# dcmlr/groundgrid

Measured on AMD Instinct MI355X. Metric: point clouds/s (Velodyne-64, ~120k pts, 120m/0.33m grid), higher is better.
Workload: dtype f32+f64 (the reference's mixed float/double arithmetic, bit-exact)

## Files before the change

groundgrid_amd/csrc/gg_context.hip:

```cpp
#include <float.h>
#include <math.h>
#include <stdio.h>
#include <string.h>

#include <algorithm>
#include <atomic>
#include <condition_variable>
#include <cstdlib>
#include <cstdio>
#include <functional>
#include <mutex>
#include <string>
#include <thread>
#include <vector>
#include <chrono>

#include <dlfcn.h>
#include <sched.h>
#include <unistd.h>

#include "gg_internal.h"
#include "host_helper.h"
#include "scroll_core.h"
#include "sweep_core.h"
// ... 816 lines not shown
    a.slot_cfg_launch = own_half[0] ? 1 : 0;
    if (split) {
        if (!ctx->probe_no_fork) {
            HIPCHK(ctx, hipEventRecord(ctx->half_fork, s));
            HIPCHK(ctx, hipStreamWaitEvent(ctx->half_stream, ctx->half_fork, 0));
        }
        Arena a2 = a;
        a2.front_sync = a.front_sync2;
        a2.sweep_sync = a.sweep_sync2;
        a2.sweep_rec_clouds = 0;
        a2.scan_sync = a.scan_sync2;
        a2.slot_cfg_launch = own_half[1] ? 1 : 0;
        a.fresh_launch = fresh_half[0] ? 1 : 0;
        a2.fresh_launch = fresh_half[1] ? 1 : 0;
        if (const int rc = fill_fresh(0, n_first, s)) return rc;
        if (const int rc = fill_fresh(n_first, nb, ctx->half_stream)) return rc;
        HIPCHK(ctx, hipMemcpyAsync(dp, hp, sizeof(CloudParams) * n_first, hipMemcpyHostToDevice, s));
        HIPCHK(ctx, hipMemcpyAsync(dp + n_first, hp + n_first, sizeof(CloudParams) * (nb - n_first), hipMemcpyHostToDevice, ctx->half_stream));
        launch_sequence(ctx, a, dp, score_half[0] ? io_score : io, n_first, max_n[0], s, nullptr, hp[0].slot, false, score_half[0]);
        launch_sequence(ctx, a2, dp + n_first, score_half[1] ? io_score : io, nb - n_first, max_n[1], ctx->half_stream, nullptr, hp[n_first].slot, false, score_half[1]);
        HIPCHK(ctx, hipGetLastError());
        HIPCHK(ctx, ctx->ring.recorded2(g, ctx->half_stream));
        HIPCHK(ctx, hipEventRecord(ctx->half_done, ctx->half_stream));
        ctx->have_half_event = true;
    } else {
        a.fresh_launch = fresh_half[0] ? 1 : 0;
        if (const int rc = fill_fresh(0, nb, s)) return rc;
        if (const int rc = launch_or_replay(ctx, a, hp, dp, score_half[0] ? io_score : io, nb, max_n[0], s, plan, score_half[0])) return rc;
        HIPCHK(ctx, hipGetLastError());
    }
    HIPCHK(ctx, ctx->ring.recorded(g, s));
    HIPCHK(ctx, hipEventRecord(ctx->batch_event, s));
    ctx->last_batch_stream = s;
    ctx->have_batch_event = true;
    if (s != ctx->stream) ctx->map_event_pending = false;
    return GG_OK;
}

void free_call_scratch(CallScratch &m)
{
    if (m.dev) hipFree(m.dev);
    if (m.pinned) hipHostFree(m.pinned);
    m = CallScratch{};
}
void free_call_scratch(CallScratch &m, ParamRing &r)
{
    free_call_scratch(m);
    r.destroy();
}

struct TableUpload {
    size_t offset;
    const void *src;
    size_t bytes;
};
int alloc_call_scratch(gg_context *ctx, const char *who, hipStream_t st, size_t dev_bytes, size_t pinned_bytes, std::initializer_list<TableUpload> tables, CallScratch *mem,
                       ParamRing *ring)
{
    hipStreamCaptureStatus cs = hipStreamCaptureStatusNone;
    if (hipStreamIsCapturing(st, &cs) == hipSuccess && cs != hipStreamCaptureStatusNone)
        return fail(ctx, GG_ERR_INVALID, who, "the first call allocates its scratch and cannot be captured into a graph");
    (void)hipGetLastError();
    CallScratch m;
    ParamRing r;
    int code = GG_ERR_NOMEM;
    const char *what = "device scratch";
    hipError_t e = hipMalloc(&m.dev, dev_bytes);
    if (e != hipSuccess) m.dev = nullptr;
    if (e == hipSuccess) {
        what = "pinned parameter ring";
        e = hipHostMalloc(&m.pinned, pinned_bytes, hipHostMallocDefault);
        if (e != hipSuccess) m.pinned = nullptr;
    }
    if (e == hipSuccess) code = GG_ERR_HIP;
    if (e == hipSuccess && ring) {
        what = "events";
        e = r.create();
    }
    for (const TableUpload &t : tables)
        if (e == hipSuccess) {
            what = "table upload";
            e = hipMemcpy((char *)m.dev + t.offset, t.src, t.bytes, hipMemcpyHostToDevice);
        }
    if (e != hipSuccess) {
        free_call_scratch(m, r);
        (void)hipGetLastError();
        return fail(ctx, code, (std::string(who) + ": " + what).c_str(), e);
    }
    *mem = m;
    if (ring) *ring = r;
    return GG_OK;
}

void map_shift(double res, double pos_x, double pos_y, double odom_x, double odom_y, int s[2], double moved[2])
{
    const double odom[2] = {odom_x, odom_y};
    const double pos[2] = {pos_x, pos_y};
    for (int i = 0; i < 2; ++i) {
        const double tmp = (odom[i] - pos[i]) / res;
        s[i] = -(int)(tmp + 0.5 * (tmp > 0 ? 1 : -1));
        moved[i] = pos[i] + (double)(-s[i]) * res;
    }
}

}

static int rebuild_patch_table(gg_context *ctx, const DevConfig &cfg);

extern "C" {

int gg_abi_version(void) { return GG_ABI_VERSION; }

const char *gg_kernel_name(int k)
{
    static const char *names[GG_NUM_KERNELS] = {"k_classify", "k_scan", "k_scatter", "k_reduce", "k_patch", "k_sweep", "k_label"};
    return (k >= 0 && k < GG_NUM_KERNELS) ? names[k] : "?";
}

void gg_default_config(gg_config *c)
{
    if (!c) return;
    c->point_count_cell_variance_threshold = 10;
    c->max_ring = 1024;
    c->groundpatch_detection_minimum_threshold = 0.01;
    c->distance_factor = 0.0001;
    c->minimum_distance_factor = 0.0005;
    c->miminum_point_height_threshold = 0.3;
    c->minimum_point_height_obstacle_threshold = 0.1;
    c->outlier_tolerance = 0.1;
    c->ground_patch_detection_minimum_point_count_threshold = 0.25;
    c->patch_size_change_distance = 20;
    c->occupied_cells_decrease_factor = 5.0;
    c->occupied_cells_point_count_factor = 20;
    c->min_outlier_detection_ground_confidence = 1.25;
    c->thread_count = 8;
}

void gg_default_geometry(gg_geometry *g)
{
    if (!g) return;
    g->length = 120.0f;
    g->resolution = .33f;
    g->vertical_point_ang_dist = (float)(0.00174532925 * 2);
    g->min_dist_squared = 12.0f;
}

int gg_create(const gg_geometry *geom_in, int n_slots, size_t max_points, int device, gg_context **out)
{
    if (!out) return GG_ERR_INVALID;
    *out = nullptr;
    if (n_slots <= 0 || max_points == 0 || max_points > (size_t)1 << 30) return GG_ERR_INVALID;
    gg_geometry geom;
    gg_default_geometry(&geom);
    if (geom_in) {
        if (geom_in->length > 0.f) geom.length = geom_in->length;
        if (geom_in->resolution > 0.f) geom.resolution = geom_in->resolution;
        const float sensor[2] = {geom_in->vertical_point_ang_dist, geom_in->min_dist_squared};
        for (const float v : sensor)
            if (!(v >= 0.f) || isinf(v)) return GG_ERR_GEOMETRY;
        if (geom_in->vertical_point_ang_dist > 0.f) geom.vertical_point_ang_dist = geom_in->vertical_point_ang_dist;
        if (geom_in->min_dist_squared > 0.f) geom.min_dist_squared = geom_in->min_dist_squared;
    }

    const double res = (double)geom.resolution;
    const int n = (int)round((double)geom.length / res);
    const size_t dimension = (size_t)geom.length;
    const size_t cellCount = (size_t)roundf((float)dimension / geom.resolution);
    if (n < 8 || (size_t)n != cellCount) return GG_ERR_GEOMETRY;

    int ndev = 0;
    if (hipGetDeviceCount(&ndev) != hipSuccess || ndev <= 0 || device < 0 || device >= ndev) return GG_ERR_NO_DEVICE;
    hipDeviceProp_t prop;
    if (hipGetDeviceProperties(&prop, device) != hipSuccess) return GG_ERR_NO_DEVICE;
    if (strncmp(prop.gcnArchName, "gfx950", 6) != 0) return GG_ERR_NO_DEVICE;

    gg_context *ctx = new (std::nothrow) gg_context();
    if (!ctx) return GG_ERR_NOMEM;
    ctx->device = device;
    ctx->geom = geom;
    ctx->n_slots = n_slots;
    ctx->max_points = max_points;
    gg_default_config(&ctx->cfg);
    ctx->pos_x.assign(n_slots, 0.0);
    ctx->no_confidence.assign(n_slots, 0);
    ctx->fresh.assign(n_slots, 0);
    ctx->fresh_z.assign(n_slots, 0.0f);
    ctx->fresh_enabled = !(getenv("GG_FRESH_MAPS") && atoi(getenv("GG_FRESH_MAPS")) == 0);
    ctx->lazy_pending.assign(n_slots, 0);
    ctx->lazy_params.assign(n_slots, CloudParams{});
    ctx->slot_own.assign(n_slots, 0);
    ctx->score_on.assign(n_slots, 0);
    ctx->slot_cfg.assign(n_slots, gg_config{});
    ctx->slot_dev.assign(n_slots, DevConfig{});
    ctx->pos_y.assign(n_slots, 0.0);

#define CREATE_CHK(call)                                             \
    do {                                                             \
        hipError_t e__ = (call);                                     \
        if (e__ != hipSuccess) {                                     \
            fprintf(stderr, "groundgrid_hip: %s failed: %s\n", #call, hipGetErrorString(e__)); \
            gg_destroy(ctx);                                         \
            return e__ == hipErrorOutOfMemory ? GG_ERR_NOMEM : GG_ERR_HIP; \
        }                                                            \
    } while (0)

    CREATE_CHK(hipSetDevice(device));
    CREATE_CHK(hipStreamCreateWithFlags(&ctx->stream, hipStreamNonBlocking));
    CREATE_CHK(hipStreamCreateWithFlags(&ctx->h2d_stream, hipStreamNonBlocking));
    CREATE_CHK(hipStreamCreateWithFlags(&ctx->d2h_stream, hipStreamNonBlocking));
    CREATE_CHK(hipStreamCreateWithFlags(&ctx->half_stream, hipStreamNonBlocking));
    CREATE_CHK(hipEventCreateWithFlags(&ctx->half_fork, hipEventDisableTiming));
    CREATE_CHK(hipEventCreateWithFlags(&ctx->half_done, hipEventDisableTiming));
    CREATE_CHK(hipEventCreateWithFlags(&ctx->map_event, hipEventDisableTiming));
    CREATE_CHK(hipEventCreateWithFlags(&ctx->batch_event, hipEventDisableTiming));
    CREATE_CHK(hipEventCreateWithFlags(&ctx->gather_event, hipEventDisableTiming));
    CREATE_CHK(hipEventCreateWithFlags(&ctx->fork_event, hipEventDisableTiming));
    CREATE_CHK(hipEventCreateWithFlags(&ctx->join_event, hipEventDisableTiming));
    CREATE_CHK(hipEventCreateWithFlags(&ctx->layers_event, hipEventDisableTiming));
    if (const char *e = getenv("GG_GRAPH")) ctx->graphs_enabled = atoi(e) != 0;

    Arena &a = ctx->arena;
    Geometry &g = a.g;
    g.rows = g.cols = n;
    g.C = n * n;
    g.tiles_r = (n + TILE - 1) / TILE;
    g.tiles_c = (n + TILE - 1) / TILE;
    g.T = g.tiles_r * g.tiles_c;
    g.resolution = res;
    g.inv_resolution = 1.0 / res;
    g.length0 = g.length1 = (double)n * res;
    g.half0 = 0.5 * g.length0;
    g.half1 = 0.5 * g.length1;
    g.resolution_f = (float)res;
    g.min_dist_squared = geom.min_dist_squared;
    g.center = n / 2 - 1;
    a.hist_pitch = (g.T + 3) & ~3;
    a.n_slots = n_slots;
    if (g.T > 65535 || (size_t)4 * a.hist_pitch * sizeof(uint32_t) > 150 * 1024) {
        gg_destroy(ctx);
        return GG_ERR_GEOMETRY;
    }
    a.PW = g.T <= 1024 ? (n_slots >= PW_BIG_CONTEXT_SLOTS ? 2048 : 1024) : 8192;
    if (getenv("GG_PW")) a.PW = atoi(getenv("GG_PW"));
    if (a.PW < 64 || a.PW % 64 != 0) {
        gg_destroy(ctx);
        return GG_ERR_INVALID;
    }
    a.tune_sweep_waves = getenv("GG_SWEEP_WAVES") ? atoi(getenv("GG_SWEEP_WAVES")) : 0;
    a.tune_sweep_gpw = getenv("GG_SWEEP_GPW") ? atoi(getenv("GG_SWEEP_GPW")) : 0;
    a.tune_sweep_split = getenv("GG_SWEEP_SPLIT") ? atoi(getenv("GG_SWEEP_SPLIT")) : 0;
    a.tune_sweep_pair = getenv("GG_SWEEP_PAIR") ? atoi(getenv("GG_SWEEP_PAIR")) : 0;
    a.tune_sweep_pair_wgs = getenv("GG_SWEEP_PAIR_WGS") ? atoi(getenv("GG_SWEEP_PAIR_WGS")) : 0;
    a.tune_sweep_pair_waves = getenv("GG_SWEEP_PAIR_WAVES") ? atoi(getenv("GG_SWEEP_PAIR_WAVES")) : 0;
    a.tune_front = getenv("GG_FRONT") ? atoi(getenv("GG_FRONT")) : 0;
    a.tune_k2_per_cloud = getenv("GG_K2_PER_CLOUD") ? atoi(getenv("GG_K2_PER_CLOUD")) : 0;
    a.tune_k2_dense_share = getenv("GG_K2_DENSE_SHARE") ? atoi(getenv("GG_K2_DENSE_SHARE")) : 0;
    a.k2_skip = getenv("GG_K2_SKIP") ? atoi(getenv("GG_K2_SKIP")) : 0;
    a.NCH = (int)((max_points + a.PW - 1) / a.PW);
    make_dev_config(ctx->cfg, a.cfg);

    ctx->h_expected.resize((size_t)g.C);
    for (size_t i = 0; i < cellCount; ++i)
        for (size_t j = 0; j < cellCount; ++j) {
            const float dist = (float)hypot((double)i - (double)cellCount / 2.0, (double)j - (double)cellCount / 2.0);
            ctx->h_expected[i + j * cellCount] = atanf(1 / dist) / geom.vertical_point_ang_dist;
        }

    ctx->sweep_params = gg::sweep::make_params(n, res, geom.min_dist_squared, ctx->cfg.occupied_cells_decrease_factor);
    if (gg::sweep_lds_bytes(ctx->sweep_params) > 158 * 1024) {
        gg_destroy(ctx);
        return GG_ERR_GEOMETRY;
    }
    std::vector<uint16_t> tile_rank(g.T), rank_tile(g.T);
    {
        std::vector<std::pair<uint32_t, int>> order(g.T);
        for (int tc = 0; tc < g.tiles_c; ++tc)
            for (int tr = 0; tr < g.tiles_r; ++tr) order[tr + tc * g.tiles_r] = {morton2((uint32_t)tr, (uint32_t)tc), tr + tc * g.tiles_r};
        std::sort(order.begin(), order.end());
        for (int r = 0; r < g.T; ++r) {
            rank_tile[r] = (uint16_t)order[r].second;
            tile_rank[order[r].second] = (uint16_t)r;
        }
    }

    const size_t A = 256;
    size_t off = 0;
    auto carve = [&](size_t bytes) {
        const size_t o = off;
        off = align_up(off + bytes, A);
        return o;
    };
    const size_t C = (size_t)g.C;
    const size_t Cpad = align_up(C * 4, A) / 4;
    const size_t Npad = align_up(max_points * 8, A) / 8;
    const size_t o_expected = carve(C * 4);
    const size_t o_ptable = carve(C * 16);
    const size_t o_trank = carve((size_t)g.T * 2);
    const size_t o_rtile = carve((size_t)g.T * 2);
    const size_t o_rcell0 = carve((size_t)g.T * 4);
    const size_t percall_slot_floats = align_up((size_t)g.T * PERCALL_BLOCK * 4, A) / 4;
    const size_t o_layers = carve((size_t)n_slots * percall_slot_floats * 4);
    a.gpl = make_gp_layout(n);
    a.gp_bits_off = (int)align_up((size_t)a.gpl.elems, 16);
    a.gp_bits_words = (a.gpl.elems / 64 + 2 + 1) & ~1;
    a.gp2_stride = align_up(((size_t)a.gp_bits_off + (size_t)a.gp_bits_words) * 8, A) / 8;
    a.gp_bits_stride = a.gp2_stride;
    const size_t o_gp2 = carve((size_t)n_slots * a.gp2_stride * 8);
    const size_t o_rec = carve((size_t)n_slots * Npad * 8);
    const size_t o_sorted = carve((size_t)n_slots * Npad * 8);
    a.zcell_stride = align_up((Npad + (size_t)32 * g.T + 64) * 4, A) / 4;
    const size_t o_zcell = carve((size_t)n_slots * a.zcell_stride * 4);
    a.hist_stride = align_up((size_t)a.NCH * a.hist_pitch * 4, A) / 4;
    const size_t o_hist = carve((size_t)n_slots * a.hist_stride * 4);
    a.emit_stride = align_up((size_t)a.NCH * 4 * 4, A) / 4;
    const size_t o_emit = carve((size_t)n_slots * a.emit_stride * 4);
    const size_t o_totals = carve((size_t)n_slots * 4 * 4);
    a.tile_start_stride = align_up((size_t)(g.T + 1) * 4, A) / 4;
    const size_t o_tstart = carve((size_t)n_slots * a.tile_start_stride * 4);
    a.tile_live_stride = align_up((size_t)g.T, A);
    const size_t o_tlive = carve((size_t)n_slots * a.tile_live_stride * 4);
    a.tile_list_stride = align_up((size_t)g.T * 16, A) / 16;
    const size_t o_tlist = carve((size_t)n_slots * a.tile_list_stride * 16);
    const size_t o_tlcnt = carve((size_t)n_slots * 2 * 4);
    const size_t o_fsync = carve(((size_t)2 * n_slots + 16) * 4);
    const size_t o_ssync = carve(64);
    const size_t o_fsync2 = carve(((size_t)2 * n_slots + 16) * 4);
    const size_t o_ssync2 = carve(64);
    const size_t o_scansync = carve((size_t)n_slots * SCAN_SYNC_WORDS * 8);
    const size_t o_scansync2 = carve((size_t)n_slots * SCAN_SYNC_WORDS * 8);
    a.sweep_xchg_stride = align_up(std::max<size_t>(gg::sweep_xchg_entries(ctx->sweep_params), 1) * 16, A) / 8;
    const size_t o_xchg = carve((size_t)n_slots * a.sweep_xchg_stride * 8);
    a.sweep_rec_stride = gg::sweep_pair_rec_floats(ctx->sweep_params);
    a.sweep_rec_clouds = a.sweep_rec_stride ? std::min(n_slots, SWEEP_PAIR_MAX_CLOUDS) : 0;
    const size_t o_srec = carve(std::max<size_t>((size_t)a.sweep_rec_clouds * a.sweep_rec_stride * 4, 64));
    const size_t o_params = carve((size_t)PARAM_RING * n_slots * sizeof(CloudParams));
    const size_t o_gparams = carve(sizeof(CloudParams));
    const size_t o_spts = carve(max_points * sizeof(gg_point16));
    const size_t o_slab = carve(max_points);
    const size_t o_sidx = carve(max_points * 4);
    const size_t o_scnt = carve(64);
    const size_t o_scls = carve(max_points);
    const size_t o_scell = carve(max_points * 4);
    size_t o_apts[GG_ASYNC_DEPTH], o_alab[GG_ASYNC_DEPTH], o_aidx[GG_ASYNC_DEPTH], o_acnt[GG_ASYNC_DEPTH];
    for (int k = 0; k < GG_ASYNC_DEPTH; ++k) {
        o_apts[k] = carve(max_points * sizeof(gg_point16));
        o_acnt[k] = carve(64 + max_points * 5 + 64);
        o_aidx[k] = o_alab[k] = 0;
    }
    const size_t o_scroll = carve(a.gp2_stride * 8);
    const size_t o_image = carve(3 * Cpad * 4);
    const size_t o_bounds = carve(64);
    const size_t gp_valid_words = ((size_t)a.gpl.elems + 31) / 32;
    const size_t o_gpvalid = carve(gp_valid_words * 4);
    std::vector<int> gp_border;
    for (int col = 0; col < n; ++col)
        for (int row = 0; row < n; ++row)
            if (std::max(std::abs(row - a.gpl.c), std::abs(col - a.gpl.c)) >= a.gpl.c) gp_border.push_back(gp_index(a.gpl, row, col));
    a.gp_border_n = (int)gp_border.size();
    const size_t o_gpborder = carve(std::max<size_t>(gp_border.size() * 4, 64));
    a.gp_fresh_cell = 1 + (a.gpl.VS - 1) * 64;
    const size_t o_dbg = carve(64 * 8);
    const size_t o_pdbg = carve(2048 * 8);
    const bool k2_timing = getenv("GG_K2_DEBUG") && (atoi(getenv("GG_K2_DEBUG")) == 9 || atoi(getenv("GG_K2_DEBUG")) == 5 || atoi(getenv("GG_K2_DEBUG")) == 6);
    const size_t o_k2dbg = carve(k2_timing ? (size_t)K2_DBG_WGS * 32 * 8 : 64);
    const size_t o_slotmaps = carve((size_t)n_slots * sizeof(ExportMap));
    ctx->arena_bytes = off;
    CREATE_CHK(hipMalloc(&ctx->d_arena, ctx->arena_bytes));
    char *base = (char *)ctx->d_arena;
    CREATE_CHK(hipMemsetAsync(base, 0, ctx->arena_bytes, ctx->stream));

    a.expected = (const float *)(base + o_expected);
    a.patch_table = (const float4 *)(base + o_ptable);
    a.tile_rank = (const uint16_t *)(base + o_trank);
    a.rank_tile = (const uint16_t *)(base + o_rtile);
    a.rank_cell0 = (const uint32_t *)(base + o_rcell0);
    a.layers = (float *)(base + o_layers);
    a.gp2 = (float2 *)(base + o_gp2);
    a.gp_bits = (unsigned long long *)(base + o_gp2) + a.gp_bits_off;
    a.slot_layer_stride = percall_slot_floats;
    a.rec = (uint2 *)(base + o_rec);
    a.sorted = (uint2 *)(base + o_sorted);
    a.zcell = (float *)(base + o_zcell);
    a.point_stride = Npad;
    a.hist = (uint32_t *)(base + o_hist);
    a.chunk_emit = (uint32_t *)(base + o_emit);
    a.totals = (uint32_t *)(base + o_totals);
    a.tile_start = (uint32_t *)(base + o_tstart);
    a.tile_live = (uint32_t *)(base + o_tlive);
    a.tile_list = (uint4 *)(base + o_tlist);
    a.tile_list_cnt = (uint32_t *)(base + o_tlcnt);
    a.front_sync = (uint32_t *)(base + o_fsync);
    a.sweep_sync = (uint32_t *)(base + o_ssync);
    a.front_sync2 = (uint32_t *)(base + o_fsync2);
    a.sweep_sync2 = (uint32_t *)(base + o_ssync2);
    a.scan_sync = (unsigned long long *)(base + o_scansync);
    a.scan_sync2 = (unsigned long long *)(base + o_scansync2);
    {
        const uint32_t first_epoch[4] = {0u, 0u, 1u, 0u};
        CREATE_CHK(hipMemcpyAsync(a.sweep_sync, first_epoch, sizeof first_epoch, hipMemcpyHostToDevice, ctx->stream));
        const uint32_t first_epoch2[4] = {0u, 0u, 0x80000001u, 0u};
        CREATE_CHK(hipMemcpyAsync(a.sweep_sync2, first_epoch2, sizeof first_epoch2, hipMemcpyHostToDevice, ctx->stream));
        CREATE_CHK(hipStreamSynchronize(ctx->stream));
    }
    {
        CREATE_CHK(hipHostMalloc((void **)&ctx->h_dev_error, 64, hipHostMallocMapped));
        *ctx->h_dev_error = 0u;
        void *dptr = nullptr;
        CREATE_CHK(hipHostGetDevicePointer(&dptr, (void *)ctx->h_dev_error, 0));
        a.dev_error = (uint32_t *)dptr;
    }
    a.sweep_xchg = (unsigned long long *)(base + o_xchg);
    a.sweep_rec = a.sweep_rec_clouds ? (float *)(base + o_srec) : nullptr;
    a.pair_dbg = getenv("GG_PAIR_TIMING") ? (unsigned long long *)(base + o_pdbg) : nullptr;
    a.flags = 0;
    a.k2_debug = getenv("GG_K2_DEBUG") ? atoi(getenv("GG_K2_DEBUG")) : 0;
    a.k2_dbg = (unsigned long long *)(base + o_k2dbg);
    a.k3_debug = getenv("GG_K3_DEBUG") ? atoi(getenv("GG_K3_DEBUG")) : 0;
    a.k5_debug = getenv("GG_K5_DEBUG") ? atoi(getenv("GG_K5_DEBUG")) : 0;
    ctx->d_params = (CloudParams *)(base + o_params);
    ctx->d_gparams = (CloudParams *)(base + o_gparams);
    ctx->d_stage_pts = (gg_point16 *)(base + o_spts);
    ctx->d_stage_labels = (uint8_t *)(base + o_slab);
    ctx->d_stage_index = (int32_t *)(base + o_sidx);
    ctx->d_stage_counts = (int32_t *)(base + o_scnt);
    ctx->d_stage_class = (uint8_t *)(base + o_scls);
    ctx->d_stage_cell = (int32_t *)(base + o_scell);
    for (int k = 0; k < GG_ASYNC_DEPTH; ++k) {
        gg_context::AsyncSlot &as = ctx->async_slot[k];
        as.d_pts = (gg_point16 *)(base + o_apts[k]);
        as.d_counts = (int32_t *)(base + o_acnt[k]);
        as.d_index = (int32_t *)(base + o_acnt[k] + 64);
        as.d_labels = nullptr;
    }
    ctx->d_scroll_scratch = (float *)(base + o_scroll);
    ctx->d_image = (float *)(base + o_image);
    ctx->d_bounds = (float *)(base + o_bounds);
    a.gp_valid = (const uint32_t *)(base + o_gpvalid);
    a.gp_border = (const int *)(base + o_gpborder);
    {
        int row, col;
        if (gp_cell_of(a.gpl, a.gp_fresh_cell, row, col)) {
            gg_destroy(ctx);
            return GG_ERR_INVALID;
        }
        CREATE_CHK(hipMemcpyAsync(base + o_gpborder, gp_border.data(), gp_border.size() * 4, hipMemcpyHostToDevice, ctx->stream));
        CREATE_CHK(hipStreamSynchronize(ctx->stream));
    }
    if (getenv("GG_SWEEP_TIMING")) {
        ctx->d_sweep_dbg = (unsigned long long *)(base + o_dbg);
        const unsigned long long mode = getenv("GG_SWEEP_DEBUG") ? strtoull(getenv("GG_SWEEP_DEBUG"), nullptr, 0) : 0ull;
        hipStreamSynchronize(ctx->stream);
        hipMemcpy(ctx->d_sweep_dbg + 63, &mode, 8, hipMemcpyHostToDevice);
    }

    std::vector<uint32_t> gp_valid(gp_valid_words, 0u);
    for (int col = 0; col < n; ++col)
        for (int row = 0; row < n; ++row) {
            const int e = gp_index(a.gpl, row, col);
            gp_valid[(size_t)e >> 5] |= 1u << (e & 31);
        }
    {
        const int group = getenv("GG_FILL_GROUP") ? atoi(getenv("GG_FILL_GROUP")) : 16;
        if (group == 8 || group == 16 || group == 32)
            for (size_t w = 0; w < gp_valid_words; ++w) {
                uint32_t v = gp_valid[w], o = 0u;
                for (int b = 0; b < 32; b += group) {
                    const uint32_t gm = (group == 32 ? 0xFFFFFFFFu : ((1u << group) - 1u)) << b;
                    if (v & gm) o |= gm;
                }
                gp_valid[w] = o;
            }
    }
    CREATE_CHK(hipMemcpyAsync(base + o_gpvalid, gp_valid.data(), gp_valid_words * 4, hipMemcpyHostToDevice, ctx->stream));
    CREATE_CHK(hipMemcpyAsync(base + o_expected, ctx->h_expected.data(), C * 4, hipMemcpyHostToDevice, ctx->stream));
    CREATE_CHK(hipMemcpyAsync(base + o_trank, tile_rank.data(), (size_t)g.T * 2, hipMemcpyHostToDevice, ctx->stream));
    CREATE_CHK(hipMemcpyAsync(base + o_rtile, rank_tile.data(), (size_t)g.T * 2, hipMemcpyHostToDevice, ctx->stream));
    std::vector<uint32_t> rank_cell0(g.T);
    for (int r = 0; r < g.T; ++r) {
        const int tile = rank_tile[r];
        rank_cell0[r] = (uint32_t)((tile % g.tiles_r) * TILE) | ((uint32_t)((tile / g.tiles_r) * TILE) << 16);
    }
    CREATE_CHK(hipMemcpyAsync(base + o_rcell0, rank_cell0.data(), (size_t)g.T * 4, hipMemcpyHostToDevice, ctx->stream));
    std::vector<ExportMap> slot_maps((size_t)n_slots);
    for (int s = 0; s < n_slots; ++s) slot_maps[(size_t)s] = ExportMap{s, 0, 0.0f, 0};
    CREATE_CHK(hipMemcpyAsync(base + o_slotmaps, slot_maps.data(), slot_maps.size() * sizeof(ExportMap), hipMemcpyHostToDevice, ctx->stream));
    ctx->d_slot_maps = (const ExportMap *)(base + o_slotmaps);
    CREATE_CHK(hipStreamSynchronize(ctx->stream));

    CREATE_CHK(hipHostMalloc((void **)&ctx->h_params, sizeof(CloudParams) * PARAM_RING * n_slots, hipHostMallocDefault));
    CREATE_CHK(hipHostMalloc((void **)&ctx->h_stage_pts, max_points * sizeof(gg_point16), hipHostMallocDefault));
    CREATE_CHK(hipHostMalloc((void **)&ctx->h_stage_labels, max_points, hipHostMallocDefault));
    CREATE_CHK(hipHostMalloc((void **)&ctx->h_stage_index, max_points * 4, hipHostMallocDefault));
    CREATE_CHK(hipHostMalloc((void **)&ctx->h_stage_counts, 64, hipHostMallocDefault));
    CREATE_CHK(ctx->ring.create());
    for (int k = 0; k < GG_ASYNC_DEPTH; ++k) {
        gg_context::AsyncSlot &as = ctx->async_slot[k];
        CREATE_CHK(hipHostMalloc((void **)&as.h_pts, max_points * sizeof(gg_point16), hipHostMallocDefault));
        CREATE_CHK(hipHostMalloc((void **)&as.h_counts, 64 + max_points * 5 + 64, hipHostMallocDefault));
        as.h_index = as.h_counts + 16;
        as.h_labels = nullptr;
        if (hipHostGetDevicePointer((void **)&as.hd_counts, as.h_counts, 0) != hipSuccess) {
            as.hd_counts = nullptr;
            (void)hipGetLastError();
        }
        CREATE_CHK(hipEventCreateWithFlags(&as.uploaded, hipEventDisableTiming));
        CREATE_CHK(hipEventCreateWithFlags(&as.computed, hipEventDisableTiming));
        CREATE_CHK(hipEventCreateWithFlags(&as.downloaded, hipEventDisableTiming));
    }

    ctx->helper.configure((getenv("GG_HOST_THREADS") ? std::max(1, std::min(atoi(getenv("GG_HOST_THREADS")), 16)) : 8) - 1);
    {
        const int rc = rebuild_patch_table(ctx, a.cfg);
        if (rc != GG_OK) {
            gg_destroy(ctx);
            return rc;
        }
    }
    {
        const int rc = gg_reset_maps(ctx, 0, n_slots, 0.0, 0.0, 0.0f, 0, nullptr);
        if (rc != GG_OK) {
            gg_destroy(ctx);
            return rc;
        }
    }
    CREATE_CHK(hipStreamSynchronize(ctx->stream));
#undef CREATE_CHK
    *out = ctx;
    return GG_OK;
}

void gg_destroy(gg_context *ctx)
{
    if (!ctx) return;
    ctx->helper.stop();
    hipSetDevice(ctx->device);
    if (ctx->have_batch_event) hipEventSynchronize(ctx->batch_event);
    if (ctx->half_stream) hipStreamSynchronize(ctx->half_stream);
    if (ctx->h2d_stream) hipStreamSynchronize(ctx->h2d_stream);
    if (ctx->stream) hipStreamSynchronize(ctx->stream);
    if (ctx->d2h_stream) hipStreamSynchronize(ctx->d2h_stream);
    for (auto &p : ctx->pending) {
        if (p.owns_start) hipEventDestroy(p.start);
        hipEventDestroy(p.stop);
    }
    for (hipEvent_t e : ctx->free_single_events) hipEventDestroy(e);
    ctx->ring.destroy();
    if (ctx->half_fork) hipEventDestroy(ctx->half_fork);
    if (ctx->half_done) hipEventDestroy(ctx->half_done);
    if (ctx->half_stream) hipStreamDestroy(ctx->half_stream);
    for (int k = 0; k < GG_ASYNC_DEPTH; ++k) {
        gg_context::AsyncSlot &as = ctx->async_slot[k];
        if (as.h_pts) hipHostFree(as.h_pts);
        if (as.h_counts) hipHostFree(as.h_counts);
        if (as.uploaded) hipEventDestroy(as.uploaded);
        if (as.computed) hipEventDestroy(as.computed);
        if (as.downloaded) hipEventDestroy(as.downloaded);
    }
    if (ctx->map_event) hipEventDestroy(ctx->map_event);
    if (ctx->batch_event) hipEventDestroy(ctx->batch_event);
    if (ctx->gather_event) hipEventDestroy(ctx->gather_event);
    drop_graphs(ctx);
    if (ctx->fork_event) hipEventDestroy(ctx->fork_event);
    if (ctx->join_event) hipEventDestroy(ctx->join_event);
    if (ctx->layers_event) hipEventDestroy(ctx->layers_event);
    for (auto &r : ctx->registered) hipHostUnregister(r.first);
    ctx->registered.clear();
    if (ctx->h2d_stream) hipStreamDestroy(ctx->h2d_stream);
    if (ctx->d2h_stream) hipStreamDestroy(ctx->d2h_stream);
    if (ctx->h_dev_error) hipHostFree((void *)ctx->h_dev_error);
    if (ctx->h_params) hipHostFree(ctx->h_params);
    if (ctx->h_stage_pts) hipHostFree(ctx->h_stage_pts);
    if (ctx->h_stage_labels) hipHostFree(ctx->h_stage_labels);
    if (ctx->h_stage_index) hipHostFree(ctx->h_stage_index);
    if (ctx->h_stage_counts) hipHostFree(ctx->h_stage_counts);
    if (ctx->d_planes) hipFree(ctx->d_planes);
    free_call_scratch(ctx->move_mem, ctx->move_ring);
    free_call_scratch(ctx->export_mem, ctx->export_ring);
    free_call_scratch(ctx->split_mem);
    if (ctx->d_pc2) hipFree(ctx->d_pc2);
    if (ctx->h_pc2) hipHostFree(ctx->h_pc2);
    if (ctx->h_planes) hipHostFree(ctx->h_planes);
    if (ctx->d_arena) hipFree(ctx->d_arena);
    if (ctx->d_slot_cfg) hipFree(ctx->d_slot_cfg);
    if (ctx->d_score_block) hipFree(ctx->d_score_block);
    if (ctx->stream) hipStreamDestroy(ctx->stream);
    delete ctx;
}

static int wait_for_batches_in_flight(gg_context *ctx)
{
    HIPCHK(ctx, hipSetDevice(ctx->device));
    if (ctx->have_batch_event) HIPCHK(ctx, hipEventSynchronize(ctx->batch_event));
    if (ctx->have_half_event) HIPCHK(ctx, hipEventSynchronize(ctx->half_done));
    HIPCHK(ctx, hipStreamSynchronize(ctx->stream));
    return GG_OK;
}

static int rebuild_patch_table(gg_context *ctx, const DevConfig &cfg)
{
    const Geometry &g = ctx->arena.g;
    const int rows = g.rows, cols = g.cols;
    std::vector<float> t((size_t)g.C * 4);
    const double res2 = (double)g.resolution_f * (double)g.resolution_f;
    for (int j = 0; j < cols; ++j)
        for (int i = 0; i < rows; ++i) {
            float *e = &t[((size_t)i + (size_t)j * rows) * 4];
            const float expected = ctx->h_expected[(size_t)i + (size_t)j * rows];
// ... 1224 lines not shown
    unsigned mask = 0u;
    if (layers)
        for (int l = 0; l < GG_NUM_LAYERS; ++l)
            if (layers[l]) mask |= 1u << l;
    if (!mask || (ctx->flags & GG_FLAG_MINIMAL_LAYERS)) {
        const int rc = filter_cloud_impl(ctx, slot, cloud, n, map_from_cloud, origin, base_z, out_cloud, out_n, out_label, out_index);
        if (rc != GG_OK || !mask) return rc;
        void *d[GG_NUM_LAYERS];
        for (int l = 0; l < GG_NUM_LAYERS; ++l) d[l] = layers[l];
        return get_layers_impl(ctx, slot, d);
    }
    HIPCHK(ctx, hipSetDevice(ctx->device));
    const size_t C = (size_t)ctx->arena.g.C, plane = align_up(C * 4, 256) / 4;
    if (!ctx->d_planes) HIPCHK(ctx, hipMalloc((void **)&ctx->d_planes, (size_t)GG_NUM_LAYERS * plane * sizeof(float)));
    if (!ctx->h_planes) HIPCHK(ctx, hipHostMalloc((void **)&ctx->h_planes, (size_t)GG_NUM_LAYERS * plane * sizeof(float), hipHostMallocDefault));
    LayerPlan plan;
    plan.mask = mask;
    bool staged[GG_NUM_LAYERS] = {};
    for (int l = 0; l < GG_NUM_LAYERS; ++l) {
        if (!((mask >> l) & 1u)) continue;
        staged[l] = !host_range_registered(ctx, layers[l], C * sizeof(float));
        plan.dst[l] = staged[l] ? (void *)(ctx->h_planes + (size_t)l * plane) : (void *)layers[l];
    }
    int ticket = -1;
    const int rc = enqueue_ticket(ctx, slot, cloud, n, map_from_cloud, origin, base_z, &ticket, false, &plan);
    if (rc != GG_OK) {
        (void)hipStreamSynchronize(ctx->d2h_stream);
        (void)hipStreamSynchronize(ctx->stream);
        return rc;
    }
    auto copy_staged = [&](unsigned group) {
        int want[GG_NUM_LAYERS], n_want = 0;
        for (int l = 0; l < GG_NUM_LAYERS; ++l)
            if (staged[l] && ((group >> l) & 1u)) want[n_want++] = l;
        if (n_want)
            ctx->helper.split((size_t)n_want * C, [&](size_t lo, size_t hi) {
                for (size_t k = lo / C; k < (size_t)n_want && k * C < hi; ++k) {
                    const size_t a0 = std::max(lo, k * C) - k * C, a1 = std::min(hi, (k + 1) * C) - k * C;
                    memcpy(layers[want[k]] + a0, ctx->h_planes + (size_t)want[k] * plane + a0, (a1 - a0) * sizeof(float));
                }
            });
    };
    if (mask & EARLY_LAYERS) {
        HIPCHK(ctx, hipEventSynchronize(ctx->join_event));
        copy_staged(EARLY_LAYERS);
    }
    const int rc_wait = gg_filter_cloud_wait(ctx, ticket, out_cloud, out_n, out_label, out_index);
    SYNCCHK(ctx, hipEventSynchronize(ctx->layers_event));
    if (rc_wait != GG_OK) return rc_wait;
    if (ctx->layer_copy_failed) {
        ctx->layer_copy_failed = false;
        ctx->last_error = "gg_filter_cloud_layers: a layer download could not be enqueued";
        return GG_ERR_HIP;
    }
    copy_staged(~EARLY_LAYERS);
    return GG_OK;
}

extern "C++" {
namespace {
struct Rccl {
    struct UniqueId {
        char internal[128];
    };
    int (*GetUniqueId)(UniqueId *) = nullptr;
    int (*CommInitRank)(void **, int, UniqueId, int) = nullptr;
    int (*CommDestroy)(void *) = nullptr;
    int (*AllGather)(const void *, void *, size_t, int, void *, hipStream_t) = nullptr;
    const char *(*GetErrorString)(int) = nullptr;
    bool ok = false;
    Rccl()
    {
        void *h = dlopen("librccl.so.1", RTLD_NOW | RTLD_GLOBAL);
        if (!h) h = dlopen("librccl.so", RTLD_NOW | RTLD_GLOBAL);
        if (!h) h = dlopen("/opt/rocm/lib/librccl.so.1", RTLD_NOW | RTLD_GLOBAL);
        if (!h) return;
        GetUniqueId = reinterpret_cast<decltype(GetUniqueId)>(dlsym(h, "ncclGetUniqueId"));
        CommInitRank = reinterpret_cast<decltype(CommInitRank)>(dlsym(h, "ncclCommInitRank"));
        CommDestroy = reinterpret_cast<decltype(CommDestroy)>(dlsym(h, "ncclCommDestroy"));
        AllGather = reinterpret_cast<decltype(AllGather)>(dlsym(h, "ncclAllGather"));
        GetErrorString = reinterpret_cast<decltype(GetErrorString)>(dlsym(h, "ncclGetErrorString"));
        ok = GetUniqueId && CommInitRank && CommDestroy && AllGather;
    }
};
Rccl &rccl()
{
    static Rccl r;
    return r;
}
}
}

int gg_collective_available(void) { return rccl().ok ? 1 : 0; }

int gg_comm_unique_id(uint8_t id_out[128])
{
    if (!id_out) return GG_ERR_INVALID;
    if (!rccl().ok) return GG_ERR_NO_DEVICE;
    Rccl::UniqueId id;
    if (rccl().GetUniqueId(&id) != 0) return GG_ERR_HIP;
    memcpy(id_out, id.internal, 128);
    return GG_OK;
}

int gg_comm_init_rank(const uint8_t id_in[128], int n_ranks, int rank, void **comm_out)
{
    if (!id_in || !comm_out || n_ranks <= 0 || rank < 0 || rank >= n_ranks) return GG_ERR_INVALID;
    *comm_out = nullptr;
    if (!rccl().ok) return GG_ERR_NO_DEVICE;
    Rccl::UniqueId id;
    memcpy(id.internal, id_in, 128);
    if (rccl().CommInitRank(comm_out, n_ranks, id, rank) != 0) return GG_ERR_HIP;
    return GG_OK;
}

int gg_comm_init_rank_for(gg_context *ctx, const uint8_t id_in[128], int n_ranks, int rank, void **comm_out)
{
    if (!ctx) return GG_ERR_INVALID;
    HIPCHK(ctx, hipSetDevice(ctx->device));
    const int rc = gg_comm_init_rank(id_in, n_ranks, rank, comm_out);
    if (rc != GG_OK) fail(ctx, rc, rc == GG_ERR_NO_DEVICE ? "librccl.so could not be loaded" : "ncclCommInitRank failed");
    return rc;
}

int gg_comm_destroy(void *comm)
{
    if (!comm) return GG_ERR_INVALID;
    if (!rccl().ok) return GG_ERR_NO_DEVICE;
    return rccl().CommDestroy(comm) == 0 ? GG_OK : GG_ERR_HIP;
}

int gg_allgather_label_masks(gg_context *ctx, void *comm, const uint8_t *d_send, uint8_t *d_recv, size_t bytes_per_rank, void *stream)
{
    if (!ctx) return GG_ERR_INVALID;
    if (!comm) return fail(ctx, GG_ERR_INVALID, "gg_allgather_label_masks: null communicator");
    if (!d_send || !d_recv || bytes_per_rank == 0) return fail(ctx, GG_ERR_INVALID, "gg_allgather_label_masks: null buffer / zero size");
    if (!rccl().ok) return fail(ctx, GG_ERR_NO_DEVICE, "librccl.so could not be loaded");
    HIPCHK(ctx, hipSetDevice(ctx->device));
    const hipStream_t s = pick_stream(ctx, stream);
    if (ctx->have_batch_event && ctx->last_batch_stream != s) HIPCHK(ctx, hipStreamWaitEvent(s, ctx->batch_event, 0));
    if (const int rc_half = stream_waits_for_second_half(ctx, s)) return rc_half;
    const int rc = rccl().AllGather(d_send, d_recv, bytes_per_rank,  1, comm, s);
    if (rc != 0) {
        char buf[256];
        snprintf(buf, sizeof buf, "ncclAllGather: %s", rccl().GetErrorString ? rccl().GetErrorString(rc) : "error");
        ctx->last_error = buf;
        return GG_ERR_HIP;
    }
    HIPCHK(ctx, hipEventRecord(ctx->gather_event, s));
    ctx->gather_stream = s;
    ctx->gather_lo = d_send;
    ctx->gather_hi = d_send + bytes_per_rank;
    return GG_OK;
}

int gg_get_point_classes(gg_context *ctx, int slot, size_t n, uint8_t *out_class, int32_t *out_cell)
{
    if (!slot_ok(ctx, slot)) return GG_ERR_CAPACITY;
    if (n > ctx->max_points) return GG_ERR_CAPACITY;
    if (n == 0) return GG_OK;
    HIPCHK(ctx, hipSetDevice(ctx->device));
    if (const int rc = own_stream_waits_for_batches(ctx)) return rc;
    launch_decode_classes(ctx->arena, slot, n, ctx->d_stage_class, ctx->d_stage_cell, ctx->stream);
    HIPCHK(ctx, hipGetLastError());
    if (out_class) HIPCHK(ctx, hipMemcpyAsync(out_class, ctx->d_stage_class, n, hipMemcpyDeviceToHost, ctx->stream));
    if (out_cell) HIPCHK(ctx, hipMemcpyAsync(out_cell, ctx->d_stage_cell, n * 4, hipMemcpyDeviceToHost, ctx->stream));
    SYNCCHK(ctx, hipStreamSynchronize(ctx->stream));
    return GG_OK;
}

int gg_run_stage(gg_context *ctx, int slot, int stage, const gg_stage_args *args)
{
    if (!slot_ok(ctx, slot)) return GG_ERR_CAPACITY;
    if (!args) return fail(ctx, GG_ERR_INVALID, "gg_run_stage: null arguments");
    const Geometry &g = ctx->arena.g;
    switch (stage) {
    case GG_STAGE_DETECT_GROUND_PATCHES:
        if (args->section < -1 || args->section > 3) return fail(ctx, GG_ERR_INVALID, "gg_run_stage: section must be 0..3 or -1");
        break;
    case GG_STAGE_SPIRAL_GROUND_INTERPOLATION: break;
    case GG_STAGE_DETECT_GROUND_PATCH_3:
    case GG_STAGE_DETECT_GROUND_PATCH_5: {
        const int h = stage == GG_STAGE_DETECT_GROUND_PATCH_3 ? 1 : 2;
        if (args->i < h || args->j < h || args->i >= g.rows - h || args->j >= g.cols - h) return fail(ctx, GG_ERR_INVALID, "gg_run_stage: the cell's block leaves the map");
        break;
    }
    case GG_STAGE_INTERPOLATE_CELL:
        if (args->i < 1 || args->j < 1 || args->i >= g.rows - 1 || args->j >= g.cols - 1) return fail(ctx, GG_ERR_INVALID, "gg_run_stage: the cell's block leaves the map");
        break;
    default: return fail(ctx, GG_ERR_INVALID, "gg_run_stage: unknown stage");
    }
    HIPCHK(ctx, hipSetDevice(ctx->device));
    if (const int rc = own_stream_waits_for_batches(ctx)) return rc;
    const hipStream_t s = ctx->stream;
    Arena a = ctx->arena;
    a.flags = ctx->flags;
    a.eigen_reduction = ctx->conv.eigen_reduction;
    const bool own = ctx->slot_own[slot] != 0;
    if (own) a.cfg = ctx->slot_dev[slot];
    if (stage == GG_STAGE_DETECT_GROUND_PATCHES || stage == GG_STAGE_SPIRAL_GROUND_INTERPOLATION) {
        int r;
        HIPCHK(ctx, ctx->ring.acquire(&r));
        CloudParams *hp = ctx->h_params + (size_t)r * ctx->n_slots, *dp = ctx->d_params + (size_t)r * ctx->n_slots;
        hp[0] = CloudParams{};
        hp[0].slot = slot;
        hp[0].base_z = (float)args->base_z;
        hp[0].pos_x = ctx->pos_x[slot];
        hp[0].pos_y = ctx->pos_y[slot];
        hp[0].cfg_index = own ? slot : -1;
        HIPCHK(ctx, hipMemcpyAsync(dp, hp, sizeof(CloudParams), hipMemcpyHostToDevice, s));
        if (stage == GG_STAGE_DETECT_GROUND_PATCHES) {
            a.slot_cfg_launch = own ? 1 : 0;
            launch_patch_stage(a, dp, slot, args->section, s);
        } else {
            sweep::Params sp = ctx->sweep_params;
            sp.decrease = own ? ctx->slot_cfg[slot].occupied_cells_decrease_factor : ctx->cfg.occupied_cells_decrease_factor;
            sp.inv_decrease = 1.0 / sp.decrease;
            sp.decay_fast = sp.decrease >= 1.25 && sp.decrease < 1e300;
            sp.keep_points = 1;
            launch_sweep(a, sp, dp, 1, s, nullptr);
        }
        HIPCHK(ctx, hipGetLastError());
        HIPCHK(ctx, ctx->ring.recorded(r, s));
    } else {
        launch_stage_cell(a, slot, stage, args->i, args->j, s);
        HIPCHK(ctx, hipGetLastError());
    }
    ctx->no_confidence[slot] = 0;
    if (const int rc = own_stream_mutated_map(ctx)) return rc;
    SYNCCHK(ctx, hipStreamSynchronize(s));
    return GG_OK;
}

int gg_insert_cloud(gg_context *ctx, int slot, const gg_point32 *cloud, size_t start, size_t end, const float origin[3], uint8_t *out_class, int32_t *out_cell)
{
    if (!slot_ok(ctx, slot)) return GG_ERR_CAPACITY;
    if (!origin || end < start || (end > start && !cloud)) return fail(ctx, GG_ERR_INVALID, "gg_insert_cloud: null cloud / origin or end < start");
    const size_t n = end - start;
    if (n > ctx->max_points) return fail(ctx, GG_ERR_CAPACITY, "gg_insert_cloud: range larger than max_points");
    if (n == 0) return GG_OK;
    HIPCHK(ctx, hipSetDevice(ctx->device));
    if (const int rc = own_stream_waits_for_batches(ctx)) return rc;
    const hipStream_t s = ctx->stream;
    if (const int rc = ensure_lazy_layers(ctx, slot, true)) return rc;
    Arena a = ctx->arena;
    a.flags = ctx->flags & ~(unsigned)GG_FLAG_MINIMAL_LAYERS;
    a.eigen_reduction = ctx->conv.eigen_reduction;
    if (ctx->slot_own[slot]) a.cfg = ctx->slot_dev[slot];
    launch_materialise_maps(a, ctx->d_slot_maps + slot, 1, s);
    HIPCHK(ctx, hipGetLastError());
    for (size_t i = 0; i < n; ++i) {
        const gg_point32 &p = cloud[start + i];
        gg_point16 &d = ctx->h_stage_pts[i];
        d.x = p.x, d.y = p.y, d.z = p.z, d.ring = p.ring, d.pad = 0;
    }
    HIPCHK(ctx, hipMemcpyAsync(ctx->d_stage_pts, ctx->h_stage_pts, n * sizeof(gg_point16), hipMemcpyHostToDevice, s));
    int r;
    HIPCHK(ctx, ctx->ring.acquire(&r));
    CloudParams *hp = ctx->h_params + (size_t)r * ctx->n_slots, *dp = ctx->d_params + (size_t)r * ctx->n_slots;
    hp[0] = CloudParams{};
    hp[0].slot = slot;
    hp[0].n_points = (int)n;
    hp[0].ox = origin[0], hp[0].oy = origin[1], hp[0].oz = origin[2];
    hp[0].pos_x = ctx->pos_x[slot];
    hp[0].pos_y = ctx->pos_y[slot];
    hp[0].no_confidence = ctx->no_confidence[slot] ? 1 : 0;
    hp[0].fresh = 0;
    HIPCHK(ctx, hipMemcpyAsync(dp, hp, sizeof(CloudParams), hipMemcpyHostToDevice, s));
    BatchIO io{};
    io.d_points = ctx->d_stage_pts;
    io.cloud_stride = ctx->max_points;
    io.point_format = GG_POINT16;
    const int front = launch_classify(a, dp, io, 1, (int)n, s);
    if (front == FRONT_THREE_LAUNCHES) launch_scan(a, dp, 1, s);
    if (front != FRONT_ONE_LAUNCH) launch_scatter(a, dp, 1, (int)n, s);
    launch_stage_insert(a, dp, s);
    launch_fill_bytes((uint8_t *)(a.tile_live + (size_t)slot * a.tile_live_stride), (size_t)a.g.T * 4, 0xFF, s);
    launch_decode_classes(a, slot, n, ctx->d_stage_class, ctx->d_stage_cell, s);
    HIPCHK(ctx, hipGetLastError());
    if (out_class) HIPCHK(ctx, hipMemcpyAsync(out_class, ctx->d_stage_class, n, hipMemcpyDeviceToHost, s));
    if (out_cell) HIPCHK(ctx, hipMemcpyAsync(out_cell, ctx->d_stage_cell, n * 4, hipMemcpyDeviceToHost, s));
    HIPCHK(ctx, ctx->ring.recorded(r, s));
    ctx->lazy_pending[slot] = 0;
    if (const int rc = own_stream_mutated_map(ctx)) return rc;
    SYNCCHK(ctx, hipStreamSynchronize(s));
    return GG_OK;
}

extern "C" int gg_debug_set_tuning(gg_context *ctx, const char *key, int value)
{
    if (!ctx || !key || value < 0) return GG_ERR_INVALID;
    if (!strcmp(key, "pw")) return ctx->arena.PW;
    if (!strcmp(key, "graph_replays")) return (int)std::min<long>(ctx->graph_replays, 1 << 30);
    if (!strcmp(key, "fresh_count")) {
        int c = 0;
        for (int k = 0; k < ctx->n_slots; ++k) c += ctx->fresh[k] ? 1 : 0;
        return c;
    }
    if (!strcmp(key, "lazy_count")) {
        int c = 0;
        for (int k = 0; k < ctx->n_slots; ++k) c += ctx->lazy_pending[k] ? 1 : 0;
        return c;
    }
    if (!strcmp(key, "export_variant_default")) return EXPORT_VARIANT_DEFAULT;
    if (!strcmp(key, "import_variant_default")) return IMPORT_VARIANT_DEFAULT;
    if (!strcmp(key, "images_variant_default")) return IMAGES_VARIANT_DEFAULT;
    if (!strcmp(key, "graphs")) {
        ctx->graphs_enabled = value != 0;
        drop_graphs(ctx);
        return GG_OK;
    }
    drop_graphs(ctx);
    if (!strcmp(key, "sweep_waves")) ctx->arena.tune_sweep_waves = value;
    else if (!strcmp(key, "sweep_gpw")) ctx->arena.tune_sweep_gpw = value;
    else if (!strcmp(key, "sweep_split")) ctx->arena.tune_sweep_split = value;
    else if (!strcmp(key, "sweep_pair")) ctx->arena.tune_sweep_pair = value;
    else if (!strcmp(key, "sweep_pair_wgs")) ctx->arena.tune_sweep_pair_wgs = value;
    else if (!strcmp(key, "sweep_pair_waves")) ctx->arena.tune_sweep_pair_waves = value;
    else if (!strcmp(key, "fresh_maps")) ctx->fresh_enabled = value != 0;
    else if (!strcmp(key, "front")) ctx->arena.tune_front = std::min(value, 3);
    else if (!strcmp(key, "sweep_poll_cap")) ctx->arena.tune_sweep_poll_cap = value;
    else if (!strcmp(key, "scan_parts")) ctx->arena.tune_scan_parts = value;
    else if (!strcmp(key, "scan_poll_cap")) ctx->arena.tune_scan_poll_cap = value;
    else if (!strcmp(key, "upload_pieces")) ctx->upload_pieces = value;
    else if (!strcmp(key, "results_direct")) ctx->results_direct = value;
    else if (!strcmp(key, "halves_min_clouds")) ctx->halves_min_clouds = std::max(2, value);
    else if (!strcmp(key, "move_chunk")) ctx->move_chunk_tune = value;
    else if (!strcmp(key, "export_variant")) ctx->export_variant = value ? 1 : 0;
    else if (!strcmp(key, "import_variant")) ctx->import_variant = value ? 1 : 0;
    else if (!strcmp(key, "images_variant")) ctx->images_variant = value ? 1 : 0;
    else if (!strcmp(key, "halves_no_fork")) ctx->probe_no_fork = value != 0;
    else if (!strcmp(key, "scan_fault")) ctx->arena.tune_scan_fault = value;
    else if (!strcmp(key, "sweep_fault")) ctx->arena.tune_sweep_fault = value;
    else if (!strcmp(key, "probe_unordered_streams")) ctx->probe_unordered_streams = value != 0;
    else if (!strcmp(key, "clear_device_error")) *ctx->h_dev_error = 0u;
    else if (!strcmp(key, "k2_per_cloud")) ctx->arena.tune_k2_per_cloud = value;
    else if (!strcmp(key, "k2_dense_share")) ctx->arena.tune_k2_dense_share = std::min(value, 15);
    else return GG_ERR_INVALID;
    return GG_OK;
}

extern "C" int gg_debug_sweep_timing(gg_context *ctx, unsigned long long out[64])
{
    if (!ctx || !out || !ctx->d_sweep_dbg) return GG_ERR_INVALID;
    if (hipMemcpy(out, ctx->d_sweep_dbg, 64 * 8, hipMemcpyDeviceToHost) != hipSuccess) return GG_ERR_HIP;
    return GG_OK;
}

extern "C" int gg_debug_pair_timing(gg_context *ctx, unsigned long long out[2048])
{
    if (!ctx || !out || !ctx->arena.pair_dbg) return GG_ERR_INVALID;
    if (hipDeviceSynchronize() != hipSuccess) return GG_ERR_HIP;
    if (hipMemcpy(out, ctx->arena.pair_dbg, 2048 * 8, hipMemcpyDeviceToHost) != hipSuccess) return GG_ERR_HIP;
    return GG_OK;
}

extern "C" int gg_debug_k2_census(gg_context *ctx, unsigned long long *out, int reset)
{
    if (!ctx || !out || ctx->arena.k2_debug != 5) return GG_ERR_INVALID;
    if (hipDeviceSynchronize() != hipSuccess) return GG_ERR_HIP;
    if (hipMemcpy(out, ctx->arena.k2_dbg, 1024 * 8 * 8, hipMemcpyDeviceToHost) != hipSuccess) return GG_ERR_HIP;
    if (reset) {
        std::vector<unsigned long long> z(1024 * 8, 0ull);
        for (int k = 0; k < 1024; ++k) z[(size_t)k * 8 + 4] = ~0ull;
        if (hipMemcpy(ctx->arena.k2_dbg, z.data(), z.size() * 8, hipMemcpyHostToDevice) != hipSuccess) return GG_ERR_HIP;
    }
    return GG_OK;
}

extern "C" int gg_debug_k2_trace(gg_context *ctx, unsigned long long *out, int n)
{
    if (!ctx || !out || ctx->arena.k2_debug != 6 || n < 1 || n > 65536) return GG_ERR_INVALID;
    if (hipDeviceSynchronize() != hipSuccess) return GG_ERR_HIP;
    if (hipMemcpy(out, ctx->arena.k2_dbg, (size_t)n * 4 * 8, hipMemcpyDeviceToHost) != hipSuccess) return GG_ERR_HIP;
    return GG_OK;
}

extern "C" int gg_debug_k2_phases(gg_context *ctx, unsigned long long out[64], int reset)
{
    if (!ctx || !out || ctx->arena.k2_debug != 9) return GG_ERR_INVALID;
    if (hipDeviceSynchronize() != hipSuccess) return GG_ERR_HIP;
    std::vector<unsigned long long> all((size_t)32768 * 32);
    if (hipMemcpy(all.data(), ctx->arena.k2_dbg, all.size() * 8, hipMemcpyDeviceToHost) != hipSuccess) return GG_ERR_HIP;
    for (int k = 0; k < 64; ++k) out[k] = 0;
    for (size_t wg = 0; wg < 32768; ++wg)
        for (int k = 0; k < 32; ++k) out[k] += all[wg * 32 + k];
    if (reset && hipMemset(ctx->arena.k2_dbg, 0, all.size() * 8) != hipSuccess) return GG_ERR_HIP;
    return GG_OK;
}

int gg_get_kernel_times(gg_context *ctx, double ms[GG_NUM_KERNELS], int64_t launches[GG_NUM_KERNELS], int reset)
{
    if (!ctx) return GG_ERR_INVALID;
    HIPCHK(ctx, hipSetDevice(ctx->device));
    const int rc = drain_profile(ctx);
    if (rc != GG_OK) return rc;
    for (int k = 0; k < GG_NUM_KERNELS; ++k) {
        if (ms) ms[k] = ctx->k_ms[k];
        if (launches) launches[k] = ctx->k_launches[k];
        if (reset) {
            ctx->k_ms[k] = 0.0;
            ctx->k_launches[k] = 0;
        }
    }
    return GG_OK;
}

}
```

groundgrid_amd/csrc/gg_internal.h:

```cpp
#pragma once

#include <hip/hip_runtime.h>
#include <stdint.h>

#include <atomic>
#include <mutex>

#include "groundgrid_hip.h"
#include "gp_layout.h"

namespace gg {

constexpr int TILE = 16;
constexpr int TILE_CELLS = TILE * TILE;
constexpr uint32_t KEY_OUTSIDE = 0xFFFFFFFFu;
constexpr int K2_DBG_WGS = 32768;
constexpr int PW_BIG_CONTEXT_SLOTS = 128;
constexpr int SWEEP_LATENCY_MAX_CLOUDS = 256;
constexpr int K2_MIN_GROUPS_PER_CLOUD = 64;
constexpr int PACKED_TILE_COUNTERS_MIN_T = 1024;
constexpr int K2_LIGHT_MAX = 512;
constexpr int KEY_TILE_SHIFT = 12;
constexpr int SCAN_MAX_PARTS = 16, SCAN_SYNC_WORDS = 1 + SCAN_MAX_PARTS;
constexpr uint32_t KEY_EMIT_BIT = 1u << 10;
constexpr int KEY_CLASS_SHIFT = 8;

struct DevConfig {
    int point_count_cell_variance_threshold;
    int max_ring;
    double outlier_tolerance;
    double gpd_min_point_count_threshold;
    double patch_size_change_distance_sq;
    double occupied_cells_decrease_factor;
    double occupied_cells_point_count_factor;
    double occupied_cells_point_count_factor_x2;
    double min_outlier_detection_ground_confidence;
    double distance_factor_sq;
    double minimum_distance_factor_sq;
    double minimum_distance_factor_x10_sq;
    double min_dist_fac;
    double min_point_height_thres;
    double min_point_height_obs_thres;
    double inv_decrease;
    int decay_fast;
};

struct Geometry {
    int rows, cols;
    int C;
    int tiles_r, tiles_c, T;
    double resolution;
    double inv_resolution;
    double length0, length1;
    double half0, half1;
    float resolution_f;
    float min_dist_squared;
    int center;
};

struct CloudParams {
    int slot;
    int n_points;
    float ox, oy, oz;
    float base_z;
    double pos_x, pos_y;
    int has_tf;
    int fresh;
    int no_confidence;
    double tf[12];
    int label_shift;
    int io_index;
    int cfg_index = -1;
};

struct Arena {
    Geometry g;
    DevConfig cfg;
    const float *expected;
    const float4 *patch_table;
    const uint16_t *tile_rank;
    const uint16_t *rank_tile;
    const uint32_t *rank_cell0;
    float *layers;  size_t slot_layer_stride;
    const uint32_t *gp_valid;
    float2 *gp2;    size_t gp2_stride;    GpLayout gpl;
    unsigned long long *gp_bits;  size_t gp_bits_stride;  int gp_fresh_cell;
    int gp_bits_off, gp_bits_words;
    const int *gp_border;  int gp_border_n;
    int fresh_launch;
    uint2 *rec;     uint2 *sorted;  size_t point_stride;
    float *zcell;   size_t zcell_stride;
    uint32_t *hist;        size_t hist_stride;
    int hist_pitch;
    uint32_t *front_sync;
    uint32_t *dev_error;
    uint32_t *chunk_emit;  size_t emit_stride;
    uint32_t *totals;
    uint32_t *tile_start;  size_t tile_start_stride;
    uint32_t *tile_live;   size_t tile_live_stride;
    uint4 *tile_list;      size_t tile_list_stride;
    uint32_t *tile_list_cnt;
    unsigned long long *scan_sync;
    uint32_t *front_sync2, *sweep_sync2;
    unsigned long long *scan_sync2;
    uint32_t *sweep_sync;
    unsigned long long *sweep_xchg; size_t sweep_xchg_stride;
    float *sweep_rec; size_t sweep_rec_stride; int sweep_rec_clouds;
    unsigned long long *pair_dbg;
    int n_slots;
    int PW;
    int NCH;
    int tune_sweep_waves;
    int tune_sweep_gpw;
    int tune_sweep_split;
    int tune_sweep_pair;
    int tune_sweep_pair_wgs;
    int tune_sweep_pair_waves;
    int tune_sweep_poll_cap;
    int tune_sweep_fault;
    int tune_scan_fault;
    int tune_scan_poll_cap;
    int tune_scan_parts;
    int tune_front;
    int tune_k2_per_cloud;
    int tune_k2_dense_share;
    int k2_skip;
    unsigned flags;
    int k2_debug;
    unsigned long long *k2_dbg;
    int k5_debug;
    int k3_debug;
    int eigen_reduction;
    const DevConfig *slot_cfg;
    int slot_cfg_launch;
};

constexpr int PERCALL_LAYERS = 9;
constexpr int PERCALL_BLOCK = PERCALL_LAYERS * TILE * TILE;
enum : int { PL_POINTS = 0, PL_VARIANCE = 1, PL_MINGROUNDHEIGHT = 2, PL_M2 = 3, PL_POINTSRAW = 4, PL_MEANVARIANCE = 5, PL_MAXGROUNDHEIGHT = 6,
             PL_GROUNDCANDIDATES = 7, PL_PLANEDIST = 8 };
__host__ __device__ inline int percall_position(int layer)
{
    switch (layer) {
    case GG_LAYER_POINTS: return PL_POINTS;
    case GG_LAYER_VARIANCE: return PL_VARIANCE;
    case GG_LAYER_MINGROUNDHEIGHT: return PL_MINGROUNDHEIGHT;
    case GG_LAYER_M2: return PL_M2;
    case GG_LAYER_POINTSRAW: return PL_POINTSRAW;
    case GG_LAYER_MEANVARIANCE: return PL_MEANVARIANCE;
    case GG_LAYER_MAXGROUNDHEIGHT: return PL_MAXGROUNDHEIGHT;
    case GG_LAYER_GROUNDCANDIDATES: return PL_GROUNDCANDIDATES;
    case GG_LAYER_PLANEDIST: return PL_PLANEDIST;
    default: return -1;
    }
}
__host__ __device__ inline float *percall_ptr(const Arena &a, int slot) { return a.layers + (size_t)slot * a.slot_layer_stride; }
__host__ __device__ inline size_t percall_index(int rank, int position, int cell) { return (size_t)rank * PERCALL_BLOCK + (size_t)position * (TILE * TILE) + (size_t)cell; }
__device__ inline size_t percall_index_of(const Arena &a, int position, int row, int col)
{
    return percall_index(a.tile_rank[(row / TILE) + (col / TILE) * a.g.tiles_r], position, (row % TILE) + (col % TILE) * TILE);
}

__host__ __device__ inline float layer_reset_value(int layer)
{
    return layer == GG_LAYER_MINGROUNDHEIGHT ? 3.402823466e+38f  : layer == GG_LAYER_MAXGROUNDHEIGHT ? 1.175494351e-38f  : 0.0f;
}
__host__ __device__ inline int live_bit(int cell) { return cell >> 3; }
__device__ inline bool cell_is_live(const Arena &a, int slot, int row, int col)
{
    const int rank = a.tile_rank[(row / TILE) + (col / TILE) * a.g.tiles_r];
    return ((a.tile_live[(size_t)slot * a.tile_live_stride + rank] >> live_bit((row % TILE) + (col % TILE) * TILE)) & 1u) != 0u;
}

__host__ __device__ inline float2 *gp2_ptr(const Arena &a, int slot) { return a.gp2 + (size_t)slot * a.gp2_stride; }
__host__ __device__ inline int gp_idx(const Arena &a, int row, int col) { return gp_index(a.gpl, row, col); }

struct BatchIO {
    const void *d_points;
    size_t cloud_stride;
    int point_format;
    uint8_t *d_labels;
    int32_t *d_out_index;
    gg_point32 *d_out_clouds;
    int32_t *d_out_counts;
    uint8_t *d_label_masks;
    uint8_t *d_out_pc2;
};

constexpr int SCORE_BINS = GG_SCORE_MAX_LABELS + 1;
constexpr int SCORE_WORDS = 1 + SCORE_BINS * 2;
struct ScoreArgs {
    const uint8_t *ring_bin;
    const uint8_t *slot_on;
    unsigned long long *scores;
};

constexpr int EXPORT_TILE = 64;
struct ExportMap {
    int slot;
    int fresh;
    float fresh_z;
    int reserved;
};
struct PlaneArgs {
    const ExportMap *maps;
    const uint32_t *block_off, *elem;
    const uint16_t *cell;
    int blocks_r, blocks_c;
    unsigned mask;
    int n_planes;
    int order;
    float *planes;
    size_t plane_stride;
};

constexpr int IMAGE_GATHER_PARTS = 64;
struct ImageArgs {
    const ExportMap *maps;
    const uint32_t *block_off, *elem;
    const uint16_t *cell;
    int blocks_r, blocks_c;
    unsigned mask;
    int n_planes;
    uint8_t *images;
    size_t image_stride;
    float *partials;
    int n_parts;
    float *bounds;
    float *terrain;
    size_t terrain_stride;
    int terrain_layout;
};
inline int image_parts(const Geometry &g, int variant)
{
    const int blocks = ((g.rows + EXPORT_TILE - 1) / EXPORT_TILE) * ((g.cols + EXPORT_TILE - 1) / EXPORT_TILE);
    const int gather = (g.C + 255) / 256 < IMAGE_GATHER_PARTS ? (g.C + 255) / 256 : IMAGE_GATHER_PARTS;
    return variant == 1 ? gather : blocks;
}

struct SplitCloud {
    int slot;
    int n_points;
    int fresh;
    float fresh_z;
    int has_tf;
    int io_index;
    double pos_x, pos_y;
    double tf[12];
};
struct SplitSet {
    gg_point16 *points;
    float *height;
    int32_t *source;
};
struct SplitArgs {
    const SplitCloud *clouds;
    int point_format;
    const void *points;
    size_t cloud_stride;
    const uint8_t *labels, *masks;
    SplitSet set[2];
    int32_t *counts;
    uint2 *chunk_counts;
    int nch;
};

struct PerDeviceOnce {
    std::atomic<uint64_t> done{0};
    std::mutex lock;
    template <class F> void run(F opt_in)
    {
        int dev = 0;
        (void)hipGetDevice(&dev);
        const bool tracked = dev >= 0 && dev < 64;
        const uint64_t bit = tracked ? 1ull << dev : 0ull;
        if (tracked && (done.load(std::memory_order_acquire) & bit)) return;
        std::lock_guard<std::mutex> g(lock);
        if (tracked && (done.load(std::memory_order_relaxed) & bit)) return;
        opt_in();
        if (tracked) done.fetch_or(bit, std::memory_order_release);
    }
};

enum : uint32_t { GG_DEVERR_NONE = 0, GG_DEVERR_FRONT_WAIT = 1 , GG_DEVERR_SWEEP_WAIT = 2 ,
                  GG_DEVERR_SCAN_WAIT = 3  };
enum : int { FRONT_AUTO = 0, FRONT_THREE_LAUNCHES = 1, FRONT_SCAN_IN_CLASSIFY = 2, FRONT_ONE_LAUNCH = 3 };
constexpr int FRONT_DEFAULT_SHAPE = FRONT_THREE_LAUNCHES;

int launch_classify(const Arena &a, const CloudParams *d_params, const BatchIO &io, int n_clouds, int max_n, hipStream_t s);
void launch_scan(const Arena &a, const CloudParams *d_params, int n_clouds, hipStream_t s);
void launch_scatter(const Arena &a, const CloudParams *d_params, int n_clouds, int max_n, hipStream_t s);
void launch_reduce(const Arena &a, const CloudParams *d_params, int n_clouds, hipStream_t s);
void launch_stage_insert(const Arena &a, const CloudParams *d_params, hipStream_t s);
void launch_reduce_lazy(const Arena &a, const CloudParams &cp, hipStream_t s);
void launch_reduce_lazy_batch(const Arena &a, const CloudParams *d_params, int n_clouds, hipStream_t s);
void launch_export(const Arena &a, const PlaneArgs &x, int n_maps, int variant, hipStream_t s);
void launch_import(const Arena &a, const PlaneArgs &x, int n_maps, int variant, hipStream_t s);
void launch_images(const Arena &a, const ImageArgs &x, int n_maps, int variant, hipStream_t s);
void launch_split(const Arena &a, const SplitArgs &x, int n_clouds, hipStream_t s);
void launch_planes_gather(const Arena &a, const PlaneArgs &x, int n_maps, hipStream_t s);
void launch_planes_scatter(const Arena &a, const PlaneArgs &x, int n_maps, hipStream_t s);
void launch_materialise_maps(const Arena &a, const ExportMap *maps, int n_maps, hipStream_t s);
void launch_patch(const Arena &a, const CloudParams *d_params, int n_clouds, hipStream_t s);
void launch_patch_stage(const Arena &a, const CloudParams *d_params, int slot, int section, hipStream_t s);
void launch_stage_cell(const Arena &a, int slot, int stage, int i, int j, hipStream_t s);
namespace sweep {
struct Params;
Params make_params(int n, double resolution, float min_dist_squared, double decrease);
}
void launch_sweep(const Arena &a, const sweep::Params &P, const CloudParams *d_params, int n_clouds, hipStream_t s,
                  unsigned long long *dbg = nullptr);
bool launch_sweep_pair(const Arena &a, const sweep::Params &P, const CloudParams *d_params, int n_clouds, hipStream_t s);
bool sweep_takes_fresh(const Arena &a, const sweep::Params &P, int n_clouds);
bool launch_sweep_pair_batch(const Arena &a, const sweep::Params &P, const CloudParams *d_params, int n_clouds, hipStream_t s);
size_t sweep_pair_rec_floats(const sweep::Params &P);
constexpr int SWEEP_PAIR_MAX_CLOUDS = 16;
size_t sweep_lds_bytes(const sweep::Params &P);
size_t sweep_xchg_entries(const sweep::Params &P);
void launch_label(const Arena &a, const CloudParams *d_params, const BatchIO &io, int n_clouds, int max_n, hipStream_t s);
void launch_score(const Arena &a, const CloudParams *d_params, const BatchIO &io, const ScoreArgs &sc, int n_clouds, int max_n, hipStream_t s);
void launch_fill(float *dst, size_t n, float v, hipStream_t s);
void launch_fill_bytes(uint8_t *dst, size_t n, uint8_t v, hipStream_t s);
void launch_fill_strided(float *dst, size_t n, size_t stride, int count, float v, hipStream_t s);
void launch_fill_percall(const Arena &a, int first_slot, int n_slots, const float init[GG_NUM_LAYERS], hipStream_t s);
void launch_fill2_strided(float2 *dst, size_t n, size_t stride, int count, float x, float y, const uint32_t *valid, hipStream_t s);
void launch_fill2(float2 *dst, size_t n, float x, float y, hipStream_t s);
void launch_reset_fresh(const Arena &a, int first_slot, int count, float x, float y, hipStream_t s, int all_ones = 0);
void launch_layer_to_u8(const float *layer, int rows, int cols, float *d_bounds, uint8_t *d_img, hipStream_t s);
void launch_terrain_image(const Arena &a, int slot, float *d_img, hipStream_t s);
void launch_scroll(const Arena &a, int slot, float2 *scratch, int s0, int s1, double pos_x, double pos_y, const double plane[4], hipStream_t s);
struct MoveParams;
void launch_scroll_batch(const Arena &a, const int2 *cells, const MoveParams *d_params, int n_maps, float2 *scratch, hipStream_t s);
void launch_pack16(const gg_point32 *src, gg_point16 *dst, size_t n, hipStream_t s);
void launch_decode_classes(const Arena &a, int slot, size_t n, uint8_t *d_class, int32_t *d_cell, hipStream_t s);

}
```

groundgrid_amd/csrc/gp_layout.h:

```cpp
#pragma once

#include <stddef.h>

#if defined(__HIPCC__)
#include <hip/hip_runtime.h>
#define GPL_HD __host__ __device__ __forceinline__
#else
#define GPL_HD inline
#endif

#ifndef GG_SWEEP_SKEW
#define GG_SWEEP_SKEW 1
#endif

namespace gg {

constexpr int GP_SHEAR = GG_SWEEP_SKEW + 1;

struct GpLayout {
    int n, c;
    int G;
    int VS;
    int elems;
};

GPL_HD GpLayout make_gp_layout(int n)
{
    GpLayout L;
    L.n = n;
    L.c = n / 2 - 1;
    const int rmax = n - 1 - L.c;
    L.G = (rmax - 1) / 64 + 1;
    L.VS = n + GP_SHEAR * 63;
    L.elems = 1 + 4 * L.G * L.VS * 64;
    return L;
}

GPL_HD int gp_index(const GpLayout &L, int row, int col)
{
    const int dx = row - L.c, dy = col - L.c;
    const int ax = dx < 0 ? -dx : dx, ay = dy < 0 ? -dy : dy;
    const int r = ax > ay ? ax : ay;
    if (r == 0) return 0;
    const int g = (r - 1) >> 6, l = (r - 1) & 63;
    int side, v;
    if (dx == -r && dy < r) {
        side = 0;
        v = col;
    } else if (dx == r) {
        side = 2;
        v = L.n - 1 - col;
    } else if (dy == -r) {
        side = 1;
        v = row;
    } else {
        side = 3;
        v = L.n - 1 - row;
    }
    return 1 + ((side * L.G + g) * L.VS + v + GP_SHEAR * l) * 64 + l;
}

GPL_HD bool gp_cell_of(const GpLayout &L, int e, int &row, int &col)
{
    if (e == 0) {
        row = col = L.c;
        return true;
    }
    if (e < 0 || e >= L.elems) return false;
    const int q = e - 1, l = q & 63, rest = q >> 6;
    const int vs = rest % L.VS, sg = rest / L.VS, g = sg % L.G, side = sg / L.G;
    const int r = 64 * g + l + 1, v = vs - GP_SHEAR * l;
    if (side > 3 || v < 0 || v >= L.n) return false;
    if (side == 0) {
        row = L.c - r;
        col = v;
    } else if (side == 2) {
        row = L.c + r;
        col = L.n - 1 - v;
    } else if (side == 1) {
        col = L.c - r;
        row = v;
    } else {
        col = L.c + r;
        row = L.n - 1 - v;
    }
    if (row < 0 || row >= L.n || col < 0 || col >= L.n) return false;
    return gp_index(L, row, col) == e;
}

}
```

groundgrid_amd/csrc/k4_sweep.hip:

```cpp
#include "gg_device.h"
#include "sweep_core.h"

#include <algorithm>
#include <cstdlib>

#include <stdlib.h>

namespace gg {

using namespace sweep;

typedef uint32_t u32x2 __attribute__((ext_vector_type(2)));

typedef __attribute__((address_space(3))) int lds_int;
typedef __attribute__((address_space(3))) uint64_t lds_u64;

__shared__ __attribute__((aligned(16))) uint32_t sweep_static[4];
#define sweep_wait_failed sweep_static[2]

template <bool DBG> struct DevMemT {
    __amdgpu_buffer_rsrc_t rsrc;
    lds_int *lds;
    int dbg_mode_rt = 0;
    unsigned long long *marks = nullptr, last_mark = 0, acc[6] = {0, 0, 0, 0, 0, 0};
    GG_DEV int dbg_mode() const { return DBG ? dbg_mode_rt : 0; }
    GG_DEV void mark(int k)
    {
        if (!(dbg_mode() & 4)) return;
        const unsigned long long now = __builtin_readcyclecounter();
        if (k > 0) acc[k] += now - last_mark;
        last_mark = now;
    }
    GG_DEV void flush_marks()
    {
        if (dbg_mode() & 4)
            for (int k = 0; k < 6; ++k) marks[k] = acc[k];
    }
    GG_DEV bool give_up(int polls, const Params &P) const
    {
        if (polls < P.poll_cap) return false;
        __hip_atomic_store(&sweep_wait_failed, 1u, __ATOMIC_RELAXED, __HIP_MEMORY_SCOPE_WORKGROUP);
        return true;
    }
    static constexpr uint32_t OOR = 0x80000000u;
    unsigned long long *xchg = nullptr;
    uint32_t seq = 0;
    GG_DEV void export_wp_if(bool c, int entry, WP v) const
    {
        if (c) {
            const unsigned long long tag = (unsigned long long)seq << 32;
            __hip_atomic_store(xchg + 2 * (size_t)entry, tag | __float_as_uint(v.w), __ATOMIC_RELAXED, __HIP_MEMORY_SCOPE_AGENT);
            __hip_atomic_store(xchg + 2 * (size_t)entry + 1, tag | __float_as_uint(v.p), __ATOMIC_RELAXED, __HIP_MEMORY_SCOPE_AGENT);
        }
    }
    GG_DEV bool import_wp(int entry, WP &v) const
    {
        const unsigned long long a = __hip_atomic_load(xchg + 2 * (size_t)entry, __ATOMIC_RELAXED, __HIP_MEMORY_SCOPE_AGENT);
        const unsigned long long b = __hip_atomic_load(xchg + 2 * (size_t)entry + 1, __ATOMIC_RELAXED, __HIP_MEMORY_SCOPE_AGENT);
        v = WP{__uint_as_float((uint32_t)a), __uint_as_float((uint32_t)b)};
        return (uint32_t)(a >> 32) == seq && (uint32_t)(b >> 32) == seq;
    }
    GG_DEV void ring_put(int word, const PrepRec &r) const
    {
        lds_u64 *p = (lds_u64 *)(lds + word);
        __hip_atomic_store(p + 0, (uint64_t)__float_as_uint(r.w_new) | ((uint64_t)__float_as_uint(r.own_g) << 32), __ATOMIC_RELAXED, __HIP_MEMORY_SCOPE_WORKGROUP);
        __hip_atomic_store(p + 1, (uint64_t)__float_as_uint(r.own_w) | ((uint64_t)__float_as_uint(r.own_p) << 32), __ATOMIC_RELAXED, __HIP_MEMORY_SCOPE_WORKGROUP);
        __hip_atomic_store(p + 2, (uint64_t)__float_as_uint(r.out_w) | ((uint64_t)__float_as_uint(r.out_p) << 32), __ATOMIC_RELAXED, __HIP_MEMORY_SCOPE_WORKGROUP);
    }
    GG_DEV PrepRec ring_get(int word) const
    {
        lds_u64 *p = (lds_u64 *)(lds + word);
        const uint64_t a = __hip_atomic_load(p + 0, __ATOMIC_RELAXED, __HIP_MEMORY_SCOPE_WORKGROUP);
        const uint64_t b = __hip_atomic_load(p + 1, __ATOMIC_RELAXED, __HIP_MEMORY_SCOPE_WORKGROUP);
        const uint64_t c = __hip_atomic_load(p + 2, __ATOMIC_RELAXED, __HIP_MEMORY_SCOPE_WORKGROUP);
        PrepRec r;
        r.w_new = __uint_as_float((uint32_t)a), r.own_g = __uint_as_float((uint32_t)(a >> 32));
        r.own_w = __uint_as_float((uint32_t)b), r.own_p = __uint_as_float((uint32_t)(b >> 32));
        r.out_w = __uint_as_float((uint32_t)c), r.out_p = __uint_as_float((uint32_t)(c >> 32));
        return r;
    }
    GG_DEV void set_counter(int word, int value) const
    {
        __hip_atomic_store(lds + word, value, __ATOMIC_RELAXED, __HIP_MEMORY_SCOPE_WORKGROUP);
    }

    GG_DEV Cell load_issue(bool valid, int cell) const
    {
        const u32x2 v = __builtin_amdgcn_raw_buffer_load_b64(rsrc, (valid && !(dbg_mode() & 2)) ? (uint32_t)cell * 8u : OOR, 0, 0);
        return Cell{__uint_as_float(v.x), __uint_as_float(v.y)};
    }
    GG_DEV Cell load_value(const Cell &queued, bool, int) const { return queued; }
    uint32_t bits_byte0 = 0u;
    GG_DEV uint32_t bits_dword(uint32_t voffset, uint32_t soffset) const { return __builtin_amdgcn_raw_buffer_load_b32(rsrc, voffset, soffset, 0); }
    GG_DEV bool bit_of(int cell) const
    {
        const unsigned e = (unsigned)cell - 1u;
        const uint32_t w = bits_dword(bits_byte0 + (e >> 5) * 4u, 0u);
        return cell <= 0 || ((w >> (e & 31u)) & 1u) != 0u;
    }
    GG_DEV Cell fresh(const Cell &v) const
    {
        Cell o;
        asm volatile("v_mov_b32 %0, %2\n\tv_mov_b32 %1, %3" : "=&v"(o.g), "=&v"(o.w) : "v"(v.g), "v"(v.w));
        return o;
    }
    GG_DEV void store(bool valid, int cell, Cell v) const
    {
        u32x2 d;
        d.x = __float_as_uint(v.g);
        d.y = __float_as_uint(v.w);
        __builtin_amdgcn_raw_buffer_store_b64(d, rsrc, (valid && !(dbg_mode() & 1)) ? (uint32_t)cell * 8u : OOR, 0, 0);
    }
    GG_DEV WP get(int word) const
    {
        const uint64_t u = __hip_atomic_load((lds_u64 *)(lds + word), __ATOMIC_RELAXED, __HIP_MEMORY_SCOPE_WORKGROUP);
        return WP{__uint_as_float((uint32_t)u), __uint_as_float((uint32_t)(u >> 32))};
    }
    GG_DEV void put(int word, WP v) const
    {
        const uint64_t u = (uint64_t)__float_as_uint(v.w) | ((uint64_t)__float_as_uint(v.p) << 32);
        __hip_atomic_store((lds_u64 *)(lds + word), u, __ATOMIC_RELAXED, __HIP_MEMORY_SCOPE_WORKGROUP);
    }
    GG_DEV void publish(int data_word, WP v, int counter_word, int value) const
    {
        const uint32_t da = (uint32_t)(data_word * 4) + lds_base(), ca = (uint32_t)(counter_word * 4) + lds_base();
        u32x2 d;
        d.x = __float_as_uint(v.w);
        d.y = __float_as_uint(v.p);
        asm volatile("ds_write_b64 %0, %1\n\tds_write_b32 %2, %3" ::"v"(da), "v"(d), "v"(ca), "v"(value) : "memory");
    }
    GG_DEV void publish_if(bool c, int lane, const LdsMap &L, int data_word, WP v, int counter_word, int value) const
    {
        const int sw = (L.scratch + 1 + 3 * lane) & ~1;
        publish(c ? data_word : sw, v, c ? counter_word : sw + 2, value);
    }
    GG_DEV void put_if(bool c, int lane, const LdsMap &L, int word, WP v) const { put(c ? word : (L.scratch + 1 + 3 * lane) & ~1, v); }
    GG_DEV WP bcast(WP v, int lane) const
    {
        return WP{__int_as_float(__builtin_amdgcn_readlane(__float_as_int(v.w), lane)), __int_as_float(__builtin_amdgcn_readlane(__float_as_int(v.p), lane))};
    }
    GG_DEV int counter(int word) const
    {
        int v;
        const uint32_t ca = (uint32_t)(word * 4) + lds_base();
        asm volatile("ds_read_b32 %0, %1\n\ts_waitcnt lgkmcnt(0)" : "=v"(v) : "v"(ca) : "memory");
        return __builtin_amdgcn_readfirstlane(v);
    }
    GG_DEV int counter_and_get(int counter_word, int data_word, WP &v) const
    {
        int c;
        u32x2 d;
        const uint32_t ca = (uint32_t)(counter_word * 4) + lds_base(), da = (uint32_t)(data_word * 4) + lds_base();
        asm volatile("ds_read_b32 %0, %2\n\tds_read_b64 %1, %3\n\ts_waitcnt lgkmcnt(0)" : "=&v"(c), "=&v"(d) : "v"(ca), "v"(da) : "memory");
        v = WP{__uint_as_float(d.x), __uint_as_float(d.y)};
        return __builtin_amdgcn_readfirstlane(c);
    }
    GG_DEV void counters3(int w0, int w1, int w2, int &v0, int &v1, int &v2) const
    {
        int a, b, c;
        const uint32_t a0 = (uint32_t)(w0 * 4) + lds_base(), a1 = (uint32_t)(w1 * 4) + lds_base(), a2 = (uint32_t)(w2 * 4) + lds_base();
        asm volatile("ds_read_b32 %0, %3\n\tds_read_b32 %1, %4\n\tds_read_b32 %2, %5\n\ts_waitcnt lgkmcnt(0)"
                     : "=&v"(a), "=&v"(b), "=&v"(c)
                     : "v"(a0), "v"(a1), "v"(a2)
                     : "memory");
        v0 = __builtin_amdgcn_readfirstlane(a);
        v1 = __builtin_amdgcn_readfirstlane(b);
        v2 = __builtin_amdgcn_readfirstlane(c);
    }
    GG_DEV uint32_t lds_base() const { return (uint32_t)(uintptr_t)lds; }
};

GG_DEV int scalar_here(int v)
{
    v = __builtin_amdgcn_readfirstlane(v);
    asm volatile("" : "+s"(v));
    return v;
}

GG_DEV float wave_shr1(float v)
{
    return __int_as_float(__builtin_amdgcn_update_dpp(__float_as_int(v), __float_as_int(v), 0x138, 0xF, 0xF, false));
}

template <bool DBG> struct WaveClockT {
    unsigned long long *out_rt;
    GG_DEV unsigned long long *out_ptr() const { return DBG ? out_rt : nullptr; }
    unsigned long long t0 = 0, polling = 0, waits = 0;
    GG_DEV void begin() { t0 = out_ptr() ? __builtin_readcyclecounter() : 0ull; }
    GG_DEV void end(int wave, int lane)
    {
        unsigned long long *out = out_ptr();
        if (out && lane == 0) {
            out[wave * 4 + 0] = t0;
            out[wave * 4 + 1] = __builtin_readcyclecounter();
            out[wave * 4 + 2] = polling;
            out[wave * 4 + 3] = waits;
        }
    }
};

#ifndef GG_SWEEP_SLEEP_LONG
#define GG_SWEEP_SLEEP_LONG 6
#endif
constexpr int SLEEP_LONG = GG_SWEEP_SLEEP_LONG;

#ifndef GG_SWEEP_REC_AHEAD
#define GG_SWEEP_REC_AHEAD 1
#endif
#ifndef GG_SWEEP_BATCH_RANGES
#define GG_SWEEP_BATCH_RANGES 3
#endif
#ifndef GG_SWEEP_BATCH_KINDS
#define GG_SWEEP_BATCH_KINDS 2
#endif
template <bool S, int B, int J> struct TripKind {
    static constexpr bool starts = S;
    static constexpr int bnd = B, join = J;
};

template <int SIDE, bool DBG, bool SPLIT, bool FRESH = false>
GG_DEV void run_chain(const Params &P, const LdsMap &L, DevMemT<DBG> &mem, int wave_of_side, int lane, WaveClockT<DBG> &clk, int g0, int g1)
{
    static_assert(!(FRESH && SPLIT), "fresh maps: the plain chain only");
    ChainLane<SIDE> st;
    int have_prep = 0;
    const int w_take = lane == 0 ? L.take_done + SIDE : ((L.scratch + 1 + 3 * lane) & ~1) + 2;
    for (int group = g0 + wave_of_side; group < g1; group += P.waves_per_side) {
        const int r0 = LANES * group + 1;
        const int nl = min(P.rings - (r0 - 1), (int)LANES);
        st.init(lane, r0, nl, group, P, L);
        const int t_first = group_first_step(), t_last = group_last_step<SIDE>(r0, nl);
        const int has_next = __builtin_amdgcn_readfirstlane(group + 1 < P.groups ? 1 : 0);
        uint32_t fo_own = 0u, fo_out = 0u, sh_own = 0u, sh_out = 0u, mq_own[2] = {0u, 0u}, mq_out[2] = {0u, 0u};
        if constexpr (FRESH) {
            const unsigned eo = (unsigned)st.ownA - 1u, eu = (unsigned)st.outA - 1u;
            fo_own = mem.bits_byte0 + 8u * (unsigned)((int)(eo >> 6) + t_first + 1 + (int)PF) + 4u * ((eo & 63u) >> 5);
            fo_out = mem.bits_byte0 + 8u * (unsigned)((int)(eu >> 6) + t_first + 1 + (int)PF) + 4u * ((eu & 63u) >> 5);
            sh_own = eo & 31u;
            sh_out = eu & 31u;
            st.xold_bit = mem.bit_of(st.xold_cell);
            st.end_bit = mem.bit_of(st.own_end);
#pragma unroll
            for (int k = 0; k < 2; ++k) {
                mq_own[k] = mem.bits_dword(fo_own, 8u * (unsigned)k);
                mq_out[k] = mem.bits_dword(fo_out, 8u * (unsigned)k);
            }
        }
        ChainSync<SIDE> sync;
        sync.init(r0, nl, group, P, L);
        const int turn = __builtin_amdgcn_readfirstlane((((join_turn_residue<SIDE>(r0) - t_first) % 3) + 3) % 3);
        auto trip = [&](const int tb, auto kind) __attribute__((always_inline)) {
            using K = decltype(kind);
            constexpr bool STARTS = K::starts;
            const bool trip_bnd = K::bnd == 3 && group > 0 && tb + (int)TRIP - 1 >= 0 && tb < st.u_len0;
            const bool trip_join = K::join == 3 && tb + (int)TRIP - 1 >= st.u_join_first && tb <= st.u_join_last;
            const bool trip_pub = K::join == 3 && has_next != 0 && tb + (int)TRIP - 1 >= st.u_l3_last && tb < st.u_lend_last;
            PrepRec rec_ahead{};
#pragma unroll
            for (int u = 0; u < TRIP; ++u) {
                const int t = tb + u;
                sync.advance(t);
                auto wait_a = [&]() {
                    const unsigned long long w0 = clk.out_ptr() ? __builtin_readcyclecounter() : 0ull;
                    sync.poll(mem);
                    int spins = 0;
#pragma nounroll
                    for (; spins < 4 && !sync.slow_ok_a(); ++spins) {
                        __builtin_amdgcn_s_sleep(1);
                        sync.poll(mem);
                    }
#pragma nounroll
                    while (!sync.slow_ok_a()) {
                        __builtin_amdgcn_s_sleep(SLEEP_LONG);
                        sync.poll(mem);
                        ++spins;
                    }
                    sync.cover();
                    if (clk.out_ptr()) {
                        clk.polling += __builtin_readcyclecounter() - w0;
                        clk.waits += spins ? 1 : 0;
                    }
                };
                auto wait_b = [&](WP &join_read) {
                    const unsigned long long w0 = clk.out_ptr() ? __builtin_readcyclecounter() : 0ull;
                    const int need = sync.need_join_at(t);
                    sync.have_join = K::join == 2 ? mem.counter_and_get(sync.w_join, st.a_join, join_read) : mem.counter(sync.w_join);
                    int spins = 0;
#pragma nounroll
                    for (; spins < 4 && sync.have_join < need; ++spins) {
                        __builtin_amdgcn_s_sleep(1);
                        sync.have_join = K::join == 2 ? mem.counter_and_get(sync.w_join, st.a_join, join_read) : mem.counter(sync.w_join);
                    }
#pragma nounroll
                    while (sync.have_join < need) {
                        __builtin_amdgcn_s_sleep(SLEEP_LONG);
                        sync.have_join = K::join == 2 ? mem.counter_and_get(sync.w_join, st.a_join, join_read) : mem.counter(sync.w_join);
                        ++spins;
                    }
                    sync.cover_b();
                    if (clk.out_ptr()) {
                        clk.polling += __builtin_readcyclecounter() - w0;
                        clk.waits += spins ? 1 : 0;
                    }
                };
                if (__builtin_expect(!sync.ok_a(), 0)) wait_a();
                const WP ho = st.handed_over();
                const WP x_in{wave_shr1(ho.w), wave_shr1(ho.p)};
                WP join_read{0.f, 0.f};
                if (K::join == 2) join_read = mem.get(st.a_join);
                constexpr int t_first_mod = ((-2 - (int)PF) % (int)SKEW + (int)SKEW) % (int)SKEW;
                const int tmod = (t_first_mod + u) % (int)SKEW;
                if (SPLIT) {
                    const int step_no = t - t_first;
                    const int AHEAD = (GG_SWEEP_REC_AHEAD && u + 1 < (int)TRIP) ? 1 : 0;
                    if (__builtin_expect(have_prep <= step_no + AHEAD, 0)) {
                        have_prep = mem.counter(L.prep_done + SIDE);
                        while (have_prep <= step_no + AHEAD) {
                            __builtin_amdgcn_s_sleep(1);
                            have_prep = mem.counter(L.prep_done + SIDE);
                        }
                    }
                    const int rec_word = L.prep + (SIDE * (int)PREP_DEPTH * (int)LANES + lane) * (int)PREP_WORDS;
                    PrepRec rec;
                    if (GG_SWEEP_REC_AHEAD && u > 0) rec = rec_ahead;
                    else rec = mem.ring_get(rec_word + u * (int)LANES * (int)PREP_WORDS);
                    if (AHEAD) rec_ahead = mem.ring_get(rec_word + (u + 1) * (int)LANES * (int)PREP_WORDS);
                    st.template take<STARTS, K::bnd>(t, tmod, rec, x_in, group > 0, mem);
                    mem.set_counter(w_take, step_no + 1 + AHEAD);
                } else if constexpr (FRESH) {
                    static_assert((int)TRIP % 2 == 0, "the bit queue's slot is a constant of the unrolled trip");
                    const uint32_t w_own = mq_own[u & 1], w_out = mq_out[u & 1];
                    const uint32_t ahead = 8u * (unsigned)(t + 2 - t_first);
                    mq_own[u & 1] = mem.bits_dword(fo_own, ahead);
                    mq_out[u & 1] = mem.bits_dword(fo_out, ahead);
                    const bool own_bit = ((w_own >> sh_own) & 1u) != 0u, out_bit = ((w_out >> sh_out) & 1u) != 0u;
                    st.template step_a<STARTS, K::bnd, true>(t, u % (int)PF, tmod, x_in, P, L, K::bnd == 3 ? trip_bnd : group > 0, mem, own_bit, out_bit);
                } else {
                    st.template step_a<STARTS, K::bnd>(t, u % (int)PF, tmod, x_in, P, L, K::bnd == 3 ? trip_bnd : group > 0, mem);
                }
                if (__builtin_expect(!sync.ok_b(), 0)) wait_b(join_read);
                st.template step_b<STARTS, K::join>(t, tmod, P, L, K::join == 3 ? trip_pub : (SPLIT ? scalar_here(has_next) : has_next) != 0, group, mem,
                                                    SKEW != 1 || (SPLIT ? scalar_here(turn) : turn) == (u % 3), join_read, trip_join);
            }
        };
        if (SPLIT || GG_SWEEP_BATCH_KINDS >= 3) {
            const int bnd_until = min(st.u_len0, st.u_join_first);
            for (int tb = t_first; tb <= t_last;) {
                if (tb > st.u_start_last && tb >= st.u_join_first && (group == 0 || tb >= st.u_len0)) {
                    for (; tb <= t_last; tb += TRIP) trip(tb, TripKind<false, 0, 2>{});
                } else if (group > 0 && tb > st.u_start_last && tb + (int)TRIP - 1 < bnd_until) {
                    for (; tb <= t_last && tb + (int)TRIP - 1 < bnd_until; tb += TRIP) trip(tb, TripKind<false, 2, 0>{});
                } else {
                    trip(tb, TripKind<true, 1, 1>{});
                    tb += TRIP;
                }
            }
        } else {
            int tb = t_first;
#if GG_SWEEP_BATCH_KINDS >= 2
            for (; tb <= t_last && tb <= st.u_start_last; tb += TRIP) trip(tb, TripKind<true, GG_SWEEP_BATCH_RANGES, GG_SWEEP_BATCH_RANGES>{});
            for (; tb <= t_last; tb += TRIP) trip(tb, TripKind<false, GG_SWEEP_BATCH_RANGES, GG_SWEEP_BATCH_RANGES>{});
#else
            for (; tb <= t_last; tb += TRIP) trip(tb, TripKind<true, GG_SWEEP_BATCH_RANGES, GG_SWEEP_BATCH_RANGES>{});
#endif
        }
    }
}

template <int SIDE, bool DBG> GG_DEV void run_prep(const Params &P, const LdsMap &L, DevMemT<DBG> &mem, int lane, int group)
{
    PrepLane<SIDE> st;
    const int r0 = LANES * group + 1;
    const int nl = min(P.rings - (r0 - 1), (int)LANES);
    st.init(lane, r0, nl, P);
    static_assert((int)PREP_DEPTH == (int)TRIP, "a step's ring slot is its position in the trip");
    const int t_first = group_first_step(), t_last = group_last_step<SIDE>(r0, nl);
    int have_taken = 0;
    const int w_prep = lane == 0 ? L.prep_done + SIDE : ((L.scratch + 1 + 3 * lane) & ~1) + 2;
    for (int tb = t_first; tb <= t_last; tb += TRIP) {
#pragma unroll
        for (int u = 0; u < TRIP; ++u) {
            const int t = tb + u, step_no = t - t_first;
            if (step_no - have_taken >= (int)PREP_DEPTH) {
                have_taken = mem.counter(L.take_done + SIDE);
                while (step_no - have_taken >= (int)PREP_DEPTH) {
                    __builtin_amdgcn_s_sleep(2);
                    have_taken = mem.counter(L.take_done + SIDE);
                }
            }
            const PrepRec rec = st.step(t, u % (int)PF, P, mem);
            mem.ring_put(L.prep + ((SIDE * (int)PREP_DEPTH + u) * (int)LANES + lane) * (int)PREP_WORDS, rec);
            mem.set_counter(w_prep, step_no + 1);
        }
    }
}

template <int CD, bool DBG, bool FRESH = false> GG_DEV void run_corner(const Params &P, const LdsMap &L, DevMemT<DBG> &mem, int lane, WaveClockT<DBG> &clk, int g0, int g1)
{
    (void)clk;
    CornerRing<CD> st;
    for (int group = g0; group < g1; ++group) {
        const int r0 = LANES * group + 1;
        const int nl = min(P.rings - (r0 - 1), (int)LANES);
        st.template issue<FRESH>(r0 + lane, P, mem);
        st.finish(P, mem);
        if (group == g0 && g0 > 0)
            while (mem.counter(L.corner_done + CD) < r0 - 1) __builtin_amdgcn_s_sleep(SLEEP_LONG);
        const int prev = L.corner + 2 * ((CD * P.c + r0 - 1) * 2);
        WP in_corner = mem.get(prev + 2);
        WP in_x1 = r0 > 1 ? mem.get(prev) : WP{0.f, 0.f};
        for (int l = 0; l < nl; ++l) {
            if (CD && r0 + l == 1) {
                while (!CornerRing<CD>::ready(1, L, mem)) __builtin_amdgcn_s_sleep(1);
                in_x1 = mem.get(L.join + 2 * (SIDE_B * P.c + 1));
            }
            WP x1, y0;
            st.recur(lane == l, lane, in_corner, in_x1, P, L, mem, x1, y0);
            in_corner = mem.bcast(y0, l);
            in_x1 = mem.bcast(x1, l);
        }
    }
    mem.flush_marks();
}

template <bool DBG> GG_DEV void run_import(const Params &P, const LdsMap &L, DevMemT<DBG> &mem, int lane, int g0)
{
    const int gb = g0, rb = LANES * g0;
    {
        WP v{0.f, 0.f};
        bool ok = lane >= 4;
        for (int polls = 0;; ++polls) {
            if (!ok) ok = mem.import_wp(xchg_misc(gb, lane), v);
            if (__all(ok) || mem.give_up(polls, P)) break;
            __builtin_amdgcn_s_sleep(SLEEP_LONG);
        }
        if (lane < 4) mem.put(L.corner + 2 * (((lane >> 1) * P.c + rb) * 2) + 2 * (lane & 1), v);
        if (lane == 0) {
            mem.set_counter(L.corner_done + 0, rb);
            mem.set_counter(L.corner_done + 1, rb);
        }
    }
    bool joins = false;
    int done[4] = {0, 0, 0, 0};
    const int len[4] = {chain_len<SIDE_A>(rb), chain_len<SIDE_B>(rb), chain_len<SIDE_C>(rb), chain_len<SIDE_D>(rb)};
    for (int idle = 0;;) {
        bool all_done = joins, progress = false;
        if (!joins) {
            WP v{0.f, 0.f};
            const bool ok = lane >= 2 || mem.import_wp(xchg_misc(gb, X_JOIN_C + lane), v);
            if (__all(ok)) {
                if (lane < 2) mem.put(L.join + 2 * ((lane == 0 ? (int)SIDE_C : (int)SIDE_D) * P.c + rb), v);
                if (lane == 0) {
                    mem.set_counter(L.join_done + SIDE_C, rb);
                    mem.set_counter(L.join_done + SIDE_D, rb);
                }
                joins = true;
                progress = true;
            }
        }
#pragma unroll
        for (int side = 0; side < 4; ++side) {
            if (done[side] >= len[side]) continue;
            all_done = false;
            const int e = done[side] + lane;
            WP v{0.f, 0.f};
            const bool ok = e < len[side] && mem.import_wp(xchg_chain(gb, side, e), v);
            const unsigned long long m = __ballot(ok);
            const int nv = (~m == 0ull) ? 64 : __builtin_ctzll(~m);
            if (nv == 0) continue;
            if (lane < nv) mem.put(L.bnd + 2 * (side * L.bnd_stride + bnd_offset(g0 - 1) - L.bnd_base + e), v);
            done[side] += nv;
            if (lane == 0) mem.set_counter(L.bnd_done + side * P.groups + (g0 - 1), done[side]);
            progress = true;
        }
        if (all_done) break;
        idle = progress ? 0 : idle + 1;
        if (!progress) {
            if (mem.give_up(idle, P)) {
                if (lane == 0) {
                    mem.set_counter(L.join_done + SIDE_C, rb);
                    mem.set_counter(L.join_done + SIDE_D, rb);
                    for (int side = 0; side < 4; ++side) mem.set_counter(L.bnd_done + side * P.groups + (g0 - 1), len[side]);
                }
                break;
            }
            __builtin_amdgcn_s_sleep(SLEEP_LONG);
        }
    }
}

template <bool DBG> GG_DEV void run_export(const Params &P, const LdsMap &L, DevMemT<DBG> &mem, int lane, int g1)
{
    const int gb = g1, rb = LANES * g1;
    int sent[4] = {0, 0, 0, 0};
    const int len[4] = {chain_len<SIDE_A>(rb), chain_len<SIDE_B>(rb), chain_len<SIDE_C>(rb), chain_len<SIDE_D>(rb)};
    bool head = false, corners = false;
    for (;;) {
        bool all_done = head && corners, progress = false;
#pragma unroll
        for (int side = 0; side < 4; ++side) {
            if (sent[side] >= len[side]) continue;
            all_done = false;
            const int avail = mem.counter(L.bnd_done + side * P.groups + (g1 - 1));
            while (sent[side] < avail) {
                const int e = sent[side] + lane;
                if (e < avail) mem.export_wp_if(true, xchg_chain(gb, side, e), mem.get(L.bnd + 2 * (side * L.bnd_stride + bnd_offset(g1 - 1) - L.bnd_base + e)));
                sent[side] = min(sent[side] + (int)LANES, avail);
                progress = true;
            }
        }
        if (!corners) {
            int c0, c1, unused;
            mem.counters3(L.corner_done + 0, L.corner_done + 1, L.join_done + SIDE_C, c0, c1, unused);
            if (c0 >= rb && c1 >= rb) {
                if (lane < 4) mem.export_wp_if(true, xchg_misc(gb, lane), mem.get(L.corner + 2 * (((lane >> 1) * P.c + rb) * 2) + 2 * (lane & 1)));
                corners = true;
                progress = true;
            }
        }
        if (!head) {
            const int jc = mem.counter(L.join_done + SIDE_C), jd = mem.counter(L.join_done + SIDE_D);
            if (jc >= rb && jd >= rb) {
                if (lane < 2 && P.debug_fault != 2) mem.export_wp_if(true, xchg_misc(gb, X_JOIN_C + lane), mem.get(L.join + 2 * ((lane == 0 ? (int)SIDE_C : (int)SIDE_D) * P.c + rb)));
                head = true;
                progress = true;
            }
        }
        if (all_done) break;
        if (!progress) __builtin_amdgcn_s_sleep(SLEEP_LONG);
    }
}

template <bool DBG, bool PARTS, bool FRESH = false, bool SC = false>
__global__ __launch_bounds__(1024, 5) void k_sweep(const Arena a, const Params P_arg, const CloudParams *__restrict__ params, int n_clouds, int n_parts_rt,
                                                   unsigned long long *dbg)
{
    const int n_parts = PARTS ? n_parts_rt : 1;
    extern __shared__ __attribute__((aligned(16))) int lds[];
    uint32_t *s_sync = sweep_static;
    uint32_t *sync_words = a.sweep_sync;
    uint32_t id = blockIdx.x, epoch = 0u;
    if (PARTS) {
        if (threadIdx.x == 0) {
            s_sync[0] = __hip_atomic_fetch_add(sync_words + 0, 1u, __ATOMIC_RELAXED, __HIP_MEMORY_SCOPE_AGENT);
            s_sync[1] = __hip_atomic_load(sync_words + 2, __ATOMIC_RELAXED, __HIP_MEMORY_SCOPE_AGENT);
        }
        __syncthreads();
        id = s_sync[0];
        epoch = s_sync[1];
        if (P_arg.debug_fault == 1) id = gridDim.x - 1u - id;
    }
    int cloud, part;
    {
        const int full = n_clouds & ~7, tail = n_clouds - full;
        if ((int)id < full * n_parts) {
            const int rem = (int)id % (8 * n_parts);
            part = rem >> 3;
            cloud = ((int)id / (8 * n_parts)) * 8 + (rem & 7);
        } else {
            const int rem = (int)id - full * n_parts;
            part = rem / tail;
            cloud = full + rem % tail;
        }
    }
    const int g0 = part * P_arg.gpw, g1 = min(g0 + P_arg.gpw, P_arg.groups);
    const LdsMap L = lds_layout(P_arg.c, P_arg.groups, g0, g1, P_arg.split_steps != 0);
    const CloudParams &cp = params[cloud];
    Params P_own;
    if (SC) {
        P_own = P_arg;
        DevConfig c;
        load_cloud_config(a, cp.cfg_index, c);
        P_own.decrease = c.occupied_cells_decrease_factor;
        P_own.inv_decrease = c.inv_decrease;
        P_own.decay_fast = c.decay_fast;
    }
    const Params &P = SC ? P_own : P_arg;
    float2 *gp2 = gp2_ptr(a, cp.slot);
    float *percall = percall_ptr(a, cp.slot);
    const int nthreads = blockDim.x;

    for (int k = threadIdx.x; k < L.corner; k += nthreads) lds[k] = 0;
    if (PARTS && threadIdx.x == 0) sweep_wait_failed = 0u;
    const WP centre{1.0f, 1.0f * cp.base_z};
    if (threadIdx.x == 0) {
        if (part == 0) gp2[gp_index(P.gl, P.c, P.c)] = make_float2(cp.base_z, 1.0f);
        float *f = reinterpret_cast<float *>(lds);
        for (int side = 0; side < 2; ++side) {
            f[L.corner + 2 * ((side * P.c + 0) * 2) + 2] = centre.w;
            f[L.corner + 2 * ((side * P.c + 0) * 2) + 3] = centre.p;
        }
        for (int side = SIDE_C; side <= SIDE_D; ++side) {
            f[L.join + 2 * (side * P.c + 0)] = centre.w;
            f[L.join + 2 * (side * P.c + 0) + 1] = centre.p;
        }
    }
    if (FRESH) {
        const float2 init = gp2[a.gp_fresh_cell];
        const unsigned long long *bw = a.gp_bits + (size_t)cp.slot * a.gp_bits_stride;
        for (int k = (int)threadIdx.x + part * nthreads; k < a.gp_border_n; k += nthreads * n_parts) {
            const int e = a.gp_border[k];
            const unsigned q = (unsigned)e - 1u;
            if (((bw[q >> 6] >> (q & 63u)) & 1ull) == 0ull) gp2[e] = init;
        }
    }
    if (!P.keep_points) {
        const uint32_t *tile_live = a.tile_live + (size_t)cp.slot * a.tile_live_stride;
        const int lane_ = threadIdx.x & 63, wave_ = (int)(threadIdx.x >> 6) + part * (nthreads >> 6), nwaves = (nthreads >> 6) * n_parts;
        for (int rank = wave_; rank < a.g.T; rank += nwaves) {
            const uint32_t cols_live = tile_live[rank];
            if (!cols_live) continue;
            float *points = percall + percall_index(rank, PL_POINTS, 0);
#pragma unroll
            for (int k = 0; k < 4; ++k) {
                const int cell = lane_ + 64 * k;
                if ((cols_live >> live_bit(cell)) & 1u) points[cell] = 0.0f;
            }
        }
    }
    __syncthreads();

    DevMemT<DBG> mem;
    mem.rsrc = __builtin_amdgcn_make_buffer_rsrc(gp2, 0, FRESH ? (a.gp_bits_off + a.gp_bits_words) * 8 : P.gl.elems * 8, 0x00020000);
    mem.lds = (lds_int *)lds;
    mem.xchg = a.sweep_xchg + (size_t)cp.slot * a.sweep_xchg_stride;
    mem.seq = epoch;
    if (FRESH) mem.bits_byte0 = (uint32_t)a.gp_bits_off * 8u;
    const int wave = __builtin_amdgcn_readfirstlane((int)(threadIdx.x >> 6)), lane = (int)(threadIdx.x & 63u);
    const int W = P.waves_per_side;
    WaveClockT<DBG> clk;
    clk.out_rt = (DBG && dbg && blockIdx.x == 0) ? dbg : nullptr;
    mem.dbg_mode_rt = (DBG && dbg) ? (int)dbg[63] : 0;
    mem.marks = (DBG && dbg) ? dbg + 48 + ((threadIdx.x >> 6) & 1) * 6 : nullptr;
    clk.begin();
    const int side = wave & 3, w_of_side = wave >> 2;
    if (!FRESH && P.split_steps) {
        if (wave < 4) {
            if (side == SIDE_A) run_chain<SIDE_A, DBG, true>(P, L, mem, 0, lane, clk, g0, g1);
            else if (side == SIDE_B) run_chain<SIDE_B, DBG, true>(P, L, mem, 0, lane, clk, g0, g1);
            else if (side == SIDE_C) run_chain<SIDE_C, DBG, true>(P, L, mem, 0, lane, clk, g0, g1);
            else run_chain<SIDE_D, DBG, true>(P, L, mem, 0, lane, clk, g0, g1);
        } else if (wave < 8) {
            if (side == SIDE_A) run_prep<SIDE_A, DBG>(P, L, mem, lane, g0);
            else if (side == SIDE_B) run_prep<SIDE_B, DBG>(P, L, mem, lane, g0);
            else if (side == SIDE_C) run_prep<SIDE_C, DBG>(P, L, mem, lane, g0);
            else run_prep<SIDE_D, DBG>(P, L, mem, lane, g0);
        } else if (wave == 8)
            run_corner<0, DBG>(P, L, mem, lane, clk, g0, g1);
        else if (wave == 9)
            run_corner<1, DBG>(P, L, mem, lane, clk, g0, g1);
        else if (PARTS && wave == 10) {
            if (part > 0) run_import<DBG>(P, L, mem, lane, g0);
        } else if (PARTS && g1 < P.groups)
            run_export<DBG>(P, L, mem, lane, g1);
    } else if (wave < 4 * W && side == SIDE_A)
        run_chain<SIDE_A, DBG, false, FRESH>(P, L, mem, w_of_side, lane, clk, g0, g1);
    else if (wave < 4 * W && side == SIDE_B)
        run_chain<SIDE_B, DBG, false, FRESH>(P, L, mem, w_of_side, lane, clk, g0, g1);
    else if (wave < 4 * W && side == SIDE_C)
        run_chain<SIDE_C, DBG, false, FRESH>(P, L, mem, w_of_side, lane, clk, g0, g1);
    else if (wave < 4 * W)
        run_chain<SIDE_D, DBG, false, FRESH>(P, L, mem, w_of_side, lane, clk, g0, g1);
    else if (wave == 4 * W)
        run_corner<0, DBG, FRESH>(P, L, mem, lane, clk, g0, g1);
    else if (wave == 4 * W + 1)
        run_corner<1, DBG, FRESH>(P, L, mem, lane, clk, g0, g1);
    else if (PARTS && wave == 4 * W + 2) {
        if (part > 0) run_import<DBG>(P, L, mem, lane, g0);
    } else if (PARTS && g1 < P.groups)
        run_export<DBG>(P, L, mem, lane, g1);
    clk.end(wave, lane);
    if (PARTS) {
        __syncthreads();
        if (threadIdx.x == 0 && sweep_wait_failed) __hip_atomic_store(a.dev_error, (uint32_t)GG_DEVERR_SWEEP_WAIT, __ATOMIC_RELAXED, __HIP_MEMORY_SCOPE_SYSTEM);
        if (threadIdx.x == 0 && __hip_atomic_fetch_add(sync_words + 1, 1u, __ATOMIC_RELAXED, __HIP_MEMORY_SCOPE_AGENT) == gridDim.x - 1u) {
            __hip_atomic_store(sync_words + 0, 0u, __ATOMIC_RELAXED, __HIP_MEMORY_SCOPE_AGENT);
            __hip_atomic_store(sync_words + 1, 0u, __ATOMIC_RELAXED, __HIP_MEMORY_SCOPE_AGENT);
            uint32_t next = ((epoch + 1u) & 0x7FFFFFFFu) | (epoch & 0x80000000u);
            if ((next & 0x7FFFFFFFu) == 0u) next |= 1u;
            __hip_atomic_store(sync_words + 2, next, __ATOMIC_RELAXED, __HIP_MEMORY_SCOPE_AGENT);
        }
    }
}

static size_t parts_lds_bytes(const Params &P, int gpw, bool split = false)
{
    size_t words = 0;
    for (int g0 = 0; g0 < std::max(P.groups, 1); g0 += gpw)
        words = std::max(words, (size_t)lds_layout(P.c, P.groups, g0, std::min(g0 + gpw, P.groups), split).words);
    return words * 4;
}
size_t sweep_lds_bytes(const Params &P) { return parts_lds_bytes(P, 1); }
size_t sweep_xchg_entries(const Params &P) { return (size_t)xchg_entries(P.groups); }

bool sweep_takes_fresh(const Arena &a, const Params &P_in, int n_clouds)
{
    if (P_in.rings <= 0 || n_clouds <= SWEEP_PAIR_MAX_CLOUDS || a.tune_sweep_gpw || a.tune_sweep_split == 1 || a.tune_sweep_fault || a.tune_sweep_pair == 4) return false;
    Params P = P_in;
    const int n_groups = std::max(P.groups, 1);
    int n_parts = std::max(1, std::min(n_groups, SWEEP_LATENCY_MAX_CLOUDS / std::max(n_clouds, 1)));
    P.gpw = (n_groups + n_parts - 1) / n_parts;
    while (P.gpw > 1 && parts_lds_bytes(P, P.gpw) > 158 * 1024) --P.gpw;
    n_parts = (n_groups + P.gpw - 1) / P.gpw;
    const bool split = P.gpw == 1 && a.tune_sweep_split != 2 && n_clouds * n_parts <= SWEEP_LATENCY_MAX_CLOUDS && parts_lds_bytes(P, 1, true) <= 158 * 1024;
    return !split;
}

void launch_sweep(const Arena &a, const Params &P_in, const CloudParams *d_params, int n_clouds, hipStream_t s, unsigned long long *dbg)
{
    if (n_clouds == 0 || P_in.rings <= 0) return;
    const bool k_sweep_forced = a.tune_sweep_waves || a.tune_sweep_gpw || a.tune_sweep_split || a.tune_sweep_fault;
    if (!dbg && a.tune_sweep_pair != 2 && !k_sweep_forced) {
        if (a.tune_sweep_pair == 4 && !a.slot_cfg_launch && launch_sweep_pair_batch(a, P_in, d_params, n_clouds, s)) return;
        if (a.tune_sweep_pair != 4 && launch_sweep_pair(a, P_in, d_params, n_clouds, s)) return;
    }
    Params P = P_in;
    const int n_groups = std::max(P.groups, 1);
    int n_parts = std::max(1, std::min(n_groups, SWEEP_LATENCY_MAX_CLOUDS / std::max(n_clouds, 1)));
    P.gpw = (n_groups + n_parts - 1) / n_parts;
    if (a.tune_sweep_gpw > 0) P.gpw = std::min(a.tune_sweep_gpw, n_groups);
    while (P.gpw > 1 && parts_lds_bytes(P, P.gpw) > 158 * 1024) --P.gpw;
    n_parts = (n_groups + P.gpw - 1) / P.gpw;
    const int groups_per_part = std::min(P.gpw, n_groups);
    if (a.tune_sweep_waves > 0)
        P.waves_per_side = std::max(1, std::min(std::min(groups_per_part, 3), a.tune_sweep_waves));
    else if (n_clouds * n_parts <= SWEEP_LATENCY_MAX_CLOUDS)
        P.waves_per_side = std::max(1, std::min(groups_per_part, 3));
    else
        P.waves_per_side = std::min(P.waves_per_side, std::max(1, std::min(groups_per_part, 3)));
    P.split_steps = (P.gpw == 1 && a.tune_sweep_split != 2 && (a.tune_sweep_split == 1 || n_clouds * n_parts <= SWEEP_LATENCY_MAX_CLOUDS) &&
                     parts_lds_bytes(P, 1, true) <= 158 * 1024)
                        ? 1
                        : 0;
    if (P.split_steps) P.waves_per_side = 1;
    const size_t lds = parts_lds_bytes(P, P.gpw, P.split_steps != 0);
    static PerDeviceOnce big_lds;
    if (lds > 64 * 1024)
        big_lds.run([] {
            hipFuncSetAttribute(reinterpret_cast<const void *>(k_sweep<false, false>), hipFuncAttributeMaxDynamicSharedMemorySize, 160 * 1024 - 256);
            hipFuncSetAttribute(reinterpret_cast<const void *>(k_sweep<false, true>), hipFuncAttributeMaxDynamicSharedMemorySize, 160 * 1024 - 256);
            hipFuncSetAttribute(reinterpret_cast<const void *>(k_sweep<true, true>), hipFuncAttributeMaxDynamicSharedMemorySize, 160 * 1024 - 256);
            hipFuncSetAttribute(reinterpret_cast<const void *>(k_sweep<false, false, true>), hipFuncAttributeMaxDynamicSharedMemorySize, 160 * 1024 - 256);
            hipFuncSetAttribute(reinterpret_cast<const void *>(k_sweep<false, true, true>), hipFuncAttributeMaxDynamicSharedMemorySize, 160 * 1024 - 256);
            hipFuncSetAttribute(reinterpret_cast<const void *>(k_sweep<false, false, false, true>), hipFuncAttributeMaxDynamicSharedMemorySize, 160 * 1024 - 256);
            hipFuncSetAttribute(reinterpret_cast<const void *>(k_sweep<false, true, false, true>), hipFuncAttributeMaxDynamicSharedMemorySize, 160 * 1024 - 256);
            hipFuncSetAttribute(reinterpret_cast<const void *>(k_sweep<false, false, true, true>), hipFuncAttributeMaxDynamicSharedMemorySize, 160 * 1024 - 256);
            hipFuncSetAttribute(reinterpret_cast<const void *>(k_sweep<false, true, true, true>), hipFuncAttributeMaxDynamicSharedMemorySize, 160 * 1024 - 256);
        });
    P.fresh_cell = a.gp_fresh_cell;
    P.poll_cap = a.tune_sweep_poll_cap > 0 ? a.tune_sweep_poll_cap : 1 << 22;
    P.debug_fault = a.tune_sweep_fault;
    const int threads = P.split_steps ? 12 * 64 : (4 * P.waves_per_side + 2 + (n_parts > 1 ? 2 : 0)) * 64;
    if (dbg)
        hipLaunchKernelGGL((k_sweep<true, true>), dim3(n_clouds * n_parts), dim3(threads), lds, s, a, P, d_params, n_clouds, n_parts, dbg);
    else if (a.slot_cfg_launch) {
        if (a.fresh_launch && !P.split_steps && n_parts == 1)
            hipLaunchKernelGGL((k_sweep<false, false, true, true>), dim3(n_clouds), dim3(threads), lds, s, a, P, d_params, n_clouds, n_parts, dbg);
        else if (a.fresh_launch && !P.split_steps)
            hipLaunchKernelGGL((k_sweep<false, true, true, true>), dim3(n_clouds * n_parts), dim3(threads), lds, s, a, P, d_params, n_clouds, n_parts, dbg);
        else if (n_parts > 1)
            hipLaunchKernelGGL((k_sweep<false, true, false, true>), dim3(n_clouds * n_parts), dim3(threads), lds, s, a, P, d_params, n_clouds, n_parts, dbg);
        else
            hipLaunchKernelGGL((k_sweep<false, false, false, true>), dim3(n_clouds * n_parts), dim3(threads), lds, s, a, P, d_params, n_clouds, n_parts, dbg);
    } else if (a.fresh_launch && !P.split_steps && n_parts == 1)
        hipLaunchKernelGGL((k_sweep<false, false, true>), dim3(n_clouds), dim3(threads), lds, s, a, P, d_params, n_clouds, n_parts, dbg);
    else if (a.fresh_launch && !P.split_steps)
        hipLaunchKernelGGL((k_sweep<false, true, true>), dim3(n_clouds * n_parts), dim3(threads), lds, s, a, P, d_params, n_clouds, n_parts, dbg);
    else if (n_parts > 1)
        hipLaunchKernelGGL((k_sweep<false, true>), dim3(n_clouds * n_parts), dim3(threads), lds, s, a, P, d_params, n_clouds, n_parts, dbg);
    else
        hipLaunchKernelGGL((k_sweep<false, false>), dim3(n_clouds * n_parts), dim3(threads), lds, s, a, P, d_params, n_clouds, n_parts, dbg);
}

}
```

groundgrid_amd/csrc/sweep_core.h:

```cpp
#pragma once

#include <float.h>
#include <stdint.h>
#include <string.h>

#include "gp_layout.h"

#if defined(__HIPCC__)
#include <hip/hip_runtime.h>
#define SW_HD __host__ __device__ __forceinline__
#else
#define SW_HD inline
#endif

namespace gg {
namespace sweep {

enum { SIDE_A = 0, SIDE_B = 1, SIDE_C = 2, SIDE_D = 3 };
enum { LANES = 64, SKEW = GG_SWEEP_SKEW, PF = 3, TRIP = 6 };
static_assert(SKEW >= 1 && SKEW <= 3 && TRIP % SKEW == 0 && TRIP % PF == 0 && TRIP % 2 == 0, "the step code names t mod SKEW residues");

struct WP {
    float w, p;
};
struct Cell {
    float g, w;
};
struct PrepRec {
    float w_new;
    float own_g, own_w, own_p;
    float out_w, out_p;
};

struct Params {
    int n;
    int c;
    int rings;
    int groups;
    int waves_per_side;
    int gpw;
    int split_steps;
    int fresh_cell;
    int r2min;
    double decrease, inv_decrease;
    int decay_fast;
    int poll_cap;
    int debug_fault;
    int keep_points;
    GpLayout gl;
};

template <int SIDE> SW_HD int chain_len(int r) { return SIDE == SIDE_A ? 2 * r - 2 : SIDE == SIDE_D ? 2 * r : 2 * r - 1; }
template <int SIDE> SW_HD int chain_k0() { return (SIDE == SIDE_A || SIDE == SIDE_C) ? 2 : 1; }

template <int SIDE> SW_HD int side_cell(const Params &P, int r, int line, int j)
{
    const int rp = P.c - r, R = P.c + r;
    int x, y;
    if (SIDE == SIDE_A) {
        x = rp - line;
        y = rp + j;
    } else if (SIDE == SIDE_B) {
        x = rp + j;
        y = rp - line;
    } else if (SIDE == SIDE_C) {
        x = R + line;
        y = R - j;
    } else {
        x = R - j;
        y = R + line;
    }
    return gp_index(P.gl, x, y);
}

template <int SIDE> SW_HD int side_r2(int r, int j)
{
    const int a = (SIDE == SIDE_A || SIDE == SIDE_B) ? j - r : r - j;
    return r * r + a * a;
}

template <int SIDE> SW_HD constexpr int tree_pos(int line, int pos)
{
    return SIDE == SIDE_A   ? (2 - line) + 3 * pos
           : SIDE == SIDE_B ? pos + 3 * (2 - line)
           : SIDE == SIDE_C ? line + 3 * (2 - pos)
                            : (2 - pos) + 3 * line;
}

SW_HD float sw_tree9(const float *e) { return ((e[0] + e[1]) + (e[2] + e[3])) + ((e[4] + e[5]) + (e[6] + (e[7] + e[8]))); }
SW_HD double sw_max(double a, double b) { return (a < b) ? b : a; }

SW_HD float sw_maxf(float a, float b) { return (a < b) ? b : a; }
#if defined(__HIP_DEVICE_COMPILE__)
SW_HD bool sw_any(bool b) { return __any(b) != 0; }
#define SW_KEEP_BRANCH() __asm__ volatile("; rare path" ::: "memory")
#else
SW_HD bool sw_any(bool b) { return b; }
#define SW_KEEP_BRANCH() ((void)0)
#endif

SW_HD float decayed_confidence(float occupied, bool decay, const Params &P)
{
    const float floor_f = (float)0.001;
    const double x = (double)occupied;
    const double t = x - x * P.inv_decrease;
    uint64_t bits;
#if defined(__HIP_DEVICE_COMPILE__)
    bits = (uint64_t)__double_as_longlong(t);
#else
    memcpy(&bits, &t, 8);
#endif
    const uint32_t low = (uint32_t)bits & 0x1FFFFFFFu;
    const bool near_boundary = (low - (0x10000000u - 64u)) <= 128u;
    float d = sw_maxf((float)t, floor_f);
    const bool exact = (!P.decay_fast || near_boundary) && decay;
    if (sw_any(exact)) {
        SW_KEEP_BRANCH();
        const float de = (float)sw_max(x - x / P.decrease, 0.001);
        d = exact ? de : d;
    }
    return decay ? d : occupied;
}

SW_HD float interpolated_height(const float (&w)[9], const float (&p)[9], float height, float occupied)
{
    const float gvlSum = sw_tree9(w) + FLT_MIN;
    const float avg = sw_tree9(p) / gvlSum;
    return (1.0f - occupied) * avg + occupied * height;
}

#if defined(__HIP_DEVICE_COMPILE__)
typedef float sw_f2 __attribute__((ext_vector_type(2)));
SW_HD float interpolated_height2(const WP (&e)[9], float height, float occupied)
{
    sw_f2 v[9];
#pragma unroll
    for (int k = 0; k < 9; ++k) v[k] = sw_f2{e[k].w, e[k].p};
    const sw_f2 sum = ((v[0] + v[1]) + (v[2] + v[3])) + ((v[4] + v[5]) + (v[6] + (v[7] + v[8])));
    const float gvlSum = sum.x + FLT_MIN;
    const float avg = sum.y / gvlSum;
    return (1.0f - occupied) * avg + occupied * height;
}
#else
SW_HD float interpolated_height2(const WP (&e)[9], float height, float occupied)
{
    float w[9], p[9];
    for (int k = 0; k < 9; ++k) {
        w[k] = e[k].w;
        p[k] = e[k].p;
    }
    return interpolated_height(w, p, height, occupied);
}
#endif

SW_HD Cell visit(const float (&w)[9], const float (&p)[9], float height, float occupied, bool decay, const Params &P)
{
    Cell out;
    out.w = decayed_confidence(occupied, decay, P);
    out.g = interpolated_height(w, p, height, occupied);
    return out;
}

struct LdsMap {
    int corner_done;
    int join_done;
    int bnd_done;
    int prep_done;
    int take_done;
    int corner;
    int join;
    int bnd;
    int bnd_stride;
    int bnd_base;
    int scratch;
    int prep;
    int words;
};

SW_HD int bnd_offset(int b) { return 64 * b * (b + 1) + 2 * b; }

SW_HD int xchg_len(int gb) { return 2 * LANES * gb + 2; }
SW_HD int xchg_base(int gb)
{
    int o = 0;
    for (int g = 1; g < gb; ++g) o += 4 * xchg_len(g) + 6;
    return o;
}
SW_HD int xchg_entries(int groups) { return xchg_base(groups > 1 ? groups : 1); }
enum { X_CORNER = 0, X_JOIN_C = 4, X_JOIN_D = 5 };
SW_HD int xchg_chain(int gb, int side, int e) { return xchg_base(gb) + side * xchg_len(gb) + e; }
SW_HD int xchg_misc(int gb, int k) { return xchg_base(gb) + 4 * xchg_len(gb) + k; }

enum { PREP_DEPTH = TRIP, PREP_WORDS = 6 };
SW_HD LdsMap lds_layout(int c, int groups, int g0 = 0, int g1 = -1, bool split_steps = false)
{
    if (g1 < 0) g1 = groups;
    LdsMap m;
    int o = 0;
    m.corner_done = o;
    o += 2;
    m.join_done = o;
    o += 4;
    m.bnd_done = o;
    o += 4 * groups;
    m.prep_done = o;
    o += 4;
    m.take_done = o;
    o += 4;
    o = (o + 1) & ~1;
    m.corner = o;
    o += 2 * c * 2 * 2;
    m.join = o;
    o += 4 * c * 2;
    const int b_first = g0 > 0 ? g0 - 1 : 0, b_end = g1 < groups ? g1 : (g1 > 0 ? g1 - 1 : 0);
    m.bnd_base = bnd_offset(b_first);
    m.bnd_stride = bnd_offset(b_end > b_first ? b_end : b_first) - m.bnd_base;
    m.bnd = o;
    o += 4 * m.bnd_stride * 2;
    m.scratch = o;
    o += LANES * 3 + 1;
    o = (o + 1) & ~1;
    m.prep = o;
    if (split_steps) o += 4 * PREP_DEPTH * LANES * PREP_WORDS;
    m.words = o;
    return m;
}


template <int SIDE> struct ChainSync {
    enum { NEVER = 0x7fffffff, ALWAYS = 0x3fffffff };
    int t_;
    int safe_a, safe_b;
    int have_corner, have_join, have_bnd;
    int start_t0, start_r0, n_start;
    int join_t0, join_r0;
    int bnd_end;
    int w_corner, w_join, w_bnd;

    SW_HD void init(int r0, int nl, int group, const Params &P, const LdsMap &L)
    {
        const int b = SIDE == SIDE_A ? -2 : SIDE == SIDE_D ? 0 : -1;
        const int side_from = SIDE == SIDE_A ? SIDE_D : SIDE == SIDE_B ? SIDE_C : SIDE == SIDE_C ? SIDE_B : SIDE_A;
        w_corner = L.corner_done + ((SIDE == SIDE_A || SIDE == SIDE_B) ? 0 : 1);
        w_join = L.join_done + side_from;
        w_bnd = L.bnd_done + SIDE * P.groups + (group > 0 ? group - 1 : 0);
        have_corner = have_join = have_bnd = 0;
        int l1 = (1 - b + 1) / 2 - r0;
        if (l1 < 0) l1 = 0;
        n_start = l1 < nl ? nl - l1 : 0;
        start_t0 = l1 < nl ? SKEW * l1 : (int)NEVER;
        start_r0 = r0 + l1;
        join_t0 = l1 < nl ? (SKEW + 2) * l1 + 2 * r0 + b - 2 : (int)NEVER;
        join_r0 = (SIDE == SIDE_A || SIDE == SIDE_B) ? r0 + l1 - 1 : r0 + l1;
        bnd_end = group > 0 ? chain_len<SIDE>(r0) - 2 : 0;
        t_ = -2 - (int)PF;
        cover();
    }
    SW_HD int need_corner_at(int t) const
    {
        const int ds = t - start_t0;
        const int ks = (int)((unsigned)ds / (unsigned)SKEW), last = n_start - 1;
        return ds < 0 ? 0 : start_r0 + (ks < last ? ks : last);
    }
    SW_HD int need_join_at(int t) const
    {
        const int dj = t - join_t0;
        const int kj = (int)((unsigned)dj / ((unsigned)SKEW + 2u)), last = n_start - 1;
        return dj < 0 ? 0 : join_r0 + (kj < last ? kj : last);
    }
    SW_HD int need_bnd_at(int t) const
    {
        const int tb = t + 1 < bnd_end ? t + 1 : bnd_end;
        return tb > 0 ? tb : 0;
    }
    SW_HD void cover()
    {
        const int last = n_start - 1;
        int sc, kc = have_corner - start_r0;
        if (start_t0 == (int)NEVER || kc >= last) sc = ALWAYS;
        else if (kc < 0) sc = start_t0 - 1;
        else sc = start_t0 + (int)SKEW * kc + (int)SKEW - 1;
        const int sb = have_bnd >= bnd_end ? (int)ALWAYS : have_bnd - 1;
        safe_a = sc < sb ? sc : sb;
        cover_b();
    }
    SW_HD void cover_b()
    {
        const int kj = have_join - join_r0;
        if (join_t0 == (int)NEVER || kj >= n_start - 1) safe_b = ALWAYS;
        else if (kj < 0) safe_b = join_t0 - 1;
        else safe_b = join_t0 + ((int)SKEW + 2) * kj + (int)SKEW + 1;
    }
    SW_HD void advance(int t) { t_ = t; }
    SW_HD bool ok_a() const { return t_ <= safe_a; }
    SW_HD bool ok_b() const { return t_ <= safe_b; }
    SW_HD bool slow_ok_a() const { return have_corner >= need_corner_at(t_) && have_bnd >= need_bnd_at(t_); }
    SW_HD bool slow_ok_b() const { return have_join >= need_join_at(t_); }
    template <class Mem> SW_HD void poll(Mem &mem) { mem.counters3(w_corner, w_join, w_bnd, have_corner, have_join, have_bnd); }
    template <class Mem> SW_HD void refresh(Mem &mem)
    {
        poll(mem);
        cover();
    }
};

template <int SIDE> struct ChainLane {
    int l, r, len;
    int l3, lend;
    int lim;
    int ownA, outA;
    int xold_cell, own_end;
    int a_s0, a_s1, a_pred, a_join, a_bnd, a_pub;
    int r2c, r2r;
    int pb_word, pb_step, pb_cnt, pb_idle;
    int u_start_last;
    int u_join_first, u_join_last;
    int u_len0;
    int u_l3_last, u_lend_last;
    WP I[3], U[3], OP;
    float Sg, Sw, Sp, Ng, Nw, Np;
    WP xold;
    WP h1, h2, h3;
    Cell q_own[PF], q_out[PF];
    WP xa, cs0, cs1, cpred;
    float w_new_;
    bool xold_bit = true, end_bit = true;

    SW_HD void init(int lane, int r0, int nl, int group, const Params &P, const LdsMap &L)
    {
        l = lane;
        const bool live = lane < nl;
        r = live ? r0 + lane : r0;
        len = live ? chain_len<SIDE>(r) : 0;
        const int k0 = chain_k0<SIDE>();
        l3 = SKEW * l;
        lend = l3 + len;
        lim = len > 0 ? len + 2 : 0;
        const int own1 = side_cell<SIDE>(P, r, 0, 1), out1 = side_cell<SIDE>(P, r, 1, 1);
        ownA = own1 + 64 * (k0 - 1 - l3);
        outA = out1 + 64 * (k0 - 1 - l3);
        xold_cell = side_cell<SIDE>(P, r, -1, k0 + len);
        own_end = side_cell<SIDE>(P, r, 0, k0 + len);
        const int side = (SIDE == SIDE_A || SIDE == SIDE_B) ? 0 : 1;
        const int own_first = L.corner + 2 * ((side * P.c + r) * 2), own_second = own_first + 2;
        const int in_first = L.corner + 2 * ((side * P.c + r - 1) * 2), in_second = in_first + 2;
        const int side_from = SIDE == SIDE_A ? SIDE_D : SIDE == SIDE_B ? SIDE_C : SIDE == SIDE_C ? SIDE_B : SIDE_A;
        a_join = L.join + 2 * (side_from * P.c + ((SIDE == SIDE_A || SIDE == SIDE_B) ? r - 1 : r));
        a_pub = L.join + 2 * (SIDE * P.c + r);
        if (SIDE == SIDE_A) {
            a_s0 = in_second;
            a_s1 = in_first;
            a_pred = own_first;
        } else if (SIDE == SIDE_B) {
            a_s0 = own_first;
            a_s1 = in_second;
            a_pred = own_second;
        } else if (SIDE == SIDE_C) {
            a_s0 = in_second;
            a_s1 = r == 1 ? a_join : in_first;
            a_pred = own_first;
        } else {
            a_s0 = own_first;
            a_s1 = in_second;
            a_pred = own_second;
        }
        a_bnd = group > 0 ? L.bnd + 2 * (SIDE * L.bnd_stride + bnd_offset(group - 1) - L.bnd_base) : L.bnd;
        r2c = k0 - r - l3;
        r2r = r * r;
        pb_idle = (L.scratch + 1 + 3 * l) & ~1;
        pb_word = l == LANES - 1 ? L.bnd + 2 * ((SIDE * L.bnd_stride) + bnd_offset(group) - L.bnd_base - l3) : pb_idle;
        pb_step = l == LANES - 1 ? 2 : 0;
        pb_cnt = l == LANES - 1 ? L.bnd_done + SIDE * P.groups + group : pb_idle + 2;
        u_start_last = SKEW * (nl - 1);
        u_len0 = chain_len<SIDE>(r0);
        u_join_first = u_len0 - 2;
        u_l3_last = SKEW * (LANES - 1);
        u_lend_last = SKEW * (nl - 1) + chain_len<SIDE>(r0 + nl - 1);
        u_join_last = u_lend_last - 2;
        I[0] = I[1] = I[2] = U[0] = U[1] = U[2] = OP = xold = h1 = h2 = h3 = WP{0.f, 0.f};
        Sg = Sw = Sp = Ng = Nw = Np = 0.f;
        for (int k = 0; k < PF; ++k) q_own[k] = q_out[k] = Cell{0.f, 0.f};
    }

    SW_HD WP handed_over() const { return SKEW == 1 ? h1 : SKEW == 2 ? h2 : h3; }

    template <bool STARTS = true, int BND = 1, bool FRESH = false, class Mem>
    SW_HD void step_a(int t, int slot, int tmod, WP x_in, const Params &P, const LdsMap &L, bool has_prev_group, Mem &mem, bool own_bit = true, bool out_bit = true)
    {
        (void)L;
        const int ao = t + r2c;
        w_new_ = decayed_confidence(Nw, r2r + ao * ao >= P.r2min, P);
        WP c_bnd{0.f, 0.f};
        if (BND == 2 || (BND == 3 && has_prev_group) || (BND == 1 && has_prev_group && t >= 0 && t < u_len0)) c_bnd = mem.get(a_bnd + (l == 0 ? 2 * t : 0));
        if (STARTS && tmod == 0 && t >= 0 && t <= u_start_last) {
            cs0 = mem.get(a_s0);
            cs1 = mem.get(a_s1);
            cpred = mem.get(a_pred);
        }
        const unsigned ua = (unsigned)(t + 2 - l3);
        const bool col = ua < (unsigned)lim;
        const int own_col = ownA + 64 * (t + 1);
        int own_now = (int)ua == len + 1 ? own_end : own_col;
        own_now = ua == 0u ? xold_cell : own_now;
        const Cell own = mem.fresh(mem.load_value(q_own[slot], col, own_now));
        const Cell out = mem.fresh(mem.load_value(q_out[slot], col, outA + 64 * (t + 1)));
        const unsigned uq = ua + (unsigned)PF;
        const bool colq = uq < (unsigned)lim;
        const int own_colq = ownA + 64 * (t + 1 + PF);
        int own_req = (int)uq == len + 1 ? own_end : own_colq;
        own_req = uq == 0u ? xold_cell : own_req;
        int out_req = outA + 64 * (t + 1 + PF);
        if (FRESH) {
            bool ob = (int)uq == len + 1 ? end_bit : own_bit;
            ob = uq == 0u ? xold_bit : ob;
            own_req = ob ? own_req : P.fresh_cell;
            out_req = out_bit ? out_req : P.fresh_cell;
        }
        q_own[slot] = mem.load_issue(colq, own_req);
        q_out[slot] = mem.load_issue(colq, out_req);
        Sg = Ng;
        Sw = Nw;
        Sp = Np;
        Ng = own.g;
        Nw = own.w;
        Np = own.w * own.g;
        xold = (tmod == (2 * SKEW - 2) % SKEW && ua == 0u) ? WP{own.w, Np} : xold;
        U[0] = U[1];
        U[1] = U[2];
        U[2] = WP{out.w, out.w * out.g};
        xa = (BND != 0 && l == 0) ? c_bnd : x_in;
        xa = t + 1 == lend ? xold : xa;
    }

    template <bool STARTS = true, int BND = 1, class Mem>
    SW_HD void take(int t, int tmod, const PrepRec &rec, WP x_in, bool has_prev_group, Mem &mem)
    {
        w_new_ = rec.w_new;
        WP c_bnd{0.f, 0.f};
        if (BND == 2 || (BND == 3 && has_prev_group) || (BND == 1 && has_prev_group && t >= 0 && t < u_len0)) c_bnd = mem.get(a_bnd + (l == 0 ? 2 * t : 0));
        if (STARTS && tmod == 0 && t >= 0 && t <= u_start_last) {
            cs0 = mem.get(a_s0);
            cs1 = mem.get(a_s1);
            cpred = mem.get(a_pred);
        }
        const unsigned ua = (unsigned)(t + 2 - l3);
        Sg = Ng;
        Sw = Nw;
        Sp = Np;
        Ng = rec.own_g;
        Nw = rec.own_w;
        Np = rec.own_p;
        xold = (tmod == (2 * SKEW - 2) % SKEW && ua == 0u) ? WP{rec.own_w, rec.own_p} : xold;
        U[0] = U[1];
        U[1] = U[2];
        U[2] = WP{rec.out_w, rec.out_p};
        xa = (BND != 0 && l == 0) ? c_bnd : x_in;
        xa = t + 1 == lend ? xold : xa;
    }

    template <bool STARTS = true, int JOIN = 1, class Mem>
    SW_HD void step_b(int t, int tmod, const Params &P, const LdsMap &L, bool has_next_group, int group, Mem &mem, bool join_turn = true, WP join_read = WP{0.f, 0.f},
                      bool trip_join = true)
    {
        WP x = xa;
        if (JOIN == 2 || (JOIN == 3 && trip_join) || (JOIN == 1 && t >= u_join_first && t <= u_join_last)) {
            const WP c_join = JOIN == 2 ? join_read : mem.get(a_join);
            x = t + 2 == lend ? c_join : x;
        }
        I[0] = I[1];
        I[1] = I[2];
        I[2] = x;
        if (STARTS && tmod == 0 && t >= 0 && t <= u_start_last) {
            const bool first = t == l3;
            I[0] = first ? cs0 : I[0];
            I[1] = first ? cs1 : I[1];
            OP = first ? cpred : OP;
        }
        const bool active = (unsigned)(t - l3) < (unsigned)len;
        WP win[9];
        win[tree_pos<SIDE>(0, 0)] = I[0];
        win[tree_pos<SIDE>(0, 1)] = I[1];
        win[tree_pos<SIDE>(0, 2)] = I[2];
        win[tree_pos<SIDE>(1, 0)] = OP;
        win[tree_pos<SIDE>(1, 1)] = WP{Sw, Sp};
        win[tree_pos<SIDE>(1, 2)] = WP{Nw, Np};
        win[tree_pos<SIDE>(2, 0)] = U[0];
        win[tree_pos<SIDE>(2, 1)] = U[1];
        win[tree_pos<SIDE>(2, 2)] = U[2];
        Cell v;
        v.w = w_new_;
        v.g = interpolated_height2(win, Sg, Sw);
        mem.store(active, ownA + 64 * t, v);
        const WP res = WP{v.w, v.w * v.g};
        OP = active ? res : OP;
        h3 = h2;
        h2 = h1;
        h1 = res;
        if (join_turn) mem.publish_if(t + 1 == lend && len > 0, l, L, a_pub, res, L.join_done + SIDE, r);
        if (has_next_group && (!STARTS || JOIN == 3 || (t >= u_l3_last && t < u_lend_last)))
            mem.publish(active ? pb_word + pb_step * t : pb_idle, res, active ? pb_cnt : pb_idle + 2, t - l3 + 1);
    }
};

template <int SIDE> struct PrepLane {
    int l3, len, lim, ownA, outA, xold_cell, own_end, r2c, r2r;
    float Nw;
    Cell q_own[PF], q_out[PF];
    SW_HD void init(int lane, int r0, int nl, const Params &P)
    {
        const bool live = lane < nl;
        const int r = live ? r0 + lane : r0;
        len = live ? chain_len<SIDE>(r) : 0;
        const int k0 = chain_k0<SIDE>();
        l3 = SKEW * lane;
        lim = len > 0 ? len + 2 : 0;
        ownA = side_cell<SIDE>(P, r, 0, 1) + 64 * (k0 - 1 - l3);
        outA = side_cell<SIDE>(P, r, 1, 1) + 64 * (k0 - 1 - l3);
        xold_cell = side_cell<SIDE>(P, r, -1, k0 + len);
        own_end = side_cell<SIDE>(P, r, 0, k0 + len);
        r2c = k0 - r - l3;
        r2r = r * r;
        Nw = 0.f;
        for (int k = 0; k < PF; ++k) q_own[k] = q_out[k] = Cell{0.f, 0.f};
    }
    template <class Mem> SW_HD PrepRec step(int t, int slot, const Params &P, Mem &mem)
    {
        PrepRec rec;
        const int ao = t + r2c;
        rec.w_new = decayed_confidence(Nw, r2r + ao * ao >= P.r2min, P);
        const unsigned ua = (unsigned)(t + 2 - l3);
        const bool col = ua < (unsigned)lim;
        int own_now = (int)ua == len + 1 ? own_end : ownA + 64 * (t + 1);
        own_now = ua == 0u ? xold_cell : own_now;
        const Cell own = mem.fresh(mem.load_value(q_own[slot], col, own_now));
        const Cell out = mem.fresh(mem.load_value(q_out[slot], col, outA + 64 * (t + 1)));
        const unsigned uq = ua + (unsigned)PF;
        const bool colq = uq < (unsigned)lim;
        int own_req = (int)uq == len + 1 ? own_end : ownA + 64 * (t + 1 + PF);
        own_req = uq == 0u ? xold_cell : own_req;
        q_own[slot] = mem.load_issue(colq, own_req);
        q_out[slot] = mem.load_issue(colq, outA + 64 * (t + 1 + PF));
        Nw = own.w;
        rec.own_g = own.g;
        rec.own_w = own.w;
        rec.own_p = own.w * own.g;
        rec.out_w = out.w;
        rec.out_p = out.w * out.g;
        return rec;
    }
};

template <int SIDE> SW_HD int join_turn_residue(int r0) { return (((chain_len<SIDE>(r0) - 1) % 3) + 3) % 3; }
SW_HD bool join_turn_of(int t, int residue) { return SKEW != 1 || ((t % 3) + 3) % 3 == residue; }

SW_HD int group_first_step() { return -2 - PF; }
template <int SIDE> SW_HD int group_last_step(int r0, int nl) { return SKEW * (nl - 1) + chain_len<SIDE>(r0 + nl - 1) - 1; }

template <int CD> struct CornerRing {
    int r;
    bool live;
    Cell q[3][4];
    int e00, e0m1;
    float g00, g0m1;
    float ow[3][4], op[3][4];
    float x0w, x1w, y0w;

    SW_HD static int cell_at(const Params &P, int r, int a, int b)
    {
        const int o = CD ? 1 : -1, z = P.c + o * r;
        if (r < 3) return gp_index(P.gl, z + o * a, z + o * b);
        const int ring = r + (a >= b ? a : b);
        const int g = (ring - 1) >> 6, l = (ring - 1) & 63;
        const int side = CD ? (a >= b ? 2 : 3) : (a >= b ? 0 : 1);
        const int along = a >= b ? b : a;
        const int v = CD ? P.n - 1 - (z + along) : z - along;
        return 1 + ((side * P.gl.G + g) * P.gl.VS + v + GP_SHEAR * l) * 64 + l;
    }
    SW_HD static bool is_old(int r, int a, int b)
    {
        return !(a == -1 && b == -1) && !(a == -1 && b == -2 && !(r == 1 && !CD));
    }
    SW_HD static int q9(int a, int b, int ca, int cb)
    {
        const int o = CD ? 1 : -1;
        return (o * (a - ca) + 1) + 3 * (o * (b - cb) + 1);
    }

    template <bool FRESH = false, class Mem> SW_HD void issue(int ring, const Params &P, Mem &mem)
    {
        live = ring <= P.rings;
        r = live ? ring : P.rings;
        for (int a = -1; a <= 1; ++a)
            for (int b = -2; b <= 1; ++b) {
                int cell = cell_at(P, r, a, b);
                if constexpr (FRESH) cell = mem.bit_of(cell) ? cell : P.fresh_cell;
                q[a + 1][b + 2] = mem.load_issue(live && is_old(r, a, b), cell);
            }
        e00 = cell_at(P, r, 0, 0);
        e0m1 = cell_at(P, r, 0, -1);
    }
    template <class Mem> SW_HD void finish(const Params &P, Mem &mem)
    {
        for (int a = -1; a <= 1; ++a)
            for (int b = -2; b <= 1; ++b) {
                const Cell v = mem.load_value(q[a + 1][b + 2], live && is_old(r, a, b), cell_at(P, r, a, b));
                ow[a + 1][b + 2] = v.w;
                op[a + 1][b + 2] = v.w * v.g;
                if (a == 0 && b == 0) g00 = v.g;
                if (a == 0 && b == -1) g0m1 = v.g;
            }
        const bool decay0 = 2 * r * r >= P.r2min, decay1 = r * r + (r - 1) * (r - 1) >= P.r2min;
        x0w = decayed_confidence(ow[1][2], decay0, P);
        x1w = decayed_confidence(ow[1][1], decay1, P);
        y0w = decayed_confidence(x0w, decay0, P);
    }
    template <class Mem>
    SW_HD void recur(bool mine, int lane, WP in_corner, WP in_x1_ring, const Params &P, const LdsMap &L, Mem &mem, WP &x1_out, WP &y0_out)
    {
        const WP in_x1 = (r == 1 && !CD) ? WP{ow[0][0], op[0][0]} : in_x1_ring;
        WP win[9];
        for (int a = -1; a <= 1; ++a)
            for (int b = -1; b <= 1; ++b) win[q9(a, b, 0, 0)] = (a == -1 && b == -1) ? in_corner : WP{ow[a + 1][b + 2], op[a + 1][b + 2]};
        const float x0g = interpolated_height2(win, g00, ow[1][2]);
        const WP x0{x0w, x0w * x0g};
        for (int a = -1; a <= 1; ++a)
            for (int b = -2; b <= 0; ++b)
                win[q9(a, b, 0, -1)] = (a == 0 && b == 0) ? x0 : (a == -1 && b == -1) ? in_corner : (a == -1 && b == -2) ? in_x1 : WP{ow[a + 1][b + 2], op[a + 1][b + 2]};
        const float x1g = interpolated_height2(win, g0m1, ow[1][1]);
        const WP x1{x1w, x1w * x1g};
        for (int a = -1; a <= 1; ++a)
            for (int b = -1; b <= 1; ++b)
                win[q9(a, b, 0, 0)] = (a == 0 && b == 0) ? x0 : (a == 0 && b == -1) ? x1 : (a == -1 && b == -1) ? in_corner : WP{ow[a + 1][b + 2], op[a + 1][b + 2]};
        const float y0g = interpolated_height2(win, x0g, x0w);
        const WP y0{y0w, y0w * y0g};
        mem.store(mine, e00, Cell{y0g, y0w});
        mem.store(mine, e0m1, Cell{x1g, x1w});
        const int base = L.corner + 2 * ((CD * P.c + r) * 2);
        mem.put_if(mine, lane, L, base, x1);
        mem.publish_if(mine, lane, L, base + 2, y0, L.corner_done + CD, r);
        if (!CD)
            mem.publish_if(mine && r == 1, lane, L, L.join + 2 * (SIDE_A * P.c + 1), x1, L.join_done + SIDE_A, 1);
        x1_out = x1;
        y0_out = y0;
    }
    template <class Mem> SW_HD static bool ready(int ring, const LdsMap &L, Mem &mem)
    {
        return !(CD && ring == 1) || mem.counter(L.join_done + SIDE_B) >= 1;
    }
};

}
}
```

groundgrid_amd/csrc/sweep_emul.hip:

```cpp
#include <stdio.h>
#include <stdlib.h>
#include <string.h>

#include <vector>
#include <cstdlib>
#include <algorithm>

#include "groundgrid_hip.h"
#include "sweep_core.h"

namespace {

using namespace gg::sweep;

struct HostMem {
    Cell *gp2;
    const std::vector<uint64_t> *bits = nullptr;
    bool bit_of(int cell) const { return cell <= 0 || (((*bits)[(size_t)(cell - 1) >> 6] >> ((cell - 1) & 63)) & 1ull) != 0ull; }
    std::vector<int32_t> lds;
    bool late;
    long loads = 0, stores = 0, lds_ops = 0;
    std::vector<uint64_t> *xchg = nullptr;
    uint32_t seq = 1;
    void export_wp_if(bool c, int entry, WP v)
    {
        if (!c) return;
        uint32_t w, p;
        memcpy(&w, &v.w, 4);
        memcpy(&p, &v.p, 4);
        (*xchg)[2 * (size_t)entry] = ((uint64_t)seq << 32) | w;
        (*xchg)[2 * (size_t)entry + 1] = ((uint64_t)seq << 32) | p;
    }
    bool import_wp(int entry, WP &v)
    {
        const uint64_t a = (*xchg)[2 * (size_t)entry], b = (*xchg)[2 * (size_t)entry + 1];
        const uint32_t w = (uint32_t)a, p = (uint32_t)b;
        memcpy(&v.w, &w, 4);
        memcpy(&v.p, &p, 4);
        return (uint32_t)(a >> 32) == seq && (uint32_t)(b >> 32) == seq;
    }
    void set_counter(int word, int value) { lds[(size_t)word] = value; }
    void ring_put(int word, const PrepRec &r)
    {
        ++lds_ops;
        memcpy(&lds[(size_t)word], &r, sizeof r);
    }
    PrepRec ring_get(int word)
    {
        ++lds_ops;
        PrepRec r;
        memcpy(&r, &lds[(size_t)word], sizeof r);
        return r;
    }
    Cell load_issue(bool valid, int cell)
    {
        if (!valid) return Cell{0.f, 0.f};
        ++loads;
        return gp2[cell];
    }
    Cell load_value(const Cell &queued, bool valid, int cell) { return (late && valid) ? gp2[cell] : queued; }
    Cell fresh(const Cell &v) { return v; }
    void mark(int) {}
    void store(bool valid, int cell, Cell v)
    {
        if (!valid) return;
        ++stores;
        gp2[cell] = v;
    }
    int counter(int word) { return lds[(size_t)word]; }
    void counters3(int w0, int w1, int w2, int &v0, int &v1, int &v2)
    {
        v0 = counter(w0);
        v1 = counter(w1);
        v2 = counter(w2);
    }
    void put(int word, WP v)
    {
        ++lds_ops;
        memcpy(&lds[(size_t)word], &v, sizeof v);
    }
    WP get(int word)
    {
        ++lds_ops;
        WP v;
        memcpy(&v, &lds[(size_t)word], sizeof v);
        return v;
    }
    void publish(int data_word, WP v, int counter_word, int value)
    {
        put(data_word, v);
        lds[(size_t)counter_word] = value;
    }
    void put_if(bool c, int, const LdsMap &, int word, WP v)
    {
        if (c) put(word, v);
    }
    void publish_if(bool c, int, const LdsMap &, int data_word, WP v, int counter_word, int value)
    {
        if (c) publish(data_word, v, counter_word, value);
    }
};

struct WaveBase {
    virtual ~WaveBase() {}
    virtual bool bad() const { return false; }
    virtual bool done() const = 0;
    virtual bool try_step() = 0;
};

template <int SIDE> struct ChainWave : WaveBase {
    const Params &P;
    const LdsMap &L;
    HostMem &mem;
    int g1;
    int wave, group, t, t_last, r0, nl;
    ChainLane<SIDE> lane[LANES];
    ChainSync<SIDE> sync;
    bool advanced = false;
    long steps = 0;
    bool plan_mismatch = false;
    ChainWave(const Params &p, const LdsMap &l, HostMem &m, int w, int g0_, int g1_) : P(p), L(l), mem(m), g1(g1_), wave(w), group(g0_ + w - p.waves_per_side) { next_group(); }
    void next_group()
    {
        group += P.waves_per_side;
        if (group >= g1) return;
        r0 = LANES * group + 1;
        nl = P.rings - (r0 - 1) < LANES ? P.rings - (r0 - 1) : LANES;
        for (int l = 0; l < LANES; ++l) {
            lane[l].init(l, r0, nl, group, P, L);
            const ChainLane<SIDE> &c = lane[l];
            const int k0 = chain_k0<SIDE>();
            for (int j = k0; j <= k0 + c.len - 1; ++j)
                if (c.ownA + 64 * (c.l3 + j - k0) != side_cell<SIDE>(P, c.r, 0, j)) plan_mismatch = true;
            for (int j = k0 - 1; c.len > 0 && j <= k0 + c.len; ++j)
                if (c.outA + 64 * (c.l3 + j - k0) != side_cell<SIDE>(P, c.r, 1, j)) plan_mismatch = true;
            if (l > 0 && l < nl && c.len > 0 && lane[l - 1].len > 0 && c.ownA != lane[l - 1].ownA + 1) plan_mismatch = true;
        }
        if (mem.bits)
            for (int l = 0; l < LANES; ++l) {
                lane[l].xold_bit = mem.bit_of(lane[l].xold_cell);
                lane[l].end_bit = mem.bit_of(lane[l].own_end);
            }
        t = group_first_step();
        t_last = group_last_step<SIDE>(r0, nl);
        t_last += (TRIP - (t_last - t + 1) % TRIP) % TRIP;
        sync.init(r0, nl, group, P, L);
        advanced = false;
    }
    bool done() const override { return group >= g1; }
    bool bad() const override { return plan_mismatch; }
    bool half = false;
    bool try_step() override
    {
        if (done()) return false;
        const int tmod = ((t % SKEW) + SKEW) % SKEW;
        if (!half) {
            if (!advanced) {
                sync.advance(t);
                advanced = true;
            }
            if (sync.ok_a() != sync.slow_ok_a()) plan_mismatch = true;
            if (!sync.ok_a()) {
                sync.refresh(mem);
                if (sync.ok_a() != sync.slow_ok_a()) plan_mismatch = true;
                if (!sync.ok_a()) return false;
            }
            for (int l = 0; l < nl; ++l) {
                const ChainLane<SIDE> &c = lane[l];
                if (c.len > 0 && t - c.l3 == 0 && mem.counter(sync.w_corner) < c.r) plan_mismatch = true;
            }
            if (group > 0 && t >= 0 && t + 2 < lane[0].len && mem.counter(sync.w_bnd) < t + 1) plan_mismatch = true;
            const int step_no = t - group_first_step();
            if (P.split_steps && mem.counter(L.prep_done + SIDE) <= step_no) return false;
            WP x_in[LANES];
            for (int l = 0; l < LANES; ++l) x_in[l] = l ? lane[l - 1].handed_over() : WP{0.f, 0.f};
            const int slot = ((t % PF) + PF) % PF;
            if (P.split_steps) {
                for (int l = 0; l < LANES; ++l)
                    lane[l].take(t, tmod, mem.ring_get(L.prep + ((SIDE * PREP_DEPTH + (step_no % PREP_DEPTH)) * LANES + l) * PREP_WORDS), x_in[l], group > 0, mem);
                mem.set_counter(L.take_done + SIDE, step_no + 1);
            } else if (mem.bits) {
                for (int l = 0; l < LANES; ++l) {
                    const int eo = lane[l].ownA + 64 * (t + 1 + (int)PF), eu = lane[l].outA + 64 * (t + 1 + (int)PF);
                    const bool in_o = eo >= 1 && eo < P.gl.elems, in_u = eu >= 1 && eu < P.gl.elems;
                    lane[l].template step_a<true, 1, true>(t, slot, tmod, x_in[l], P, L, group > 0, mem, in_o && mem.bit_of(eo), in_u && mem.bit_of(eu));
                }
            } else {
                for (int l = 0; l < LANES; ++l) lane[l].step_a(t, slot, tmod, x_in[l], P, L, group > 0, mem);
            }
            half = true;
        }
        if (sync.ok_b() != sync.slow_ok_b()) plan_mismatch = true;
        if (!sync.ok_b()) {
            sync.refresh(mem);
            if (sync.ok_b() != sync.slow_ok_b()) plan_mismatch = true;
            if (!sync.ok_b()) return false;
        }
        for (int l = 0; l < nl; ++l) {
            const ChainLane<SIDE> &c = lane[l];
            const int s_ = t - c.l3;
            if (c.len > 0 && s_ == c.len - 2 && s_ >= -1 && mem.counter(sync.w_join) < ((SIDE == SIDE_A || SIDE == SIDE_B) ? c.r - 1 : c.r)) plan_mismatch = true;
        }
        for (int l = 0; l < LANES; ++l) lane[l].step_b(t, tmod, P, L, group + 1 < P.groups, group, mem, join_turn_of(t, join_turn_residue<SIDE>(r0)));
        half = false;
        ++steps;
        advanced = false;
        if (++t > t_last) next_group();
        return true;
    }
};

template <int CD> struct CornerWave : WaveBase {
    const Params &P;
    const LdsMap &L;
    HostMem &mem;
    int g0, g1;
    int r;
    int r_end;
    bool prepared = false;
    CornerRing<CD> lane[LANES];
    WP in_corner{0.f, 0.f}, in_x1{0.f, 0.f};
    CornerWave(const Params &p, const LdsMap &l, HostMem &m, int g0_, int g1_)
        : P(p), L(l), mem(m), g0(g0_), g1(g1_), r(LANES * g0_ + 1), r_end(LANES * g1_ < p.rings ? LANES * g1_ : p.rings) {}
    bool done() const override { return r > r_end; }
    bool try_step() override
    {
        if (done() || !CornerRing<CD>::ready(r, L, mem)) return false;
        const int l = (r - 1) % LANES, r0 = r - l;
        if (!prepared) {
            if (g0 > 0 && r0 == LANES * g0 + 1 && mem.counter(L.corner_done + CD) < r0 - 1) return false;
            for (int k = 0; k < LANES; ++k) {
                if (mem.bits) lane[k].template issue<true>(r0 + k, P, mem);
                else lane[k].issue(r0 + k, P, mem);
            }
            for (int k = 0; k < LANES; ++k) lane[k].finish(P, mem);
            const int prev = L.corner + 2 * ((CD * P.c + r0 - 1) * 2);
            in_corner = mem.get(prev + 2);
            in_x1 = r0 > 1 ? mem.get(prev) : WP{0.f, 0.f};
            prepared = true;
        }
        if (CD && r == 1) in_x1 = mem.get(L.join + 2 * (SIDE_B * P.c + 1));
        WP x1, y0;
        lane[l].recur(true, l, in_corner, in_x1, P, L, mem, x1, y0);
        in_corner = y0;
        in_x1 = x1;
        ++r;
        if (l == LANES - 1) prepared = false;
        return true;
    }
};

template <int SIDE> struct PrepWave : WaveBase {
    const Params &P;
    const LdsMap &L;
    HostMem &mem;
    int group, r0, nl, t, t_last;
    PrepLane<SIDE> lane[LANES];
    PrepWave(const Params &p, const LdsMap &l, HostMem &m, int g) : P(p), L(l), mem(m), group(g)
    {
        r0 = LANES * group + 1;
        nl = P.rings - (r0 - 1) < LANES ? P.rings - (r0 - 1) : LANES;
        for (int k = 0; k < LANES; ++k) lane[k].init(k, r0, nl, P);
        t = group_first_step();
        t_last = group_last_step<SIDE>(r0, nl);
        t_last += (TRIP - (t_last - t + 1) % TRIP) % TRIP;
    }
    bool done() const override { return t > t_last; }
    bool try_step() override
    {
        if (done()) return false;
        const int step_no = t - group_first_step();
        if (step_no - mem.counter(L.take_done + SIDE) >= PREP_DEPTH) return false;
        const int slot = ((t % PF) + PF) % PF;
        for (int k = 0; k < LANES; ++k)
            mem.ring_put(L.prep + ((SIDE * PREP_DEPTH + (step_no % PREP_DEPTH)) * LANES + k) * PREP_WORDS, lane[k].step(t, slot, P, mem));
        mem.set_counter(L.prep_done + SIDE, step_no + 1);
        ++t;
        return true;
    }
};

struct ExportWave : WaveBase {
    const Params &P;
    const LdsMap &L;
    HostMem &mem;
    int g1;
    bool head = false, corners = false;
    int sent[4] = {0, 0, 0, 0}, len[4];
    ExportWave(const Params &p, const LdsMap &l, HostMem &m, int g1_) : P(p), L(l), mem(m), g1(g1_)
    {
        const int rb = LANES * g1;
        len[0] = chain_len<SIDE_A>(rb), len[1] = chain_len<SIDE_B>(rb), len[2] = chain_len<SIDE_C>(rb), len[3] = chain_len<SIDE_D>(rb);
    }
    bool done() const override { return head && corners && sent[0] >= len[0] && sent[1] >= len[1] && sent[2] >= len[2] && sent[3] >= len[3]; }
    bool try_step() override
    {
        const int rb = LANES * g1;
        bool progress = false;
        for (int side = 0; side < 4; ++side) {
            const int avail = mem.counter(L.bnd_done + side * P.groups + (g1 - 1));
            for (; sent[side] < avail; ++sent[side], progress = true)
                mem.export_wp_if(true, xchg_chain(g1, side, sent[side]), mem.get(L.bnd + 2 * (side * L.bnd_stride + bnd_offset(g1 - 1) - L.bnd_base + sent[side])));
        }
        if (!corners && mem.counter(L.corner_done + 0) >= rb && mem.counter(L.corner_done + 1) >= rb) {
            for (int k = 0; k < 4; ++k) mem.export_wp_if(true, xchg_misc(g1, k), mem.get(L.corner + 2 * (((k >> 1) * P.c + rb) * 2) + 2 * (k & 1)));
            corners = true;
            progress = true;
        }
        if (!head && mem.counter(L.join_done + SIDE_C) >= rb && mem.counter(L.join_done + SIDE_D) >= rb) {
            for (int k = 0; k < 2; ++k) mem.export_wp_if(true, xchg_misc(g1, X_JOIN_C + k), mem.get(L.join + 2 * ((k == 0 ? (int)SIDE_C : (int)SIDE_D) * P.c + rb)));
            head = true;
            progress = true;
        }
        return progress;
    }
};

struct ImportWave : WaveBase {
    const Params &P;
    const LdsMap &L;
    HostMem &mem;
    int g0;
    bool head = false, joins = false;
    int have[4] = {0, 0, 0, 0}, len[4];
    ImportWave(const Params &p, const LdsMap &l, HostMem &m, int g0_) : P(p), L(l), mem(m), g0(g0_)
    {
        const int rb = LANES * g0;
        len[0] = chain_len<SIDE_A>(rb), len[1] = chain_len<SIDE_B>(rb), len[2] = chain_len<SIDE_C>(rb), len[3] = chain_len<SIDE_D>(rb);
    }
    bool done() const override { return head && joins && have[0] >= len[0] && have[1] >= len[1] && have[2] >= len[2] && have[3] >= len[3]; }
    bool try_step() override
    {
        const int rb = LANES * g0;
        if (!head) {
            WP v[4];
            for (int k = 0; k < 4; ++k)
                if (!mem.import_wp(xchg_misc(g0, k), v[k])) return false;
            for (int k = 0; k < 4; ++k) mem.put(L.corner + 2 * (((k >> 1) * P.c + rb) * 2) + 2 * (k & 1), v[k]);
            mem.set_counter(L.corner_done + 0, rb);
            mem.set_counter(L.corner_done + 1, rb);
            head = true;
            return true;
        }
        bool progress = false;
        if (!joins) {
            WP c, d;
            if (mem.import_wp(xchg_misc(g0, X_JOIN_C), c) && mem.import_wp(xchg_misc(g0, X_JOIN_D), d)) {
                mem.put(L.join + 2 * (SIDE_C * P.c + rb), c);
                mem.put(L.join + 2 * (SIDE_D * P.c + rb), d);
                mem.set_counter(L.join_done + SIDE_C, rb);
                mem.set_counter(L.join_done + SIDE_D, rb);
                joins = true;
                progress = true;
            }
        }
        for (int side = 0; side < 4; ++side) {
            int nv = 0;
            WP v;
            while (nv < LANES && have[side] + nv < len[side] && mem.import_wp(xchg_chain(g0, side, have[side] + nv), v)) {
                mem.put(L.bnd + 2 * (side * L.bnd_stride + bnd_offset(g0 - 1) - L.bnd_base + have[side] + nv), v);
                ++nv;
            }
            if (nv) {
                have[side] += nv;
                mem.set_counter(L.bnd_done + side * P.groups + (g0 - 1), have[side]);
                progress = true;
            }
        }
        return progress;
    }
};

}

namespace gg {
namespace sweep {

Params make_params(int n, double resolution, float min_dist_squared, double decrease)
{
    Params P;
    P.n = n;
    P.c = n / 2 - 1;
    P.rings = P.c - 1 > 0 ? P.c - 1 : 0;
    P.groups = (P.rings + LANES - 1) / LANES;
    P.waves_per_side = P.groups <= 1 ? 1 : P.groups <= 3 ? 2 : 3;
    P.split_steps = 0;
    P.poll_cap = 1 << 22;
    P.debug_fault = 0;
    P.keep_points = 0;
    P.fresh_cell = 0;
    P.gpw = P.groups > 1 ? P.groups : 1;
    if (getenv("GG_SWEEP_WAVES")) P.waves_per_side = std::max(1, std::min(std::min(P.groups, 3), atoi(getenv("GG_SWEEP_WAVES"))));
    int r2 = 0;
    while (r2 < 2 * n * n && !((double)r2 * (resolution * resolution) > (double)min_dist_squared)) ++r2;
    P.r2min = r2;
    P.decrease = decrease;
    P.inv_decrease = 1.0 / decrease;
    P.decay_fast = decrease >= 1.25 && decrease < 1e300;
    P.gl = make_gp_layout(n);
    return P;
}

}
}

namespace {
template <int SIDE> long sync_mismatches(const Params &P)
{
    long bad = 0;
    const LdsMap L = lds_layout(P.c, P.groups);
    for (int group = 0; group < std::max(P.groups, 1); ++group) {
        const int r0 = LANES * group + 1, nl = std::min(P.rings - (r0 - 1), (int)LANES);
        if (nl <= 0) break;
        const int t_last = group_last_step<SIDE>(r0, nl) + TRIP, top = r0 + nl + 2, bnd_top = chain_len<SIDE>(r0) + 2;
        for (int which = 0; which < 3; ++which)
            for (int have = 0; have <= (which == 2 ? bnd_top : top); ++have) {
                ChainSync<SIDE> sy;
                sy.init(r0, nl, group, P, L);
                sy.have_corner = which == 0 ? have : top;
                sy.have_join = which == 1 ? have : top;
                sy.have_bnd = which == 2 ? have : bnd_top;
                sy.cover();
                for (int t = group_first_step(); t <= t_last; ++t) {
                    sy.advance(t);
                    bad += sy.ok_a() != sy.slow_ok_a();
                    bad += sy.ok_b() != sy.slow_ok_b();
                }
            }
    }
    return bad;
}
}

extern "C" long gg_debug_sweep_sync_selftest(int n)
{
    if (n < 8) return -1;
    const Params P = gg::sweep::make_params(n, 0.33, 12.0f, 10.0);
    return sync_mismatches<SIDE_A>(P) + sync_mismatches<SIDE_B>(P) + sync_mismatches<SIDE_C>(P) + sync_mismatches<SIDE_D>(P);
}

static int emulate_ring_sweep(int n, double resolution, float min_dist_squared, float *gp2, float base_z, double decrease, unsigned seed, int late_loads, long *stats,
                              const unsigned char *patched, float fresh_ground)
{
    if (n < 8 || !gp2) return GG_ERR_INVALID;
    Params P = gg::sweep::make_params(n, resolution, min_dist_squared, decrease);
    P.fresh_cell = 1 + (P.gl.VS - 1) * 64;
    if (getenv("GG_SWEEP_GPW")) {
        P.gpw = std::max(1, std::min(atoi(getenv("GG_SWEEP_GPW")), std::max(P.groups, 1)));
        P.waves_per_side = std::max(1, std::min(P.waves_per_side, P.gpw));
        if (getenv("GG_SWEEP_SPLIT") && atoi(getenv("GG_SWEEP_SPLIT")) && P.gpw == 1) P.split_steps = 1;
    }
    const int n_groups = std::max(P.groups, 1), n_parts = (n_groups + P.gpw - 1) / P.gpw;
    std::vector<Cell> sheared((size_t)P.gl.elems, Cell{0.f, 0.f});
    for (int col = 0; col < n; ++col)
        for (int row = 0; row < n; ++row) sheared[(size_t)gp_index(P.gl, row, col)] = Cell{gp2[2 * ((size_t)row + (size_t)col * n)], gp2[2 * ((size_t)row + (size_t)col * n) + 1]};
    std::vector<uint64_t> bits;
    if (patched) {
        if (late_loads) return GG_ERR_INVALID;
        bits.assign((size_t)P.gl.elems / 64 + 2, 0ull);
        const float poison = __builtin_nanf("");
        for (int col = 0; col < n; ++col)
            for (int row = 0; row < n; ++row) {
                const int e = gp_index(P.gl, row, col);
                if (patched[(size_t)row + (size_t)col * n] && e > 0) bits[(size_t)(e - 1) >> 6] |= 1ull << ((e - 1) & 63);
                else sheared[(size_t)e] = Cell{poison, poison};
            }
        sheared[(size_t)P.fresh_cell] = Cell{fresh_ground, (float)0.0000001};
        for (int col = 0; col < n; ++col)
            for (int row = 0; row < n; ++row)
                if (std::max(std::abs(row - P.c), std::abs(col - P.c)) >= P.c && !patched[(size_t)row + (size_t)col * n])
                    sheared[(size_t)gp_index(P.gl, row, col)] = sheared[(size_t)P.fresh_cell];
    }
    std::vector<uint64_t> xchg(2 * (size_t)std::max(xchg_entries(P.groups), 1), 0ull);
    std::vector<LdsMap> maps((size_t)n_parts);
    std::vector<HostMem> mems((size_t)n_parts);
    sheared[(size_t)gp_index(P.gl, P.c, P.c)] = Cell{base_z, 1.0f};
    const WP centre{1.0f, 1.0f * base_z};
    std::vector<WaveBase *> waves;
    size_t lds_words = 0;
    for (int part = 0; part < n_parts; ++part) {
        const int g0 = part * P.gpw, g1 = std::min(g0 + P.gpw, P.groups);
        LdsMap &L = maps[(size_t)part];
        HostMem &mem = mems[(size_t)part];
        L = lds_layout(P.c, P.groups, g0, g1, P.split_steps != 0);
        lds_words = std::max(lds_words, (size_t)L.words);
        mem.gp2 = sheared.data();
        mem.bits = patched ? &bits : nullptr;
        mem.lds.assign((size_t)L.words, 0);
        mem.late = late_loads != 0;
        mem.xchg = &xchg;
        mem.seq = 7;
        for (int side = 0; side < 2; ++side) mem.put(L.corner + 2 * ((side * P.c + 0) * 2) + 2, centre);
        mem.put(L.join + 2 * (SIDE_C * P.c + 0), centre);
        mem.put(L.join + 2 * (SIDE_D * P.c + 0), centre);
        for (int w = 0; w < P.waves_per_side; ++w) waves.push_back(new ChainWave<SIDE_A>(P, L, mem, w, g0, g1));
        for (int w = 0; w < P.waves_per_side; ++w) waves.push_back(new ChainWave<SIDE_B>(P, L, mem, w, g0, g1));
        for (int w = 0; w < P.waves_per_side; ++w) waves.push_back(new ChainWave<SIDE_C>(P, L, mem, w, g0, g1));
        for (int w = 0; w < P.waves_per_side; ++w) waves.push_back(new ChainWave<SIDE_D>(P, L, mem, w, g0, g1));
        if (P.split_steps) {
            waves.push_back(new PrepWave<SIDE_A>(P, L, mem, g0));
            waves.push_back(new PrepWave<SIDE_B>(P, L, mem, g0));
            waves.push_back(new PrepWave<SIDE_C>(P, L, mem, g0));
            waves.push_back(new PrepWave<SIDE_D>(P, L, mem, g0));
        }
        waves.push_back(new CornerWave<0>(P, L, mem, g0, g1));
        waves.push_back(new CornerWave<1>(P, L, mem, g0, g1));
        if (part > 0) waves.push_back(new ImportWave(P, L, mem, g0));
        if (g1 < P.groups) waves.push_back(new ExportWave(P, L, mem, g1));
    }

    uint32_t rng = seed * 2654435761u + 12345u;
    auto rnd = [&]() { return rng = rng * 1664525u + 1013904223u; };
    long total_steps = 0, stalls = 0, rounds = 0;
    int rc = GG_OK;
    for (;;) {
        bool all_done = true, progress = false;
        for (auto *w : waves) all_done &= w->done();
        if (all_done) break;
        ++rounds;
        if (seed == 0) {
            for (auto *w : waves)
                if (w->try_step()) {
                    progress = true;
                    ++total_steps;
                } else if (!w->done())
                    ++stalls;
        } else {
            for (int tries = 0; tries < 4 * (int)waves.size() && !progress; ++tries) {
                WaveBase *w = waves[(rnd() >> 8) % waves.size()];
                const uint32_t mode = (rnd() >> 8) % 8;
                int burst = mode == 0 ? 1 << 30 : mode < 4 ? 1 + (int)((rnd() >> 8) % 64) : 1;
                while (burst-- > 0 && w->try_step()) {
                    progress = true;
                    ++total_steps;
                }
                if (!progress && !w->done()) ++stalls;
            }
            if (!progress)
                for (auto *w : waves)
                    if (w->try_step()) {
                        progress = true;
                        ++total_steps;
                        break;
                    }
        }
        if (!progress) {
            rc = -10;
            break;
        }
    }
    if (getenv("GG_EMUL_VERBOSE")) fprintf(stderr, "ring sweep emulation: n %d, %ld scheduler rounds, %ld wave-steps, %ld stalls\n", n, rounds, total_steps, stalls);
    if (stats) {
        stats[0] = total_steps;
        stats[1] = stalls;
        stats[2] = stats[3] = stats[4] = 0;
        for (const HostMem &m : mems) {
            stats[2] += m.loads;
            stats[3] += m.stores;
            stats[4] += m.lds_ops;
        }
        stats[5] = (long)lds_words * 4;
        stats[6] = (P.waves_per_side * 4 + 2) * n_parts + 2 * (n_parts - 1);
        stats[7] = P.r2min;
    }
    for (auto *w : waves) {
        if (w->bad() && rc == GG_OK) rc = -11;
        delete w;
    }
    for (int col = 0; col < n; ++col)
        for (int row = 0; row < n; ++row) {
            const Cell v = sheared[(size_t)gp_index(P.gl, row, col)];
            gp2[2 * ((size_t)row + (size_t)col * n)] = v.g;
            gp2[2 * ((size_t)row + (size_t)col * n) + 1] = v.w;
        }
    return rc;
}

extern "C" int gg_debug_emulate_ring_sweep(int n, double resolution, float min_dist_squared, float *gp2, float base_z, double decrease,
                                           unsigned seed, int late_loads, long *stats)
{
    return emulate_ring_sweep(n, resolution, min_dist_squared, gp2, base_z, decrease, seed, late_loads, stats, nullptr, 0.0f);
}
extern "C" int gg_debug_emulate_ring_sweep_fresh(int n, double resolution, float min_dist_squared, float *gp2, const unsigned char *patched, float fresh_ground, float base_z,
                                                 double decrease, unsigned seed, long *stats)
{
    if (!patched) return GG_ERR_INVALID;
    return emulate_ring_sweep(n, resolution, min_dist_squared, gp2, base_z, decrease, seed, 0, stats, patched, fresh_ground);
}

#include "sweep_pair.h"

namespace {
namespace gp = gg::sweep::pair;

struct PairHostMem {
    Cell *layer;
    std::vector<float> *out;
    void emit(int slot, float g)
    {
        ++stores;
        (*out)[(size_t)slot] = g;
    }
    std::vector<int32_t> lds;
    long stores = 0, lds_ops = 0;
    bool fault = false;
    float lds_f(int word)
    {
        ++lds_ops;
        float v;
        memcpy(&v, &lds[(size_t)word], 4);
        return v;
    }
    void lds_put(int word, float v)
    {
        ++lds_ops;
        memcpy(&lds[(size_t)word], &v, 4);
    }
    void lds_put2(int word, float v0, float v1)
    {
        if (word & 1) fault = true;
        lds_put(word, v0);
        lds_put(word + 1, v1);
    }
    void lds_entry(int word, float v)
    {
        lds_put(word, v);
        lds[(size_t)word + 1] = 1;
    }
    int lds_i(int word) { return lds[(size_t)word]; }
    void lds_set(int word, int v) { lds[(size_t)word] = v; }
    void store(bool valid, int cell, Cell v)
    {
        if (!valid) return;
        ++stores;
        layer[cell] = v;
    }
};

struct Records {
    std::vector<float> visit;
    std::vector<gp::CornerRec> corner;
};

template <int PAIR> struct PairWave : WaveBase {
    const Params &P;
    const gp::Plan &pl;
    const gp::Lds &L;
    PairHostMem &mem;
    const Records &rec;
    float centre_p;
    int W, group, t, t_end;
    gp::Group G;
    gp::PairLane<PAIR> lane[64];
    bool plan_mismatch = false;
    PairWave(const Params &p, const gp::Plan &pl_, const gp::Lds &l, PairHostMem &m, const Records &r, float cp, int w, int W_)
        : P(p), pl(pl_), L(l), mem(m), rec(r), centre_p(cp), W(W_), group(w - W_)
    {
        next_group();
    }
    void next_group()
    {
        group += W;
        if (group >= pl.groups) return;
        G = gp::group_of(PAIR, group, P.rings);
        for (int k = 0; k < 64; ++k) {
            lane[k].init(k, group, G, P, pl, L);
            const gp::PairLane<PAIR> &c = lane[k];
            const int side = c.is_x ? gp::side_x(PAIR) : gp::side_y(PAIR);
            for (int s = 0; s < c.len; ++s) {
                int x, y;
                gp::side_xy(side, P.c, c.r, 0, gp::k0_of(side) + s, x, y);
                if (c.st_base + 64 * (c.start + s) != gp_index(P.gl, x, y)) plan_mismatch = true;
                int slot = -1;
                if (!gp::chain_slot_of_cell(P, pl, x, y, slot) || slot != gp::out_slot(c.out_step0 + c.start + s, c.lane_)) plan_mismatch = true;
            }
        }
        t = G.t_first;
        t_end = G.t_first + G.steps;
    }
    bool done() const override { return group >= pl.groups; }
    bool bad() const override { return plan_mismatch || mem.fault; }
    bool try_step() override
    {
        if (done()) return false;
        for (int k = 0; k < 64; ++k) {
            const gp::PairLane<PAIR> &c = lane[k];
            if (c.first_at(t) && mem.lds_i(L.cnt_corner + c.cd) < c.r) return false;
            if (c.imports_at(t, group) && mem.lds_i(c.import_entry(t) + 1) == 0) return false;
            if (c.join_from_lds_at(t, group) && mem.lds_i(c.a_jl + 1) == 0) return false;
        }
        for (int k = 0; k < 64; ++k) lane[k].pre(t, mem);
        float x_prev[64], j_perm[64];
        for (int k = 0; k < 64; ++k) {
            x_prev[k] = k ? lane[k - 1].h2 : 0.f;
            j_perm[k] = k < 32 ? (k ? lane[32 + k - 1].h1 : 0.f) : lane[k - 32].h1;
        }
        const int step = pl.base[PAIR][group] + (t - G.t_first);
        for (int k = 0; k < 64; ++k) lane[k].step(t, group, gp::rec_at(rec.visit.data(), step, k), gp::rec_at(rec.visit.data(), step + 1, k), x_prev[k], j_perm[k], centre_p, mem);
        if (++t >= t_end) next_group();
        return true;
    }
};

template <int CD> struct PairCornerWave : WaveBase {
    const Params &P;
    const gp::Plan &pl;
    const gp::Lds &L;
    PairHostMem &mem;
    const Records &rec;
    float centre_p;
    int r = 1;
    gp::CornerLane<CD> lane[64];
    float in_corner, in_x1 = 0.f;
    PairCornerWave(const Params &p, const gp::Plan &pl_, const gp::Lds &l, PairHostMem &m, const Records &rc, float cp) : P(p), pl(pl_), L(l), mem(m), rec(rc), centre_p(cp), in_corner(cp) {}
    bool done() const override { return r > P.rings; }
    bool try_step() override
    {
        if (done()) return false;
        if (CD && r == 1) {
            if (mem.lds_i(L.b1 + 1) == 0) return false;
            in_x1 = mem.lds_f(L.b1);
        }
        const int k = (r - 1) % 64;
        if (k == 0)
            for (int j = 0; j < 64; ++j) {
                const int ring = r + j;
                lane[j].init(ring, P, rec.corner[(size_t)CD * (P.rings + 1) + (ring <= P.rings ? ring : P.rings)]);
            }
        float x1g, x1, y0g, y0;
        lane[k].visits(in_corner, in_x1, x1g, x1, y0g, y0);
        lane[k].keep(true, x1g, y0g);
        lane[k].flush(true, mem);
        gp::CornerLane<CD>::publish(r, x1, y0, P, L, mem);
        if (!CD && r == 1) {
            const int st0 = pl.base[gp::PAIR_BC][0] + (0 - gp::group_of(gp::PAIR_BC, 0, P.rings).t_first);
            const float *v = rec.visit.data();
            mem.lds_entry(L.b1, gp::b1_of_ring1(gp::rec_at(v, st0 - 2, 0), gp::rec_at(v, st0 - 1, 0), gp::rec_at(v, st0, 0), gp::rec_at(v, st0 + 1, 0), x1, y0, centre_p));
        }
        in_corner = y0;
        in_x1 = x1;
        ++r;
        return true;
    }
};

}

extern "C" int gg_debug_emulate_pair_sweep(int n, double resolution, float min_dist_squared, float *gp2, float base_z, double decrease, unsigned seed, int n_wgs,
                                           int waves_per_pair, long *stats)
{
    if (n < 8 || !gp2) return GG_ERR_INVALID;
    const Params P = gg::sweep::make_params(n, resolution, min_dist_squared, decrease);
    const gp::Plan pl = gp::make_plan(P.rings);
    if (pl.groups <= 0) return GG_ERR_INVALID;
    std::vector<Cell> sheared((size_t)P.gl.elems, Cell{0.f, 0.f});
    for (int col = 0; col < n; ++col)
        for (int row = 0; row < n; ++row) sheared[(size_t)gp_index(P.gl, row, col)] = Cell{gp2[2 * ((size_t)row + (size_t)col * n)], gp2[2 * ((size_t)row + (size_t)col * n) + 1]};
    Records rec;
    const float poison = __builtin_nanf("");
    rec.visit.assign(((size_t)pl.total_steps / 4 + 1) * gp::QUAD_BLOCK_FLOATS, poison);
    auto load = [&](int x, int y) { return sheared[(size_t)gp_index(P.gl, x, y)]; };
    long n_visits = 0;
    for (int p = 0; p < 2; ++p)
        for (int g = 0; g < pl.groups; ++g) {
            const gp::Group G = gp::group_of(p, g, P.rings);
            for (int t0 = G.t_first; t0 < G.t_first + G.steps; t0 += gp::QUAD)
                for (int lane = 0; lane < 64; ++lane) {
                    const bool is_x = lane < 32;
                    const int l = lane & 31, side = is_x ? gp::side_x(p) : gp::side_y(p);
                    if (l >= G.nl) continue;
                    const int r = G.r0 + l, len = gp::len_of(side, r), s0 = t0 - (2 * l + gp::start0(p, is_x));
                    if (s0 + 3 < -(int)gp::WARMUP || s0 > len) continue;
                    float q[gp::QUAD_FLOATS];
                    gp::make_visit_quad(P, p, is_x, r, s0, load, q);
                    const int step = pl.base[p][g] + (t0 - G.t_first);
                    for (int i = 0; i < 4; ++i) {
                        const int s = s0 + i;
                        if (s < -(int)gp::WARMUP || s > len) continue;
                        float *w = rec.visit.data() + gp::quad_word(step + i, lane, i);
                        w[0] = q[4 * i], w[1] = q[4 * i + 1], w[2] = q[4 * i + 2], w[3] = q[4 * i + 3];
                        rec.visit[(size_t)gp::quad_word(step + i, lane, 4) + i] = q[16 + i];
                        n_visits += s >= 0 && s < len;
                    }
                }
        }
    rec.corner.resize(2 * (size_t)(P.rings + 1));
    for (int r = 1; r <= P.rings; ++r) {
        rec.corner[(size_t)r] = gp::make_corner_rec<0>(P, r, load);
        rec.corner[(size_t)(P.rings + 1) + r] = gp::make_corner_rec<1>(P, r, load);
    }
    sheared[(size_t)gp_index(P.gl, P.c, P.c)] = Cell{base_z, 1.0f};
    const float centre_p = 1.0f * base_z;
    std::vector<float> out((size_t)pl.total_steps * 64, poison);
    if (n_wgs != 2) n_wgs = 1;
    const gp::Lds L = gp::lds_of(P.c, pl, n_wgs == 1);
    const int W = std::max(1, std::min(waves_per_pair > 0 ? waves_per_pair : pl.groups, pl.groups));
    std::vector<PairHostMem> mems((size_t)n_wgs);
    std::vector<WaveBase *> waves;
    for (int wg = 0; wg < n_wgs; ++wg) {
        PairHostMem &mem = mems[(size_t)wg];
        mem.layer = sheared.data();
        mem.out = &out;
        mem.lds.assign((size_t)L.words, 0);
        for (int k = 0; k < 64; ++k) mem.lds[(size_t)L.scratch + 2 * k + 1] = 1;
        for (int cd = 0; cd < 2; ++cd) mem.lds_put(gp::corner_word(L, P.c, cd, 0, 1), centre_p);
        for (int w = 0; w < W; ++w) {
            if (n_wgs == 1 || wg == 0) waves.push_back(new PairWave<gp::PAIR_AD>(P, pl, L, mem, rec, centre_p, w, W));
            if (n_wgs == 1 || wg == 1) waves.push_back(new PairWave<gp::PAIR_BC>(P, pl, L, mem, rec, centre_p, w, W));
        }
        waves.push_back(new PairCornerWave<0>(P, pl, L, mem, rec, centre_p));
        waves.push_back(new PairCornerWave<1>(P, pl, L, mem, rec, centre_p));
    }
    uint32_t rng = seed * 2654435761u + 12345u;
    auto rnd = [&]() { return rng = rng * 1664525u + 1013904223u; };
    long total_steps = 0, stalls = 0;
    int rc = GG_OK;
    for (;;) {
        bool all_done = true, progress = false;
        for (auto *w : waves) all_done &= w->done();
        if (all_done) break;
        if (seed == 0) {
            for (auto *w : waves)
                if (w->try_step()) {
                    progress = true;
                    ++total_steps;
                } else if (!w->done())
                    ++stalls;
        } else {
            for (int tries = 0; tries < 4 * (int)waves.size() && !progress; ++tries) {
                WaveBase *w = waves[(rnd() >> 8) % waves.size()];
                const uint32_t mode = (rnd() >> 8) % 8;
                int burst = mode == 0 ? 1 << 30 : mode < 4 ? 1 + (int)((rnd() >> 8) % 64) : 1;
                while (burst-- > 0 && w->try_step()) {
                    progress = true;
                    ++total_steps;
                }
                if (!progress && !w->done()) ++stalls;
            }
            if (!progress)
                for (auto *w : waves)
                    if (w->try_step()) {
                        progress = true;
                        ++total_steps;
                        break;
                    }
        }
        if (!progress) {
            rc = -10;
            break;
        }
    }
    long finished = 0, cells_seen = 0;
    for (int e = 0; e < P.gl.elems; ++e) {
        int x, y, slot;
        if (!gg::gp_cell_of(P.gl, e, x, y)) continue;
        ++cells_seen;
        if (!gp::chain_slot_of_cell(P, pl, x, y, slot)) continue;
        sheared[(size_t)e] = gp::finished_cell(P, x, y, sheared[(size_t)e].w, out[(size_t)slot]);
        ++finished;
    }
    if ((finished != n_visits || cells_seen != (long)n * n) && rc == GG_OK) rc = -12;
    if (stats) {
        stats[0] = total_steps;
        stats[1] = stalls;
        stats[2] = n_visits;
        stats[3] = 0;
        for (const PairHostMem &m : mems) stats[3] += m.stores;
        stats[4] = (long)L.words * 4;
        stats[5] = (long)waves.size();
        stats[6] = pl.total_steps;
        stats[7] = pl.groups;
    }
    for (auto *w : waves) {
        if (w->bad() && rc == GG_OK) rc = -11;
        delete w;
    }
    for (int col = 0; col < n; ++col)
        for (int row = 0; row < n; ++row) {
            const Cell v = sheared[(size_t)gp_index(P.gl, row, col)];
            gp2[2 * ((size_t)row + (size_t)col * n)] = v.g;
            gp2[2 * ((size_t)row + (size_t)col * n) + 1] = v.w;
        }
    return rc;
}
// ... 268 lines not shown
```

Before: 217,200.

## Stage fresh-map patch bits in LDS for the single-workgroup sweep

For fresh-map sweeps that run as one work-group per cloud, the kernel now copies the per-cloud patched-bit words from global memory into a new LDS region during setup. The chain steps then read their bits from LDS rather than issuing global dword loads through the bit queue. The region is sized from the span of bit words the chains touch and is only enabled when the larger LDS footprint does not reduce work-groups per CU. The cost is a bulk copy at kernel start and more LDS use, and the emulator gains an equivalent path for checking.

```diff
diff --git a/groundgrid_amd/csrc/gg_context.hip b/groundgrid_amd/csrc/gg_context.hip
--- a/groundgrid_amd/csrc/gg_context.hip
+++ b/groundgrid_amd/csrc/gg_context.hip
@@ -1142,7 +1142,7 @@
     const size_t o_layers = carve((size_t)n_slots * percall_slot_floats * 4);
     a.gpl = make_gp_layout(n);
     a.gp_bits_off = (int)align_up((size_t)a.gpl.elems, 16);
-    a.gp_bits_words = (a.gpl.elems / 64 + 2 + 1) & ~1;
+    a.gp_bits_words = gp_bits_words_of(a.gpl);
     a.gp2_stride = align_up(((size_t)a.gp_bits_off + (size_t)a.gp_bits_words) * 8, A) / 8;
     a.gp_bits_stride = a.gp2_stride;
     const size_t o_gp2 = carve((size_t)n_slots * a.gp2_stride * 8);
@@ -2973,6 +2973,9 @@
         for (int k = 0; k < ctx->n_slots; ++k) c += ctx->lazy_pending[k] ? 1 : 0;
         return c;
     }
+    if (!strcmp(key, "sweep_launches_plain")) return (int)std::min<long>(sweep_launch_count(0), 1 << 30);
+    if (!strcmp(key, "sweep_launches_fresh_global")) return (int)std::min<long>(sweep_launch_count(1), 1 << 30);
+    if (!strcmp(key, "sweep_launches_fresh_lds")) return (int)std::min<long>(sweep_launch_count(2), 1 << 30);
     if (!strcmp(key, "export_variant_default")) return EXPORT_VARIANT_DEFAULT;
     if (!strcmp(key, "import_variant_default")) return IMPORT_VARIANT_DEFAULT;
     if (!strcmp(key, "images_variant_default")) return IMAGES_VARIANT_DEFAULT;
@@ -2989,6 +2992,7 @@
     else if (!strcmp(key, "sweep_pair_wgs")) ctx->arena.tune_sweep_pair_wgs = value;
     else if (!strcmp(key, "sweep_pair_waves")) ctx->arena.tune_sweep_pair_waves = value;
     else if (!strcmp(key, "fresh_maps")) ctx->fresh_enabled = value != 0;
+    else if (!strcmp(key, "fresh_bits_lds")) ctx->arena.tune_fresh_bits_global = value ? 0 : 1;
     else if (!strcmp(key, "front")) ctx->arena.tune_front = std::min(value, 3);
     else if (!strcmp(key, "sweep_poll_cap")) ctx->arena.tune_sweep_poll_cap = value;
     else if (!strcmp(key, "scan_parts")) ctx->arena.tune_scan_parts = value;
diff --git a/groundgrid_amd/csrc/gg_internal.h b/groundgrid_amd/csrc/gg_internal.h
--- a/groundgrid_amd/csrc/gg_internal.h
+++ b/groundgrid_amd/csrc/gg_internal.h
@@ -133,6 +133,7 @@
     int eigen_reduction;
     const DevConfig *slot_cfg;
     int slot_cfg_launch;
+    int tune_fresh_bits_global;
 };
 
 constexpr int PERCALL_LAYERS = 9;
@@ -316,6 +317,8 @@
 size_t sweep_pair_rec_floats(const sweep::Params &P);
 constexpr int SWEEP_PAIR_MAX_CLOUDS = 16;
 size_t sweep_lds_bytes(const sweep::Params &P);
+int sweep_fresh_bits_region(const sweep::Params &P, int gp_bits_words, int threads, size_t *lds_bytes);
+long sweep_launch_count(int kind);
 size_t sweep_xchg_entries(const sweep::Params &P);
 void launch_label(const Arena &a, const CloudParams *d_params, const BatchIO &io, int n_clouds, int max_n, hipStream_t s);
 void launch_score(const Arena &a, const CloudParams *d_params, const BatchIO &io, const ScoreArgs &sc, int n_clouds, int max_n, hipStream_t s);
diff --git a/groundgrid_amd/csrc/gp_layout.h b/groundgrid_amd/csrc/gp_layout.h
--- a/groundgrid_amd/csrc/gp_layout.h
+++ b/groundgrid_amd/csrc/gp_layout.h
@@ -60,6 +60,8 @@
     return 1 + ((side * L.G + g) * L.VS + v + GP_SHEAR * l) * 64 + l;
 }
 
+GPL_HD int gp_bits_words_of(const GpLayout &L) { return (L.elems / 64 + 2 + 1) & ~1; }
+
 GPL_HD bool gp_cell_of(const GpLayout &L, int e, int &row, int &col)
 {
     if (e == 0) {
diff --git a/groundgrid_amd/csrc/k4_sweep.hip b/groundgrid_amd/csrc/k4_sweep.hip
--- a/groundgrid_amd/csrc/k4_sweep.hip
+++ b/groundgrid_amd/csrc/k4_sweep.hip
@@ -2,6 +2,7 @@
 #include "sweep_core.h"
 
 #include <algorithm>
+#include <atomic>
 #include <cstdlib>
 
 #include <stdlib.h>
@@ -98,6 +99,7 @@
         const uint32_t w = bits_dword(bits_byte0 + (e >> 5) * 4u, 0u);
         return cell <= 0 || ((w >> (e & 31u)) & 1u) != 0u;
     }
+    GG_DEV uint32_t bits_lds(int word) const { return (uint32_t)lds[word]; }
     GG_DEV Cell fresh(const Cell &v) const
     {
         Cell o;
@@ -210,6 +212,9 @@
 #ifndef GG_SWEEP_BATCH_RANGES
 #define GG_SWEEP_BATCH_RANGES 3
 #endif
+#ifndef GG_SWEEP_FRESH_LDS_AHEAD
+#define GG_SWEEP_FRESH_LDS_AHEAD 0
+#endif
 #ifndef GG_SWEEP_BATCH_KINDS
 #define GG_SWEEP_BATCH_KINDS 2
 #endif
@@ -218,10 +223,11 @@
     static constexpr int bnd = B, join = J;
 };
 
-template <int SIDE, bool DBG, bool SPLIT, bool FRESH = false>
+template <int SIDE, bool DBG, bool SPLIT, bool FRESH = false, bool FBL = false>
 GG_DEV void run_chain(const Params &P, const LdsMap &L, DevMemT<DBG> &mem, int wave_of_side, int lane, WaveClockT<DBG> &clk, int g0, int g1)
 {
     static_assert(!(FRESH && SPLIT), "fresh maps: the plain chain only");
+    static_assert(FRESH || !FBL, "the bits in LDS: fresh maps only");
     ChainLane<SIDE> st;
     int have_prep = 0;
     const int w_take = lane == 0 ? L.take_done + SIDE : ((L.scratch + 1 + 3 * lane) & ~1) + 2;
@@ -232,7 +238,19 @@
         const int t_first = group_first_step(), t_last = group_last_step<SIDE>(r0, nl);
         const int has_next = __builtin_amdgcn_readfirstlane(group + 1 < P.groups ? 1 : 0);
         uint32_t fo_own = 0u, fo_out = 0u, sh_own = 0u, sh_out = 0u, mq_own[2] = {0u, 0u}, mq_out[2] = {0u, 0u};
-        if constexpr (FRESH) {
+        int lw_own = 0, lw_out = 0;
+        if constexpr (FRESH && FBL) {
+            lw_own = L.bits + fresh_bits_word(st.ownA + 64 * (t_first + 1 + (int)PF));
+            lw_out = L.bits + fresh_bits_word(st.outA + 64 * (t_first + 1 + (int)PF));
+            sh_own = fresh_bits_shift(st.ownA);
+            sh_out = fresh_bits_shift(st.outA);
+            st.xold_bit = mem.bit_of(st.xold_cell);
+            st.end_bit = mem.bit_of(st.own_end);
+            if (GG_SWEEP_FRESH_LDS_AHEAD) {
+                mq_own[0] = mem.bits_lds(lw_own);
+                mq_out[0] = mem.bits_lds(lw_out);
+            }
+        } else if constexpr (FRESH) {
             const unsigned eo = (unsigned)st.ownA - 1u, eu = (unsigned)st.outA - 1u;
             fo_own = mem.bits_byte0 + 8u * (unsigned)((int)(eo >> 6) + t_first + 1 + (int)PF) + 4u * ((eo & 63u) >> 5);
             fo_out = mem.bits_byte0 + 8u * (unsigned)((int)(eu >> 6) + t_first + 1 + (int)PF) + 4u * ((eu & 63u) >> 5);
@@ -327,6 +345,19 @@
                     if (AHEAD) rec_ahead = mem.ring_get(rec_word + (u + 1) * (int)LANES * (int)PREP_WORDS);
                     st.template take<STARTS, K::bnd>(t, tmod, rec, x_in, group > 0, mem);
                     mem.set_counter(w_take, step_no + 1 + AHEAD);
+                } else if constexpr (FRESH && FBL) {
+                    const int here = 2 * (t - t_first);
+                    uint32_t w_own, w_out;
+                    if (GG_SWEEP_FRESH_LDS_AHEAD) {
+                        w_own = mq_own[0], w_out = mq_out[0];
+                        mq_own[0] = mem.bits_lds(lw_own + here + 2);
+                        mq_out[0] = mem.bits_lds(lw_out + here + 2);
+                    } else {
+                        w_own = mem.bits_lds(lw_own + here);
+                        w_out = mem.bits_lds(lw_out + here);
+                    }
+                    const bool own_bit = ((w_own >> sh_own) & 1u) != 0u, out_bit = ((w_out >> sh_out) & 1u) != 0u;
+                    st.template step_a<STARTS, K::bnd, true>(t, u % (int)PF, tmod, x_in, P, L, K::bnd == 3 ? trip_bnd : group > 0, mem, own_bit, out_bit);
                 } else if constexpr (FRESH) {
                     static_assert((int)TRIP % 2 == 0, "the bit queue's slot is a constant of the unrolled trip");
                     const uint32_t w_own = mq_own[u & 1], w_out = mq_out[u & 1];
@@ -531,7 +562,7 @@
     }
 }
 
-template <bool DBG, bool PARTS, bool FRESH = false, bool SC = false>
+template <bool DBG, bool PARTS, bool FRESH = false, bool SC = false, bool FBL = false>
 __global__ __launch_bounds__(1024, 5) void k_sweep(const Arena a, const Params P_arg, const CloudParams *__restrict__ params, int n_clouds, int n_parts_rt,
                                                    unsigned long long *dbg)
 {
@@ -564,7 +595,8 @@
         }
     }
     const int g0 = part * P_arg.gpw, g1 = min(g0 + P_arg.gpw, P_arg.groups);
-    const LdsMap L = lds_layout(P_arg.c, P_arg.groups, g0, g1, P_arg.split_steps != 0);
+    static_assert(!FBL || (FRESH && !PARTS), "the bits in LDS: fresh maps, one work-group per cloud");
+    const LdsMap L = lds_layout(P_arg.c, P_arg.groups, g0, g1, P_arg.split_steps != 0, FBL ? P_arg.fresh_bits_words : 0);
     const CloudParams &cp = params[cloud];
     Params P_own;
     if (SC) {
@@ -579,6 +611,17 @@
     float2 *gp2 = gp2_ptr(a, cp.slot);
     float *percall = percall_ptr(a, cp.slot);
     const int nthreads = blockDim.x;
+    const uint4 *bits_src = nullptr;
+    uint4 bits_q[4];
+    const int bits_n = FBL ? a.gp_bits_words >> 1 : 0;
+    if (FBL) {
+        bits_src = reinterpret_cast<const uint4 *>(a.gp_bits + (size_t)cp.slot * a.gp_bits_stride);
+#pragma unroll
+        for (int k = 0; k < 4; ++k) {
+            const int i = (int)threadIdx.x + k * nthreads;
+            bits_q[k] = i < bits_n ? bits_src[i] : make_uint4(0u, 0u, 0u, 0u);
+        }
+    }
 
     for (int k = threadIdx.x; k < L.corner; k += nthreads) lds[k] = 0;
     if (PARTS && threadIdx.x == 0) sweep_wait_failed = 0u;
@@ -617,6 +660,15 @@
                 if ((cols_live >> live_bit(cell)) & 1u) points[cell] = 0.0f;
             }
         }
+    }
+    if (FBL) {
+        uint4 *bits_dst = reinterpret_cast<uint4 *>(lds + L.bits);
+#pragma unroll
+        for (int k = 0; k < 4; ++k) {
+            const int i = (int)threadIdx.x + k * nthreads;
+            if (i < bits_n) bits_dst[i] = bits_q[k];
+        }
+        for (int i = (int)threadIdx.x + 4 * nthreads; i < bits_n; i += nthreads) bits_dst[i] = bits_src[i];
     }
     __syncthreads();
 
@@ -654,13 +706,13 @@
         } else if (PARTS && g1 < P.groups)
             run_export<DBG>(P, L, mem, lane, g1);
     } else if (wave < 4 * W && side == SIDE_A)
-        run_chain<SIDE_A, DBG, false, FRESH>(P, L, mem, w_of_side, lane, clk, g0, g1);
+        run_chain<SIDE_A, DBG, false, FRESH, FBL>(P, L, mem, w_of_side, lane, clk, g0, g1);
     else if (wave < 4 * W && side == SIDE_B)
-        run_chain<SIDE_B, DBG, false, FRESH>(P, L, mem, w_of_side, lane, clk, g0, g1);
+        run_chain<SIDE_B, DBG, false, FRESH, FBL>(P, L, mem, w_of_side, lane, clk, g0, g1);
     else if (wave < 4 * W && side == SIDE_C)
-        run_chain<SIDE_C, DBG, false, FRESH>(P, L, mem, w_of_side, lane, clk, g0, g1);
+        run_chain<SIDE_C, DBG, false, FRESH, FBL>(P, L, mem, w_of_side, lane, clk, g0, g1);
     else if (wave < 4 * W)
-        run_chain<SIDE_D, DBG, false, FRESH>(P, L, mem, w_of_side, lane, clk, g0, g1);
+        run_chain<SIDE_D, DBG, false, FRESH, FBL>(P, L, mem, w_of_side, lane, clk, g0, g1);
     else if (wave == 4 * W)
         run_corner<0, DBG, FRESH>(P, L, mem, lane, clk, g0, g1);
     else if (wave == 4 * W + 1)
@@ -692,6 +744,42 @@
 }
 size_t sweep_lds_bytes(const Params &P) { return parts_lds_bytes(P, 1); }
 size_t sweep_xchg_entries(const Params &P) { return (size_t)xchg_entries(P.groups); }
+
+static int wgs_per_cu(size_t dyn_lds_bytes, int threads)
+{
+    const size_t granule = 2048, need = (dyn_lds_bytes + 16 + granule - 1) / granule * granule;
+    return (int)std::min<size_t>(160 * 1024 / need, (size_t)(20 / std::max(threads / 64, 1)));
+}
+int sweep_fresh_bits_region(const Params &P, int gp_bits_words, int threads, size_t *lds_bytes)
+{
+    if (lds_bytes) *lds_bytes = 0;
+    if (P.rings <= 0 || P.gpw < P.groups || P.split_steps) return 0;
+    const LdsMap T = lds_layout(P.c, P.groups, 0, P.groups, false);
+    const int words = fresh_bits_region_words(P, 2 * gp_bits_words);
+    if (words <= 0) return 0;
+    const LdsMap L = lds_layout(P.c, P.groups, 0, P.groups, false, words);
+    const size_t with = (size_t)L.words * 4, without = (size_t)T.words * 4;
+    if (with > 158 * 1024 || wgs_per_cu(with, threads) < wgs_per_cu(without, threads)) return 0;
+    if (lds_bytes) *lds_bytes = with;
+    return words;
+}
+static std::atomic<long> sweep_launch_counts[3];
+long sweep_launch_count(int kind) { return kind >= 0 && kind < 3 ? sweep_launch_counts[kind].load() : -1; }
+
+extern "C" int gg_debug_fresh_sweep_lds(int n, long out[6])
+{
+    if (n < 8 || !out) return GG_ERR_INVALID;
+    const Params P = make_params(n, 0.33, 12.0f, 10.0);
+    const int threads = (4 * P.waves_per_side + 2) * 64;
+    size_t with = 0;
+    out[2] = sweep_fresh_bits_region(P, gp_bits_words_of(P.gl), threads, &with);
+    out[0] = (long)with;
+    out[1] = (long)parts_lds_bytes(P, P.gpw);
+    out[3] = with ? wgs_per_cu(with, threads) : 0;
+    out[4] = wgs_per_cu((size_t)out[1], threads);
+    out[5] = (long)sizeof(sweep_static);
+    return GG_OK;
+}
 
 bool sweep_takes_fresh(const Arena &a, const Params &P_in, int n_clouds)
 {
@@ -733,7 +821,13 @@
                         ? 1
                         : 0;
     if (P.split_steps) P.waves_per_side = 1;
-    const size_t lds = parts_lds_bytes(P, P.gpw, P.split_steps != 0);
+    size_t lds = parts_lds_bytes(P, P.gpw, P.split_steps != 0);
+    const int threads = P.split_steps ? 12 * 64 : (4 * P.waves_per_side + 2 + (n_parts > 1 ? 2 : 0)) * 64;
+    size_t lds_with_bits = 0;
+    P.fresh_bits_words = 0;
+    if (!dbg && a.fresh_launch && !P.split_steps && n_parts == 1 && !a.tune_fresh_bits_global) P.fresh_bits_words = sweep_fresh_bits_region(P, a.gp_bits_words, threads, &lds_with_bits);
+    const bool fbl = P.fresh_bits_words > 0;
+    if (fbl) lds = lds_with_bits;
     static PerDeviceOnce big_lds;
     if (lds > 64 * 1024)
         big_lds.run([] {
@@ -746,15 +840,19 @@
             hipFuncSetAttribute(reinterpret_cast<const void *>(k_sweep<false, true, false, true>), hipFuncAttributeMaxDynamicSharedMemorySize, 160 * 1024 - 256);
             hipFuncSetAttribute(reinterpret_cast<const void *>(k_sweep<false, false, true, true>), hipFuncAttributeMaxDynamicSharedMemorySize, 160 * 1024 - 256);
             hipFuncSetAttribute(reinterpret_cast<const void *>(k_sweep<false, true, true, true>), hipFuncAttributeMaxDynamicSharedMemorySize, 160 * 1024 - 256);
+            hipFuncSetAttribute(reinterpret_cast<const void *>(k_sweep<false, false, true, false, true>), hipFuncAttributeMaxDynamicSharedMemorySize, 160 * 1024 - 256);
+            hipFuncSetAttribute(reinterpret_cast<const void *>(k_sweep<false, false, true, true, true>), hipFuncAttributeMaxDynamicSharedMemorySize, 160 * 1024 - 256);
         });
     P.fresh_cell = a.gp_fresh_cell;
     P.poll_cap = a.tune_sweep_poll_cap > 0 ? a.tune_sweep_poll_cap : 1 << 22;
     P.debug_fault = a.tune_sweep_fault;
-    const int threads = P.split_steps ? 12 * 64 : (4 * P.waves_per_side + 2 + (n_parts > 1 ? 2 : 0)) * 64;
+    sweep_launch_counts[dbg || !a.fresh_launch || P.split_steps ? 0 : fbl ? 2 : 1]++;
     if (dbg)
         hipLaunchKernelGGL((k_sweep<true, true>), dim3(n_clouds * n_parts), dim3(threads), lds, s, a, P, d_params, n_clouds, n_parts, dbg);
     else if (a.slot_cfg_launch) {
-        if (a.fresh_launch && !P.split_steps && n_parts == 1)
+        if (fbl)
+            hipLaunchKernelGGL((k_sweep<false, false, true, true, true>), dim3(n_clouds), dim3(threads), lds, s, a, P, d_params, n_clouds, n_parts, dbg);
+        else if (a.fresh_launch && !P.split_steps && n_parts == 1)
             hipLaunchKernelGGL((k_sweep<false, false, true, true>), dim3(n_clouds), dim3(threads), lds, s, a, P, d_params, n_clouds, n_parts, dbg);
         else if (a.fresh_launch && !P.split_steps)
             hipLaunchKernelGGL((k_sweep<false, true, true, true>), dim3(n_clouds * n_parts), dim3(threads), lds, s, a, P, d_params, n_clouds, n_parts, dbg);
@@ -762,7 +860,9 @@
             hipLaunchKernelGGL((k_sweep<false, true, false, true>), dim3(n_clouds * n_parts), dim3(threads), lds, s, a, P, d_params, n_clouds, n_parts, dbg);
         else
             hipLaunchKernelGGL((k_sweep<false, false, false, true>), dim3(n_clouds * n_parts), dim3(threads), lds, s, a, P, d_params, n_clouds, n_parts, dbg);
-    } else if (a.fresh_launch && !P.split_steps && n_parts == 1)
+    } else if (fbl)
+        hipLaunchKernelGGL((k_sweep<false, false, true, false, true>), dim3(n_clouds), dim3(threads), lds, s, a, P, d_params, n_clouds, n_parts, dbg);
+    else if (a.fresh_launch && !P.split_steps && n_parts == 1)
         hipLaunchKernelGGL((k_sweep<false, false, true>), dim3(n_clouds), dim3(threads), lds, s, a, P, d_params, n_clouds, n_parts, dbg);
     else if (a.fresh_launch && !P.split_steps)
         hipLaunchKernelGGL((k_sweep<false, true, true>), dim3(n_clouds * n_parts), dim3(threads), lds, s, a, P, d_params, n_clouds, n_parts, dbg);
diff --git a/groundgrid_amd/csrc/sweep_core.h b/groundgrid_amd/csrc/sweep_core.h
--- a/groundgrid_amd/csrc/sweep_core.h
+++ b/groundgrid_amd/csrc/sweep_core.h
@@ -48,6 +48,7 @@
     int debug_fault;
     int keep_points;
     GpLayout gl;
+    int fresh_bits_words;
 };
 
 template <int SIDE> SW_HD int chain_len(int r) { return SIDE == SIDE_A ? 2 * r - 2 : SIDE == SIDE_D ? 2 * r : 2 * r - 1; }
@@ -174,6 +175,7 @@
     int bnd_base;
     int scratch;
     int prep;
+    int bits;
     int words;
 };
 
@@ -192,7 +194,7 @@
 SW_HD int xchg_misc(int gb, int k) { return xchg_base(gb) + 4 * xchg_len(gb) + k; }
 
 enum { PREP_DEPTH = TRIP, PREP_WORDS = 6 };
-SW_HD LdsMap lds_layout(int c, int groups, int g0 = 0, int g1 = -1, bool split_steps = false)
+SW_HD LdsMap lds_layout(int c, int groups, int g0 = 0, int g1 = -1, bool split_steps = false, int bits_words = 0)
 {
     if (g1 < 0) g1 = groups;
     LdsMap m;
@@ -222,6 +224,12 @@
     o = (o + 1) & ~1;
     m.prep = o;
     if (split_steps) o += 4 * PREP_DEPTH * LANES * PREP_WORDS;
+    m.bits = 0;
+    if (bits_words > 0) {
+        o = (o + 3) & ~3;
+        m.bits = o;
+        o += bits_words;
+    }
     m.words = o;
     return m;
 }
@@ -556,6 +564,39 @@
 SW_HD int group_first_step() { return -2 - PF; }
 template <int SIDE> SW_HD int group_last_step(int r0, int nl) { return SKEW * (nl - 1) + chain_len<SIDE>(r0 + nl - 1) - 1; }
 
+SW_HD int fresh_bits_word(int e) { return 2 * ((e - 1) >> 6) + (((e - 1) & 63) >> 5); }
+SW_HD unsigned fresh_bits_shift(int e) { return (unsigned)(e - 1) & 31u; }
+template <int SIDE> inline void fresh_bits_range(const Params &P, const LdsMap &L, int group, int &lo, int &hi)
+{
+    const int r0 = LANES * group + 1;
+    const int nl = P.rings - (r0 - 1) < (int)LANES ? P.rings - (r0 - 1) : (int)LANES;
+    const int t_first = group_first_step();
+    int t_last = group_last_step<SIDE>(r0, nl);
+    t_last += (TRIP - (t_last - t_first + 1) % TRIP) % TRIP;
+    for (int lane = 0; lane < LANES; ++lane) {
+        ChainLane<SIDE> st;
+        st.init(lane, r0, nl, group, P, L);
+        const int a[2] = {st.ownA, st.outA};
+        for (int k = 0; k < 2; ++k) {
+            const int w0 = fresh_bits_word(a[k] + 64 * (t_first + 1 + (int)PF)), w1 = fresh_bits_word(a[k] + 64 * (t_last + 1 + (int)PF));
+            lo = w0 < lo ? w0 : lo;
+            hi = w1 > hi ? w1 : hi;
+        }
+    }
+}
+inline int fresh_bits_region_words(const Params &P, int bits_words32)
+{
+    const LdsMap T = lds_layout(P.c, P.groups, 0, P.groups, false, 4);
+    int lo = 0, hi = bits_words32 - 1;
+    for (int group = 0; group < P.groups; ++group) {
+        fresh_bits_range<SIDE_A>(P, T, group, lo, hi);
+        fresh_bits_range<SIDE_B>(P, T, group, lo, hi);
+        fresh_bits_range<SIDE_C>(P, T, group, lo, hi);
+        fresh_bits_range<SIDE_D>(P, T, group, lo, hi);
+    }
+    return T.bits + lo < 0 ? -1 : (hi + 1 + 3) & ~3;
+}
+
 template <int CD> struct CornerRing {
     int r;
     bool live;
diff --git a/groundgrid_amd/csrc/sweep_emul.hip b/groundgrid_amd/csrc/sweep_emul.hip
--- a/groundgrid_amd/csrc/sweep_emul.hip
+++ b/groundgrid_amd/csrc/sweep_emul.hip
@@ -20,6 +20,16 @@
     std::vector<int32_t> lds;
     bool late;
     long loads = 0, stores = 0, lds_ops = 0;
+    bool lds_fault = false;
+    uint32_t bits_lds(int word)
+    {
+        ++lds_ops;
+        if (word < 0 || (size_t)word >= lds.size()) {
+            lds_fault = true;
+            return ~0u;
+        }
+        return (uint32_t)lds[(size_t)word];
+    }
     std::vector<uint64_t> *xchg = nullptr;
     uint32_t seq = 1;
     void export_wp_if(bool c, int entry, WP v)
@@ -148,7 +158,7 @@
         advanced = false;
     }
     bool done() const override { return group >= g1; }
-    bool bad() const override { return plan_mismatch; }
+    bool bad() const override { return plan_mismatch || mem.lds_fault; }
     bool half = false;
     bool try_step() override
     {
@@ -179,6 +189,13 @@
                 for (int l = 0; l < LANES; ++l)
                     lane[l].take(t, tmod, mem.ring_get(L.prep + ((SIDE * PREP_DEPTH + (step_no % PREP_DEPTH)) * LANES + l) * PREP_WORDS), x_in[l], group > 0, mem);
                 mem.set_counter(L.take_done + SIDE, step_no + 1);
+            } else if (mem.bits && L.bits) {
+                for (int l = 0; l < LANES; ++l) {
+                    const uint32_t w_own = mem.bits_lds(L.bits + fresh_bits_word(lane[l].ownA + 64 * (t + 1 + (int)PF)));
+                    const uint32_t w_out = mem.bits_lds(L.bits + fresh_bits_word(lane[l].outA + 64 * (t + 1 + (int)PF)));
+                    lane[l].template step_a<true, 1, true>(t, slot, tmod, x_in[l], P, L, group > 0, mem, ((w_own >> fresh_bits_shift(lane[l].ownA)) & 1u) != 0u,
+                                                           ((w_out >> fresh_bits_shift(lane[l].outA)) & 1u) != 0u);
+                }
             } else if (mem.bits) {
                 for (int l = 0; l < LANES; ++l) {
                     const int eo = lane[l].ownA + 64 * (t + 1 + (int)PF), eu = lane[l].outA + 64 * (t + 1 + (int)PF);
@@ -389,6 +406,7 @@
     P.debug_fault = 0;
     P.keep_points = 0;
     P.fresh_cell = 0;
+    P.fresh_bits_words = 0;
     P.gpw = P.groups > 1 ? P.groups : 1;
     if (getenv("GG_SWEEP_WAVES")) P.waves_per_side = std::max(1, std::min(std::min(P.groups, 3), atoi(getenv("GG_SWEEP_WAVES"))));
     int r2 = 0;
@@ -440,7 +458,7 @@
 }
 
 static int emulate_ring_sweep(int n, double resolution, float min_dist_squared, float *gp2, float base_z, double decrease, unsigned seed, int late_loads, long *stats,
-                              const unsigned char *patched, float fresh_ground)
+                              const unsigned char *patched, float fresh_ground, int bits_in_lds = 1, int bits_copy = -1)
 {
     if (n < 8 || !gp2) return GG_ERR_INVALID;
     Params P = gg::sweep::make_params(n, resolution, min_dist_squared, decrease);
@@ -457,7 +475,7 @@
     std::vector<uint64_t> bits;
     if (patched) {
         if (late_loads) return GG_ERR_INVALID;
-        bits.assign((size_t)P.gl.elems / 64 + 2, 0ull);
+        bits.assign((size_t)gg::gp_bits_words_of(P.gl), 0ull);
         const float poison = __builtin_nanf("");
         for (int col = 0; col < n; ++col)
             for (int row = 0; row < n; ++row) {
@@ -470,6 +488,11 @@
             for (int row = 0; row < n; ++row)
                 if (std::max(std::abs(row - P.c), std::abs(col - P.c)) >= P.c && !patched[(size_t)row + (size_t)col * n])
                     sheared[(size_t)gp_index(P.gl, row, col)] = sheared[(size_t)P.fresh_cell];
+    }
+    if (patched && bits_in_lds && n_parts == 1 && P.rings > 0) {
+        const int words = fresh_bits_region_words(P, 2 * (int)bits.size());
+        if (words < 0) return -13;
+        P.fresh_bits_words = words;
     }
     std::vector<uint64_t> xchg(2 * (size_t)std::max(xchg_entries(P.groups), 1), 0ull);
     std::vector<LdsMap> maps((size_t)n_parts);
@@ -482,11 +505,16 @@
         const int g0 = part * P.gpw, g1 = std::min(g0 + P.gpw, P.groups);
         LdsMap &L = maps[(size_t)part];
         HostMem &mem = mems[(size_t)part];
-        L = lds_layout(P.c, P.groups, g0, g1, P.split_steps != 0);
+        L = lds_layout(P.c, P.groups, g0, g1, P.split_steps != 0, P.fresh_bits_words);
         lds_words = std::max(lds_words, (size_t)L.words);
         mem.gp2 = sheared.data();
         mem.bits = patched ? &bits : nullptr;
         mem.lds.assign((size_t)L.words, 0);
+        if (L.bits) {
+            std::fill(mem.lds.begin() + L.bits, mem.lds.end(), (int32_t)-1);
+            const size_t n_copy = bits_copy < 0 ? bits.size() : std::min(bits.size(), (size_t)bits_copy);
+            memcpy(&mem.lds[(size_t)L.bits], bits.data(), n_copy * 8);
+        }
         mem.late = late_loads != 0;
         mem.xchg = &xchg;
         mem.seq = 7;
@@ -580,6 +608,12 @@
                                            unsigned seed, int late_loads, long *stats)
 {
     return emulate_ring_sweep(n, resolution, min_dist_squared, gp2, base_z, decrease, seed, late_loads, stats, nullptr, 0.0f);
+}
+extern "C" int gg_debug_emulate_ring_sweep_fresh_bits(int n, double resolution, float min_dist_squared, float *gp2, const unsigned char *patched, float fresh_ground, float base_z,
+                                                      double decrease, unsigned seed, long *stats, int bits_in_lds, int bits_copy)
+{
+    if (!patched) return GG_ERR_INVALID;
+    return emulate_ring_sweep(n, resolution, min_dist_squared, gp2, base_z, decrease, seed, 0, stats, patched, fresh_ground, bits_in_lds, bits_copy);
 }
 extern "C" int gg_debug_emulate_ring_sweep_fresh(int n, double resolution, float min_dist_squared, float *gp2, const unsigned char *patched, float fresh_ground, float base_z,
                                                  double decrease, unsigned seed, long *stats)
```

After: 218,000, median of 6. No clear change (+0.4%).
